# achacond/k-step_FM-index

Hardware: AMD Instinct MI355X
Metric: Mqueries/s (100 bp reads, 3 Gbase index) (higher is better)
Workload: dtype u32; 1 GPU; Task-2Step backward search, 3 Gbase index, 10M x 100 bp reads per GPU; backend=task-mid, k=2, d=64, ref_size=3000000000, queries_per_gpu=10000000, qlen=100, query_upload=ascii, parallelism=query-sharded dp1, index replicated per GPU, no collective

## Files before the change

### include/kstep_fmi.h

```cpp
#ifndef KSTEP_FMI_H_
#define KSTEP_FMI_H_

#include <stdint.h>

#ifdef __cplusplus
extern "C" {
#endif

enum {
  KFMI_SUCCESS                = 0,
  KFMI_E_OPENING_INDEX_FILE   = 1,
  KFMI_E_ALLOCATING_BWT       = 2,
  KFMI_E_ALLOCATING_FMI       = 3,
  KFMI_E_READING_BWT          = 4,
  KFMI_E_READING_FMI          = 5,
  KFMI_E_SAVING_INDEX_FILE    = 6,
  KFMI_E_SAVING_BWT_FILE      = 7,
  KFMI_E_BUILDING_BWT         = 8,
  KFMI_E_BUILDING_FMI         = 9,
  KFMI_E_OPENING_REFERENCE_FILE = 10,
  KFMI_E_ALLOCATING_REFERENCE = 11,
  KFMI_E_READING_MFASTA_FILE  = 12,
  KFMI_E_READING_REFERENCE_FILE = 13,
  KFMI_E_OPENING_MFASTA_FILE  = 14,
  KFMI_E_ALLOCATING_MFASTA    = 15,
  KFMI_E_ALLOCATING_RESULTS   = 16,
  KFMI_E_OPENING_RESULTS_FILE = 17,
  KFMI_E_READING_RESULTS_FILE = 18,
  KFMI_E_NOT_IMPLEMENTED      = 19,
  KFMI_E_NO_DEVICE            = 30,
  KFMI_E_DEVICE_ALLOC         = 31,
  KFMI_E_KERNEL               = 32,
  KFMI_E_BAD_ARGUMENT         = 33,
  KFMI_E_NOT_ON_DEVICE        = 34,
  KFMI_INDEX_VER_BASELINE      = 100,
  KFMI_INDEX_VER_INTERLEAVE    = 101,
  KFMI_INDEX_VER_BASELINE_AC   = 200,
  KFMI_INDEX_VER_INTERLEAVE_AC = 201
};


int32_t loadIndex(const char *fn, void **index);
int32_t saveIndex(const char *fn, void *index);
int32_t initResults(uint32_t numresults, void **results);
void    searchIndexGPU(void *index, void *queries, void *resIntervals);
void    searchIndexCPU(void *index, void *queries, void *resIntervals);
int32_t freeIndex(void **index);
int32_t freeReference(void **reference, void **index);
int32_t buildIndex(void *reference, void **index);
int32_t freeQueriesGPU(void **queries);
int32_t freeResultsGPU(void **results);
int32_t freeIndexGPU(void **index);
int32_t transferGPUtoCPU(void *results);
int32_t transferCPUtoGPU(void *index, void *queries, void *results);
int32_t kfmi_queries_upload_form(void *queries);

double   sampleTime(void);
uint32_t base2index(uint32_t base);
int32_t  loadRef(const char *fn, uint32_t refsize, void **reference);
int32_t  saveRef(const char *fn, void *reference);
int32_t  loadQueries(const char *fn, uint32_t sizequery, uint32_t numqueries, void **queries);
int32_t  writeResults(const char *fn, uint32_t *results, uint32_t numqueries);
int32_t  loadResults(const char *fn, void **results);
int32_t  freeQueries(void **queries);
int32_t  freeResults(void **results);
int32_t  saveResults(const char *fn, void *results, void *index);
char    *errorCommon(int32_t e);


int32_t     kfmi_set_backend(const char *name);
const char *kfmi_get_backend(void);
int32_t     kfmi_set_device(int32_t device);
int32_t     kfmi_device_count(void);
int32_t     kfmi_device_pci_bus_id(int32_t device, char *buf, int32_t len);
int32_t     kfmi_last_error(void);
int32_t     kfmi_search(void *index, void *queries, void *results);
int32_t     kfmi_search_cpu(void *index, void *queries, void *results, int32_t nthreads);
#define KFMI_FTAB_AUTO 0xFFFFFFFFu
int32_t     kfmi_set_ftab(uint32_t bases);
uint32_t    kfmi_ftab_auto_bases(uint64_t rows, uint32_t K, uint64_t budget_bytes);
#define KFMI_FTAB_BUDGET_FREE 0xFFFFFFFFFFFFFFFFull
int32_t     kfmi_set_ftab_budget(uint64_t bytes);
uint64_t    kfmi_device_ftab_bytes(void *index);
#define KFMI_SKIP_AUTO 0xFFFFFFFFu
int32_t     kfmi_set_skip(uint32_t mode);
uint32_t    kfmi_skip_in_effect(void);
uint32_t    kfmi_skip_auto(uint64_t rows, uint32_t K, uint64_t budget_bytes);
uint64_t    kfmi_device_skip_bytes(void *index);
int32_t     kfmi_device_skip_table(void *index, void *out, uint64_t entries, uint32_t *steps);
#define KFMI_JUMP_AUTO 0xFFFFFFFFu
#define KFMI_JUMP_MIN_DEFAULT 8u
int32_t     kfmi_set_jump(uint32_t mode);
uint32_t    kfmi_jump_in_effect(void);
int32_t     kfmi_set_jump_min(uint32_t bases);
uint32_t    kfmi_jump_min(void);
uint32_t    kfmi_jump_auto(uint64_t rows, uint32_t K, uint64_t budget_bytes);
uint64_t    kfmi_device_jump_bytes(void *index);
int32_t     kfmi_device_jump_tables(void *index, uint32_t member, uint32_t *sa, uint32_t *isa, uint64_t rows,
                                    uint32_t *text, uint64_t words);
int32_t     kfmi_set_jump_lines(uint32_t mode);
uint32_t    kfmi_jump_lines(void);
uint64_t    kfmi_device_jump_line_bytes(void *index);
int32_t     kfmi_device_jump_lines(void *index, uint32_t member, uint32_t *out, uint64_t lines);
int32_t     kfmi_jump_line_geometry(uint64_t n, uint64_t p, uint32_t nb, uint64_t *out);
int32_t     kfmi_set_split_class(uint32_t cls);
int32_t     kfmi_set_fused(int32_t on);
int32_t     kfmi_set_walk_check(uint32_t mode);
int32_t     kfmi_fail_index_uploads(uint32_t n);
int32_t     kfmi_walk_check_last(void);
int32_t     kfmi_set_devices(const int32_t *devices, int32_t n);
int32_t     kfmi_get_devices(int32_t *devices, int32_t cap);
int32_t     kfmi_last_timing(double *ms_total, double *ms_pack, double *ms_lf);

int32_t kfmi_load_index_tag(const char *fn, uint32_t required_tag, void **index);
int32_t kfmi_index_from_image(const void *image, uint64_t bytes, void **index);
int32_t kfmi_index_image(void *index, const void **image, uint64_t *bytes);
int32_t kfmi_index_header(void *index, uint32_t *out14);

int32_t kfmi_transform_interleave(void *index100, void **index101);
int32_t kfmi_transform_ac(void *index100, void **index200, void **index201);
int32_t kfmi_transform_plain(void *index_ac, void **index100);

int32_t   kfmi_queries_from_buffer(const char *ascii, uint64_t num, uint32_t size, void **queries);
int32_t   kfmi_results_alloc(uint64_t num, void **results);
uint32_t *kfmi_results_host(void *results);
uint64_t  kfmi_results_num(void *results);

int32_t kfmi_build_index_cpu(const char *text, uint64_t n, uint32_t k, uint32_t d, void **index);
int32_t kfmi_build_index_gpu(const char *text, uint64_t n, uint32_t k, uint32_t d,
                             int32_t want_host_image, void **index);
int32_t kfmi_derive_index_gpu(void *index, uint32_t k_out, int32_t want_host_image, void **out);
int32_t kfmi_set_alphabet(const char *mode);
int32_t kfmi_build_stats(uint64_t *ties, uint32_t *rounds);

int32_t kfmi_count_blocks(void *index, void *queries, uint64_t *blocks);
int32_t kfmi_count_lines(void *index, void *queries, uint64_t out[4]);

int32_t kfmi_search_stream(void *index, const char *ascii, uint64_t num, uint32_t size,
                           uint32_t *results, uint64_t chunk);
int32_t kfmi_load_queries_gpu(const char *fn, uint32_t sizequery, uint64_t numqueries, void **queries);
int32_t kfmi_pack_queries(const char *ascii, uint64_t num, uint32_t size, uint32_t *words);
int32_t kfmi_pack_queries_k(const char *ascii, uint64_t num, uint32_t size, uint32_t k, uint32_t *words);
int32_t kfmi_host_threads(void);
int32_t kfmi_host_alloc(uint64_t bytes, void **p);
int32_t kfmi_host_free(void *p);
int32_t kfmi_stream_release(void);
double  kfmi_stream_hostpacked_fraction(void);

enum { KFMI_STRAND_FWD = 1, KFMI_STRAND_REV = 2, KFMI_STRAND_BOTH = 3 };
int32_t kfmi_search_strands(void *index, void *queries, void *results, uint32_t strands);
int32_t kfmi_search_stream_strands(void *index, const char *ascii, uint64_t num, uint32_t size,
                                   uint32_t *results, uint64_t chunk, uint32_t strands);
int32_t kfmi_search_cpu_strands(void *index, void *queries, void *results, uint32_t strands, int32_t nthreads);
int32_t kfmi_revcomp_queries(const char *ascii, uint64_t num, uint32_t size, char *out);
int32_t kfmi_strand_words_host(const uint32_t *words, uint64_t num, uint32_t size, uint32_t k,
                               uint32_t strands, uint32_t *out);
int32_t kfmi_reverse_stream_host(const uint32_t *words, uint64_t num, uint32_t size, uint32_t maxw,
                                 uint32_t *out);

int32_t kfmi_search_seeds(void *index, void *queries, void *intervals, void *spans,
                          uint32_t max_seeds, uint32_t strands);
int32_t kfmi_search_seeds_cpu(void *index, void *queries, void *intervals, void *spans,
                              uint32_t max_seeds, uint32_t strands, int32_t nthreads);

#define KFMI_HIT_NONE         0xFFFFFFFFu
#define KFMI_HIT_MISM_MASK    0x0000FFFFu
#define KFMI_HIT_MULTI        0x00010000u
#define KFMI_HIT_SCORED_SHIFT 20
#define KFMI_VERIFY_MAX_OCC   256u
int32_t kfmi_verify_seeds(void *index, void *queries, void *intervals, void *spans, void *hits,
                          uint32_t max_seeds, uint32_t strands, uint32_t max_occ, uint32_t max_mism);
int32_t kfmi_verify_seeds_cpu(const char *text, uint64_t n, const uint32_t *sa, uint64_t rows,
                              void *queries, void *intervals, void *spans, void *hits,
                              uint32_t max_seeds, uint32_t strands, uint32_t max_occ, uint32_t max_mism,
                              int32_t nthreads);
int32_t kfmi_results_to_device(void *results);

enum {
  KFMI_TRACE_STEP = 1u, KFMI_TRACE_SKIP_HIT = 1u << 16, KFMI_TRACE_SKIP_MISS = 1u << 24,
  KFMI_TRACE_JUMP_TRIED = 1u, KFMI_TRACE_JUMP_LINE = 2u,
  KFMI_TRACE_JUMP_OUT_SHIFT = 2, KFMI_TRACE_JUMP_POS_SHIFT = 4, KFMI_TRACE_JUMP_NB_SHIFT = 16,
  KFMI_TRACE_JUMP_TAKEN = 0, KFMI_TRACE_JUMP_REFUSED = 1, KFMI_TRACE_JUMP_DIFFERED = 2, KFMI_TRACE_JUMP_BAD_ISA = 3
};
int32_t kfmi_search_trace(void *index, void *queries, void *results, uint32_t *trace);

int32_t kfmi_probe_replay(void *index, void *queries, int32_t unroll, int32_t groups, int32_t reps, double *ms,
                          uint64_t *lines, uint64_t *trace_bytes);

uint64_t kfmi_device_index_bytes(void *index);


int32_t kfmi_build_index_ex(const char *text, uint64_t n, uint32_t k, uint32_t d, uint32_t sa_rate,
                            int32_t on_device, void **index);
int32_t kfmi_index_sa(void *index, const uint32_t **sa, uint64_t *count, uint32_t *rate);
int32_t kfmi_save_sa(const char *fn, void *index);
int32_t kfmi_load_sa(const char *fn, void *index);
int32_t         kfmi_locate(void *index, void *results, uint32_t max_occ, void **locations);
uint64_t        kfmi_locations_total(void *locations);
const uint64_t *kfmi_locations_offsets(void *locations);
const uint32_t *kfmi_locations_positions(void *locations);
int32_t         kfmi_locations_free(void **locations);

#ifdef __cplusplus
}
#endif

#endif
```

### k-step_fm-index_amd/csrc/hip/kfmi_coop.h

```cpp
#ifndef KFMI_COOP_H_
#define KFMI_COOP_H_

#include <type_traits>

#include "kfmi_device.h"

namespace kfmi {


template <class G>
struct CoopCfg {
  static constexpr int BC = G::BMW / 4;
  static constexpr bool NBR = G::NEIGHBOR;
  static constexpr int TPR = NBR ? pow2ceil(2 * BC) : pow2ceil(BC + 1);
  static constexpr int RPR = 64 / TPR;
  static constexpr int SLOT = TPR * 16;
  static constexpr int MAXREQ = 128;
  static constexpr int MAXR = MAXREQ / RPR;
  using Desc = typename std::conditional<(G::NC > 16), uint64_t, uint32_t>::type;
  static constexpr int WAVE_LDS = MAXREQ * SLOT + MAXREQ * (int) sizeof(Desc);
  static constexpr int WPB0 = 65536 / WAVE_LDS;
  static constexpr int WPB = WPB0 < 1 ? 1 : (WPB0 > 4 ? 4 : WPB0);
  static constexpr bool OK = (G::BMW % 4 == 0) && (G::EW % 4 == 0) && (G::BOFF % 4 == 0) &&
                             (!G::ACRULE || G::HALF >= 4) && (!G::MIDLINES || G::NC >= 4) &&
                             TPR <= 64;
};

template <class G>
__device__ __forceinline__ const uint8_t* coop_chunk_addr(const IdxArgs& ix, uint32_t b, uint32_t c, int k)
{
  using C = CoopCfg<G>;
  const uint8_t* base = reinterpret_cast<const uint8_t*>(ix.ent);
  const uint64_t eb = (uint64_t) b * (G::EW * 4);
  if constexpr (G::MIDLINES) {
    const uint64_t lb = (uint64_t) (b >> 1) * (G::EW * 4);
    if (k < C::BC) return base + lb + ((b & 1u) * G::BMW + 4 * k) * 4;
    return base + lb + (G::MIDCNT + (c & ~3u)) * 4;
  }
  if constexpr (G::LAY == LAY_GRP) {
    const uint64_t lb = ((uint64_t) b * G::NGRP + c / G::NCG) * (G::EW * 4);
    if (k < C::BC) return base + lb + 16 * k;
    return base + lb + (G::BMW + ((c % G::NCG) & ~3u)) * 4;
  }
  if (k < C::BC) return base + eb + (G::BOFF + 4 * k) * 4;
  if constexpr (G::LAY == LAY_INTER) {
    return base + eb + (G::BMW + (c & ~3u)) * 4;
  } else {
    const bool e = ((b & 1u) != 0) == (c < (uint32_t) G::HALF);
    return base + (uint64_t) (b + (e ? 1u : 0u)) * (G::EW * 4) + ((c & (G::HALF - 1)) & ~3u) * 4;
  }
}

template <class G>
__device__ __forceinline__ uint32_t coop_lf(const IdxArgs& ix, const uint8_t* slot, uint32_t b, uint32_t X,
                                            uint32_t c, const uint32_t (&sx)[2 * G::K])
{
  using C = CoopCfg<G>;
  const int o = (int) (X - b * (uint32_t) G::D);
  bool e = false;
  if constexpr (G::ACRULE) e = ((b & 1u) != 0) == (c < (uint32_t) G::HALF);
  if constexpr (G::MIDLINES) e = (b & 1u) == 0;
  uint32_t pop = 0, all = 0;
  if constexpr (G::PW <= 4) {
#pragma unroll
    for (int k = 0; k < C::BC; ++k) {
      const uint4 v = *reinterpret_cast<const uint4*>(slot + 16 * k);
      const uint32_t pl[4] = {v.x, v.y, v.z, v.w};
#pragma unroll
      for (int h = 0; h < 4 / G::PW; ++h) {
        const int w = k * (4 / G::PW) + h;
        uint32_t m = row_mask(o - 32 * w);
        if constexpr (G::TWO_SIDED) m = e ? ~m : m;
        const uint32_t sel = select_rows<G::K>(&pl[h * G::PW], sx);
        pop += __popc(m & sel);
        if constexpr (G::LAY == LAY_MIDAC) all += __popc(sel);
      }
    }
  } else {
    uint32_t pl[G::BMW];
#pragma unroll
    for (int k = 0; k < C::BC; ++k) {
      const uint4 v = *reinterpret_cast<const uint4*>(slot + 16 * k);
      pl[4 * k] = v.x; pl[4 * k + 1] = v.y; pl[4 * k + 2] = v.z; pl[4 * k + 3] = v.w;
    }
#pragma unroll
    for (int w = 0; w < G::NB; ++w) {
      uint32_t m = row_mask(o - 32 * w);
      if constexpr (G::TWO_SIDED) m = e ? ~m : m;
      pop += __popc(m & select_rows<G::K>(&pl[w * G::PW], sx));
    }
  }
  const uint32_t cnt = reinterpret_cast<const uint32_t*>(slot + 16 * C::BC)[c & 3u];
  if constexpr (G::LAY == LAY_MIDAC)
    if (b >= ix.ac_tail_b0) return ac_tail_step<G>(ix, b, c, X, pop, all);
  return finish<G>(ix, cnt, pop, b, c, X, e);
}

template <class G>
__device__ __forceinline__ uint32_t coop_lf_nbr(const IdxArgs& ix, const uint8_t* slot, uint32_t b, uint32_t X,
                                                uint32_t c, const uint32_t (&sx)[2 * G::K], uint32_t cnt, bool e,
                                                bool prev)
{
  using C = CoopCfg<G>;
  const int o = (int) (X - b * (uint32_t) G::D);
  uint32_t pl[G::BMW];
#pragma unroll
  for (int k = 0; k < C::BC; ++k) {
    const uint4 v = *reinterpret_cast<const uint4*>(slot + 16 * k);
    pl[4 * k] = v.x; pl[4 * k + 1] = v.y; pl[4 * k + 2] = v.z; pl[4 * k + 3] = v.w;
  }
  uint32_t pop = 0;
#pragma unroll
  for (int w = 0; w < G::NB; ++w) {
    uint32_t m = row_mask(o - 32 * w);
    if constexpr (G::TWO_SIDED) m = e ? ~m : m;
    pop += __popc(m & select_rows<G::K>(&pl[w * G::PW], sx));
  }
  if (prev) {
#pragma unroll
    for (int k = 0; k < C::BC; ++k) {
      const uint4 v = *reinterpret_cast<const uint4*>(slot + 16 * (C::BC + k));
      pl[4 * k] = v.x; pl[4 * k + 1] = v.y; pl[4 * k + 2] = v.z; pl[4 * k + 3] = v.w;
    }
#pragma unroll
    for (int w = 0; w < G::NB; ++w) pop += __popc(select_rows<G::K>(&pl[w * G::PW], sx));
    return finish_prev<G>(ix, cnt, pop, b, c, X);
  }
  return finish<G>(ix, cnt, pop, b, c, X, e);
}

template <class G>
__host__ __device__ constexpr uint32_t coop_stage_rows(uint32_t m)
{
  uint32_t r = 64;
  while (r >= 16 && r * m + 16 > (uint32_t) CoopCfg<G>::WAVE_LDS) r >>= 1;
  return r >= 16 ? r : 0u;
}

template <class G, int MAXW>
__global__ __launch_bounds__(64 * CoopCfg<G>::WPB) void coop_kernel(IdxArgs ix, const uint32_t* __restrict__ qp,
                                                                    const uint8_t* __restrict__ ascii, uint32_t m,
                                                                    uint64_t num, uint32_t steps, uint32_t nwords,
                                                                    uint32_t* __restrict__ res)
{
  using C = CoopCfg<G>;
  constexpr int RW = MAXW > 0 ? MAXW : 1;
  constexpr int CW = MAXW > 0 && G::K == 3 ? k3_words<RW>() : RW;
  extern __shared__ __attribute__((aligned(16))) uint8_t lds[];
  const int wave = threadIdx.x >> 6;
  const int lane = threadIdx.x & 63;
  uint8_t* wl = lds + wave * C::WAVE_LDS;
  using Desc = typename C::Desc;
  Desc* tab = reinterpret_cast<Desc*>(wl + C::MAXREQ * C::SLOT);
  const uint64_t q0 = ((uint64_t) blockIdx.x * C::WPB + wave) * 64;
  if (q0 >= num) return;
  const uint64_t q = q0 + lane;
  const uint64_t qs = q < num ? q : num - 1;
  const int k = lane % C::TPR;
  const int g = lane / C::TPR;
  uint32_t cw[CW];
  uint32_t rc = 0;
  if constexpr (MAXW > 0) {
    uint32_t raw[RW];
    const uint32_t rpr = coop_stage_rows<G>(m);
#pragma unroll 1
    for (uint32_t h = 0; h < 64u / rpr; ++h) {
      const uint64_t r0 = q0 + h * rpr;
      const uint64_t nr = r0 < num ? (num - r0 < rpr ? num - r0 : rpr) : 0;
      const uint32_t n16 = (uint32_t) ((nr * m + 15) / 16);
      const uint4* src = reinterpret_cast<const uint4*>(ascii + r0 * m);
      for (uint32_t i = lane; i < n16; i += 64) reinterpret_cast<uint4*>(wl)[i] = src[i];
      asm volatile("s_waitcnt vmcnt(0) lgkmcnt(0)" ::: "memory");
      if ((uint32_t) lane / rpr == h) {
        row_codes<MAXW>(wl, (uint64_t) (lane % rpr) * m, m - ix.rem, raw);
        rc = rem_code(wl + (uint64_t) (lane % rpr) * m + m - ix.rem, ix.rem);
      }
      asm volatile("s_waitcnt lgkmcnt(0)" ::: "memory");
    }
    if (q >= num) {
#pragma unroll
      for (int i = 0; i < RW; ++i) raw[i] = 0;
      rc = 0;
    }
    if constexpr (G::K == 3) recut30<RW>(raw, cw);
    else {
#pragma unroll
      for (int i = 0; i < CW; ++i) cw[i] = raw[i];
    }
  }
  uint32_t L = 0, R = ix.bwtsize;
  uint32_t skip = 0;
  if (ix.ftab && steps >= ix.ftab_steps) {
    skip = ix.ftab_steps;
    uint32_t w0;
    if constexpr (MAXW > 0) w0 = cw[0];
    else w0 = qp[qs];
    const uint2 lr = ix.ftab[w0 & ix.ftab_mask];
    L = lr.x;
    R = lr.y;
  }
  if (ix.rem) {
    if constexpr (MAXW == 0) rc = qp[(uint64_t) nwords * num + qs];
    const uint2 lr = ix.rtab[rc];
    L = lr.x;
    R = lr.y;
  }

  for (uint32_t w = 0; w < nwords; ++w) {
    uint32_t word;
    if constexpr (MAXW > 0) {
      word = cw[0];
#pragma unroll
      for (int i = 0; i + 1 < CW; ++i) cw[i] = cw[i + 1];
    } else {
      word = qp[(uint64_t) w * num + qs];
    }
    const uint32_t left = steps - w * G::SPW;
#pragma unroll 1
    for (int j = 0; j < G::SPW; ++j) {
      if ((uint32_t) j >= left) break;
      if (w * G::SPW + j < skip) continue;
      const uint32_t c = (word >> (2 * G::K * j)) & (uint32_t) (G::NC - 1);
      const uint32_t bl = L / (uint32_t) G::D, br = R / (uint32_t) G::D;
      const bool needR = br != bl;
      const uint64_t mask = __ballot(needR);
      const uint32_t nreq = 64u + (uint32_t) __popcll(mask);
      const uint32_t slotR = 64u + __builtin_amdgcn_mbcnt_hi((uint32_t) (mask >> 32),
                                                             __builtin_amdgcn_mbcnt_lo((uint32_t) mask, 0u));
      bool eL = false, eR = false, pL = false, pR = false;
      const uint32_t* acL = nullptr;
      const uint32_t* acR = nullptr;
      if constexpr (C::NBR) {
        Where<G> wL = locate<G>(ix, bl, c);
        Where<G> wR = locate<G>(ix, br, c);
        line_local_prev<G>(ix, bl, c, wL);
        line_local_prev<G>(ix, br, c, wR);
        eL = wL.e;
        pL = wL.prev;
        acL = wL.cnt;
        eR = wR.e;
        pR = wR.prev;
        acR = wR.cnt;
      }
      tab[lane] = (Desc) bl * (Desc) G::NC + c;
      if (needR) tab[slotR] = (Desc) br * (Desc) G::NC + c;
      asm volatile("s_waitcnt lgkmcnt(0)" ::: "memory");
      uint32_t cwL = 0, cwR = 0;
      const uint32_t rounds = (nreq + C::RPR - 1) / C::RPR;
      for (uint32_t r = 0; r < rounds; ++r) {
        const uint32_t s = r * C::RPR + g;
        if constexpr (C::NBR) {
          if (s < nreq && k < 2 * C::BC) {
            const Desc desc = tab[s];
            const uint32_t b = (uint32_t) (desc / (Desc) G::NC), cc = (uint32_t) (desc % (Desc) G::NC);
            Where<G> w = locate<G>(ix, b, cc);
            line_local_prev<G>(ix, b, cc, w);
            const uint32_t* p = k < C::BC ? w.planes + 4 * k
                                : w.prev ? w.pplanes + 4 * (k - C::BC)
                                : k == C::BC ? reinterpret_cast<const uint32_t*>(reinterpret_cast<uintptr_t>(w.cnt) & ~(uintptr_t) 15)
                                : nullptr;
            if (p)
              __builtin_amdgcn_global_load_lds((const void*) p,
                                               (__attribute__((address_space(3))) void*) (wl + r * 1024), 16, 0, 0);
          }
        } else if (s < nreq && k <= C::BC) {
          const Desc desc = tab[s];
          const uint32_t b = (uint32_t) (desc / (Desc) G::NC), cc = (uint32_t) (desc % (Desc) G::NC);
          const uint8_t* src = coop_chunk_addr<G>(ix, b, cc, k);
          __builtin_amdgcn_global_load_lds((const void*) src,
                                           (__attribute__((address_space(3))) void*) (wl + r * 1024), 16, 0, 0);
        }
      }
      if constexpr (C::NBR) {
        const uint64_t mpl = __ballot(pL), mpr = __ballot(needR && pR);
        uint64_t sv, gm;
        asm volatile("s_mov_b64 %[sv], exec\n"
                     "s_bfm_b64 %[gm], 32, 0\n"
                     "s_and_b64 exec, %[sv], %[gm]\n"
                     "s_and_b64 exec, exec, %[ml]\n"
                     "s_cbranch_execz .Lcl0_%=\n"
                     "global_load_dword %[cl], %[al], off\n"
                     ".Lcl0_%=:\n"
                     "s_and_b64 exec, %[sv], %[gm]\n"
                     "s_and_b64 exec, exec, %[mr]\n"
                     "s_cbranch_execz .Lcc0_%=\n"
                     "global_load_dword %[cr], %[ar], off\n"
                     ".Lcc0_%=:\n"
                     "s_bfm_b64 %[gm], 32, 32\n"
                     "s_and_b64 exec, %[sv], %[gm]\n"
                     "s_and_b64 exec, exec, %[ml]\n"
                     "s_cbranch_execz .Lcl1_%=\n"
                     "global_load_dword %[cl], %[al], off\n"
                     ".Lcl1_%=:\n"
                     "s_and_b64 exec, %[sv], %[gm]\n"
                     "s_and_b64 exec, exec, %[mr]\n"
                     "s_cbranch_execz .Lcc1_%=\n"
                     "global_load_dword %[cr], %[ar], off\n"
                     ".Lcc1_%=:\n"
                     "s_mov_b64 exec, %[sv]\n"
                     "s_waitcnt vmcnt(0)\n"
                     : [cl] "=&v"(cwL), [cr] "=&v"(cwR), [sv] "=&s"(sv), [gm] "=&s"(gm)
                     : [al] "v"(acL), [ar] "v"(acR), [ml] "s"(mpl), [mr] "s"(mpr)
                     : "memory", "scc");
      } else {
        asm volatile("s_waitcnt vmcnt(0)" ::: "memory");
      }
      uint32_t sx[2 * G::K];
      plane_xor<G::K>(c, sx);
      uint32_t nL, nR;
      if constexpr (C::NBR) {
        const uint8_t* sL = wl + lane * C::SLOT;
        const uint8_t* sR = wl + (needR ? slotR : (uint32_t) lane) * C::SLOT;
        const uint32_t cL = pL ? cwL : reinterpret_cast<const uint32_t*>(sL + 16 * C::BC)[c & 3u];
        const uint32_t cR = needR ? (pR ? cwR : reinterpret_cast<const uint32_t*>(sR + 16 * C::BC)[c & 3u]) : cL;
        nL = coop_lf_nbr<G>(ix, sL, bl, L, c, sx, cL, eL, pL);
        nR = coop_lf_nbr<G>(ix, sR, br, R, c, sx, cR, needR ? eR : eL, needR ? pR : pL);
      } else {
        nL = coop_lf<G>(ix, wl + lane * C::SLOT, bl, L, c, sx);
        nR = coop_lf<G>(ix, wl + (needR ? slotR : (uint32_t) lane) * C::SLOT, br, R, c, sx);
      }
      L = nL;
      R = nR;
      asm volatile("s_waitcnt lgkmcnt(0)" ::: "memory");
    }
  }
  if (q < num) *reinterpret_cast<uint2*>(res + 2 * q) = make_uint2(L, R);
}

template <class G>
hipError_t coop_launch(hipStream_t st, IdxArgs ix, const uint32_t* qp, const uint8_t* ascii, uint32_t m, int maxw,
                       uint64_t num, uint32_t steps, uint32_t nwords, uint32_t* res)
{
  using C = CoopCfg<G>;
  if constexpr (!C::OK) {
    return hipErrorInvalidValue;
  } else {
    const uint64_t waves = (num + 63) / 64;
    const uint64_t blocks = (waves + C::WPB - 1) / C::WPB;
    const size_t lds = (size_t) C::WPB * C::WAVE_LDS;
    if (maxw == 8)
      hipLaunchKernelGGL((coop_kernel<G, 8>), dim3((uint32_t) blocks), dim3(64 * C::WPB), lds, st, ix, qp, ascii, m,
                         num, steps, nwords, res);
    else if (maxw == 16)
      hipLaunchKernelGGL((coop_kernel<G, 16>), dim3((uint32_t) blocks), dim3(64 * C::WPB), lds, st, ix, qp, ascii, m,
                         num, steps, nwords, res);
    else
      hipLaunchKernelGGL((coop_kernel<G, 0>), dim3((uint32_t) blocks), dim3(64 * C::WPB), lds, st, ix, qp, ascii, m,
                         num, steps, nwords, res);
    return hipGetLastError();
  }
}

}

#endif
```

### k-step_fm-index_amd/csrc/hip/kfmi_device.h

```cpp
#ifndef KFMI_DEVICE_H_
#define KFMI_DEVICE_H_

#include <hip/hip_runtime.h>
#include <stdint.h>

namespace kfmi {

enum Layout : int { LAY_INTER = 0, LAY_AC = 1, LAY_MID = 3, LAY_MIDAC = 5, LAY_GRP = 6 };

__host__ __device__ constexpr int pow2ceil(int x) { int p = 1; while (p < x) p <<= 1; return p; }

template <int K_, int NB_, int LAY_>
struct Geo {
  static constexpr int K = K_;
  static constexpr int NB = NB_;
  static constexpr int LAY = LAY_;
  static constexpr int D = 32 * NB;
  static constexpr int NC = 1 << (2 * K);
  static constexpr int HALF = NC / 2;
  static constexpr int PW = 2 * K;
  static constexpr int BMW = PW * NB;
  static constexpr int NCG = NC < 16 ? NC : 16;
  static constexpr int NGRP = NC / NCG;
  static constexpr int EW = LAY == LAY_INTER ? BMW + NC
                          : LAY == LAY_AC    ? HALF + BMW
                          : LAY == LAY_GRP    ? pow2ceil(BMW + NCG)
                          : pow2ceil(2 * BMW + NC);
  static constexpr int BOFF = LAY == LAY_AC ? HALF : 0;
  static constexpr int MIDCNT = 2 * BMW;
  static constexpr bool ACRULE = LAY == LAY_AC;
  static constexpr int SPW = 32 / (2 * K);
  static constexpr bool SMALL = BMW <= 16;
  static constexpr bool TWO_SIDED = LAY == LAY_AC || LAY == LAY_MID || LAY == LAY_MIDAC;
  static constexpr bool MIDLINES = LAY == LAY_MID || LAY == LAY_MIDAC;
  static constexpr bool NEIGHBOR = (LAY == LAY_INTER || LAY == LAY_AC) && SMALL && BOFF + EW + BMW <= 32;
};

struct DollarArgs {
  uint32_t dpos[4];
  uint32_t dbase[4];
  uint32_t dblk[4];
  uint32_t duniq;
};

struct IdxArgs {
  const uint32_t* __restrict__ ent;
  uint32_t bwtsize;
  DollarArgs dl;
  const uint2* __restrict__ ftab;
  uint32_t ftab_steps, ftab_mask;
  const uint32_t* __restrict__ ac_tail;
  uint32_t ac_tail_b0;
  const uint2* __restrict__ rtab;
  uint32_t rem;
  uint32_t split;
  uint32_t lf_cap;
  const uint2* __restrict__ skip;
  uint32_t skip_rows, skip_steps, skip_split;
  const uint32_t* __restrict__ jsa;
  uint32_t jump_min, jump_split;
};

constexpr uint32_t SKIP_NONE = 0xFFFFFFFFu;

constexpr uint32_t JUMP_LINE_S = 16, JUMP_LINE_W = 256 - JUMP_LINE_S, JUMP_LINE_DW = 32, JUMP_LINE_TEXT = JUMP_LINE_S;
static_assert(JUMP_LINE_S == 16 && JUMP_LINE_S + 256 / 16 == JUMP_LINE_DW, "a line: S entries, then 256 bases in 16 dwords");
constexpr uint32_t JUMP_SPLIT4 = 4u, JUMP_LINES = 0x100u, JUMP_LINES_GROUPED = 0x200u;
constexpr uint32_t JUMP_LINES_GROUPED_MAX_M = 192;

__host__ __device__ constexpr uint64_t jump_text_words(uint64_t n) { return n / 16 + 2; }
__host__ __device__ constexpr uint64_t jump_line_count(uint64_t n) { return n / JUMP_LINE_S + 2; }
__host__ __device__ constexpr uint64_t jump_lines_off(uint64_t rows)
{
  return (2 * rows + jump_text_words(rows - 1) + (JUMP_LINE_DW - 1)) & ~(uint64_t) (JUMP_LINE_DW - 1);
}

struct JumpLineAt {
  uint64_t isa_dw, text_dw;
  uint32_t shift, ndw;
};
__host__ __device__ constexpr JumpLineAt jump_line_at(uint32_t n, uint32_t p, uint32_t nb)
{
  const uint32_t e = n - p + nb, j = e / JUMP_LINE_S;
  const uint32_t s = 256u - JUMP_LINE_S + e % JUMP_LINE_S - nb;
  const uint64_t line = (uint64_t) j * JUMP_LINE_DW;
  return JumpLineAt{line + e % JUMP_LINE_S, line + JUMP_LINE_TEXT + (s >> 4), (s & 15u) * 2u,
                    ((s + nb + 15u) >> 4) - (s >> 4)};
}

typedef unsigned int v4u __attribute__((ext_vector_type(4)));
typedef unsigned int v2u __attribute__((ext_vector_type(2)));

template <bool NT>
__device__ __forceinline__ v4u ld4(const uint32_t* p)
{
  if constexpr (NT) return __builtin_nontemporal_load(reinterpret_cast<const v4u*>(p));
  else return *reinterpret_cast<const v4u*>(p);
}
template <bool NT>
__device__ __forceinline__ v2u ld2(const uint32_t* p)
{
  if constexpr (NT) return __builtin_nontemporal_load(reinterpret_cast<const v2u*>(p));
  else return *reinterpret_cast<const v2u*>(p);
}
template <bool NT>
__device__ __forceinline__ uint32_t ld1(const uint32_t* p)
{
  if constexpr (NT) return __builtin_nontemporal_load(p);
  else return *p;
}

template <class G>
__host__ __device__ constexpr int plane_align()
{
  int a = 16;
  while (a > 4 && ((4 * G::EW) % a || (4 * G::BOFF) % a)) a >>= 1;
  return a;
}

template <int A, int N, bool NT = false>
__device__ __forceinline__ void load_words(const uint32_t* __restrict__ p, uint32_t* __restrict__ out)
{
  if constexpr (A >= 16 && N % 4 == 0) {
#pragma unroll
    for (int i = 0; i < N / 4; ++i) {
      const v4u v = ld4<NT>(p + 4 * i);
      out[4 * i + 0] = v.x; out[4 * i + 1] = v.y; out[4 * i + 2] = v.z; out[4 * i + 3] = v.w;
    }
  } else if constexpr (A >= 8 && N % 2 == 0) {
#pragma unroll
    for (int i = 0; i < N / 2; ++i) {
      asm volatile("" ::: "memory");
      const v2u v = ld2<NT>(p + 2 * i);
      out[2 * i + 0] = v.x; out[2 * i + 1] = v.y;
    }
  } else {
#pragma unroll
    for (int i = 0; i < N; ++i) {
      asm volatile("" ::: "memory");
      out[i] = ld1<NT>(p + i);
    }
  }
}

__device__ __forceinline__ uint32_t code_of(uint32_t x)
{
  uint32_t b1 = x & 4u, f2 = x & 2u;
  uint32_t b0 = b1 ? (f2 ^ 2u) : f2;
  return (b1 | b0) >> 1;
}

__device__ __forceinline__ uint32_t group_codes_rev(uint32_t x)
{
  const uint32_t b1 = (x >> 2) & 0x01010101u;
  const uint32_t y = (b1 << 1) | (((x >> 1) & 0x01010101u) ^ b1);
  return ((y >> 24) & 0x03u) | ((y >> 14) & 0x0Cu) | ((y >> 4) & 0x30u) | ((y << 6) & 0xC0u);
}

template <int MAXW>
__device__ __forceinline__ void push_codes(uint32_t (&cw)[MAXW], uint32_t v, uint32_t sh)
{
#pragma unroll
  for (int k = MAXW - 1; k > 0; --k) cw[k] = __builtin_amdgcn_alignbit(cw[k], cw[k - 1], 32u - sh);
  cw[0] = (cw[0] << sh) | v;
}

template <int MAXW>
__device__ __forceinline__ void row_codes(const uint8_t* __restrict__ base, uint64_t off, uint32_t m,
                                          uint32_t (&cw)[MAXW])
{
  const uint32_t* a = reinterpret_cast<const uint32_t*>(base + (off & ~3ull));
  const uint32_t sh = (uint32_t) (off & 3u);
#pragma unroll
  for (int k = 0; k < MAXW; ++k) asm volatile("v_mov_b32 %0, 0" : "=v"(cw[k]));
  const uint32_t ng = m >> 2, rem = m & 3u;
  uint32_t lo = a[0];
#pragma unroll 8
  for (uint32_t i = 0; i < ng; ++i) {
    const uint32_t hi = a[i + 1];
    push_codes<MAXW>(cw, group_codes_rev(__builtin_amdgcn_alignbyte(hi, lo, sh)), 8u);
    lo = hi;
  }
  if (rem) {
    const uint32_t x = __builtin_amdgcn_alignbyte(a[ng + 1], lo, sh);
    push_codes<MAXW>(cw, group_codes_rev(x) >> (2u * (4u - rem)), 2u * rem);
  }
}

__device__ __forceinline__ uint32_t rem_code(const uint8_t* __restrict__ p, uint32_t rem)
{
  uint32_t c = 0;
  for (uint32_t u = 0; u < rem; ++u) c |= code_of(p[rem - 1 - u]) << (2 * u);
  return c;
}

template <int MAXW>
__host__ __device__ constexpr int k3_words() { return (MAXW * 32 + 29) / 30; }

template <int MAXW>
__device__ __forceinline__ void recut30(const uint32_t (&in)[MAXW], uint32_t (&out)[k3_words<MAXW>()])
{
#pragma unroll
  for (int j = 0; j < k3_words<MAXW>(); ++j) {
    const int bit = 30 * j, w = bit >> 5, sh = bit & 31;
    const uint32_t lo = w < MAXW ? in[w] : 0u;
    const uint32_t hi = w + 1 < MAXW ? in[w + 1] : 0u;
    out[j] = (sh ? ((lo >> sh) | (hi << (32 - sh))) : lo) & 0x3FFFFFFFu;
  }
}

__host__ __device__ constexpr uint32_t stage_rows(uint32_t m) { return m <= 128 ? 32u : 16u; }
__host__ __device__ constexpr uint32_t stage_slot_bytes(uint32_t m) { return (stage_rows(m) * m + 31u) & ~15u; }

template <int MAXW>
__device__ __forceinline__ void stage_query_codes(const uint8_t* __restrict__ ascii, uint64_t num, uint32_t m,
                                                  uint8_t* __restrict__ lds, uint32_t (&cw)[MAXW], uint32_t rem,
                                                  uint32_t& rc)
{
  const uint32_t lane = threadIdx.x & 63u, wv = threadIdx.x >> 6;
  const uint32_t rpr = stage_rows(m);
  uint8_t* wl = lds + wv * stage_slot_bytes(m);
  const uint64_t q0 = (uint64_t) blockIdx.x * 256 + wv * 64;
#pragma unroll 1
  for (uint32_t h = 0; h < 64u / rpr; ++h) {
    const uint64_t r0 = q0 + h * rpr;
    const uint64_t nr = r0 < num ? (num - r0 < rpr ? num - r0 : rpr) : 0;
    const uint32_t n16 = (uint32_t) ((nr * m + 15) / 16);
    const uint4* src = reinterpret_cast<const uint4*>(ascii + r0 * m);
    for (uint32_t i = lane; i < n16; i += 64) reinterpret_cast<uint4*>(wl)[i] = src[i];
    __syncthreads();
    if (lane / rpr == h) {
      row_codes<MAXW>(wl, (uint64_t) (lane % rpr) * m, m - rem, cw);
      rc = rem_code(wl + (uint64_t) (lane % rpr) * m + m - rem, rem);
    }
    __syncthreads();
  }
}

__device__ __forceinline__ uint32_t row_mask(int sh)
{
  sh = sh < 0 ? 0 : (sh > 32 ? 32 : sh);
  return (uint32_t) ((0xFFFFFFFF00000000ull) >> sh);
}

template <int K>
__device__ __forceinline__ void plane_xor(uint32_t c, uint32_t (&sx)[2 * K])
{
#pragma unroll
  for (int p = 0; p < 2 * K; ++p) sx[p] = ((c >> p) & 1u) ? 0u : 0xFFFFFFFFu;
}

template <int K>
__device__ __forceinline__ uint32_t select_rows(const uint32_t* pl, const uint32_t (&sx)[2 * K])
{
  uint32_t v = ~0u;
#pragma unroll
  for (int p = 0; p < 2 * K; ++p) v &= pl[p] ^ sx[p];
  return v;
}

template <int K, bool TWO>
__device__ __forceinline__ int dollar_fix(const DollarArgs& dl, uint32_t b, uint32_t c, uint32_t X, bool e)
{
  int corr = 0;
#pragma unroll
  for (int s = 0; s < K; ++s) {
    bool hit = (dl.dblk[s] == b) && (dl.dbase[s] == c);
    bool cond = (TWO && e) ? (X <= dl.dpos[s]) : (X > dl.dpos[s]);
    corr += (hit && cond) ? 1 : 0;
  }
  return corr;
}

template <class G>
struct Where {
  const uint32_t* planes;
  const uint32_t* cnt;
  bool e;
  bool prev = false;
  const uint32_t* pplanes = nullptr;
};

template <class G>
__device__ __forceinline__ void line_local_prev(const IdxArgs& ix, uint32_t b, uint32_t c, Where<G>& w)
{
  if constexpr (G::NEIGHBOR) {
    if (b == 0) return;
    const uint64_t pb = 4ull * ((uint64_t) b * G::EW + G::BOFF);
    const uint64_t line = pb >> 7;
    if (((uint64_t) (w.cnt - ix.ent) * 4ull) >> 7 == line) return;
    if constexpr (G::LAY == LAY_AC) {
      if (!w.e || b >= ix.ac_tail_b0) return;
    }
    const uint32_t cw = G::LAY == LAY_AC ? (c & (G::HALF - 1)) : (uint32_t) G::BMW + c;
    const uint64_t e0 = (uint64_t) (b - 1) * G::EW;
    if ((4ull * (e0 + G::BOFF)) >> 7 != line || (4ull * (e0 + G::BOFF + G::BMW) - 1) >> 7 != line ||
        (4ull * (e0 + cw)) >> 7 != line)
      return;
    w.prev = true;
    w.e = false;
    w.pplanes = ix.ent + e0 + G::BOFF;
    w.cnt = ix.ent + e0 + cw;
  }
}

template <class G>
__device__ __forceinline__ Where<G> locate(const IdxArgs& ix, uint32_t b, uint32_t c)
{
  Where<G> w;
  if constexpr (G::LAY == LAY_INTER) {
    const uint32_t* ent = ix.ent + (uint64_t) b * G::EW;
    w.planes = ent;
    w.cnt = ent + G::BMW + c;
    w.e = false;
  } else if constexpr (G::LAY == LAY_AC) {
    const uint32_t* ent = ix.ent + (uint64_t) b * G::EW;
    w.e = ((b & 1u) != 0) == (c < (uint32_t) G::HALF);
    w.planes = ent + G::BOFF;
    w.cnt = ix.ent + (uint64_t) (b + (w.e ? 1u : 0u)) * G::EW + (c & (G::HALF - 1));
  } else if constexpr (G::LAY == LAY_GRP) {
    const uint32_t* line = ix.ent + ((uint64_t) b * G::NGRP + c / G::NCG) * G::EW;
    w.planes = line;
    w.cnt = line + G::BMW + c % G::NCG;
    w.e = false;
  } else {
    const uint32_t* line = ix.ent + (uint64_t) (b >> 1) * G::EW;
    w.e = (b & 1u) == 0;
    w.planes = line + (b & 1u) * G::BMW;
    w.cnt = line + G::MIDCNT + c;
  }
  return w;
}

template <class G, bool NT = false>
__device__ __forceinline__ uint32_t load_counter(const IdxArgs& ix, const Where<G>& w, uint32_t b, uint32_t c)
{
  (void) ix; (void) b; (void) c;
  return ld1<NT>(w.cnt);
}

template <class G>
__device__ __forceinline__ uint32_t ac_clamp(const IdxArgs& ix, uint32_t v)
{
  const uint32_t cap = ((ix.bwtsize + (uint32_t) G::D - 1u) / (uint32_t) G::D + 2u) * (uint32_t) G::D - 1u;
  return v > cap ? cap : v;
}

template <int K>
__device__ __forceinline__ uint32_t dollar_dup(const DollarArgs& dl, uint32_t b, uint32_t c)
{
  uint32_t n = 0;
#pragma unroll
  for (int s = 1; s < K; ++s) n += (dl.dblk[s] == b && dl.dbase[s] == c && !((dl.duniq >> s) & 1u)) ? 1u : 0u;
  return n;
}

template <class G>
__device__ __forceinline__ bool ac_rule_e(uint32_t b, uint32_t c)
{
  return ((b & 1u) != 0) == (c < (uint32_t) G::HALF);
}

template <class G>
__device__ __forceinline__ uint32_t finish(const IdxArgs& ix, uint32_t cnt, uint32_t pop, uint32_t b, uint32_t c,
                                          uint32_t X, bool e)
{
  const int corr = dollar_fix<G::K, G::TWO_SIDED>(ix.dl, b, c, X, e);
  const uint32_t bc = pop - (uint32_t) corr;
  if constexpr (G::ACRULE) return ac_clamp<G>(ix, e ? cnt - bc : cnt + bc);
  if constexpr (G::MIDLINES) {
    uint32_t v = e ? cnt - bc : cnt + bc;
    if (G::K > 1 && ix.dl.duniq != (1u << G::K) - 1u) {
      const uint32_t dup = dollar_dup<G::K>(ix.dl, b, c);
      const bool want = G::LAY == LAY_MIDAC && ac_rule_e<G>(b, c);
      v = v - (e ? dup : 0u) + (want ? dup : 0u);
    }
    return min(v, ix.lf_cap);
  }
  if constexpr (G::TWO_SIDED) return min(e ? cnt - bc : cnt + bc, ix.lf_cap);
  return min(cnt + bc, ix.lf_cap);
}

template <class G>
__device__ __forceinline__ uint32_t finish_prev(const IdxArgs& ix, uint32_t cnt, uint32_t pop, uint32_t b,
                                               uint32_t c, uint32_t X)
{
  int corr = 0;
#pragma unroll
  for (int s = 0; s < G::K; ++s) {
    if (ix.dl.dbase[s] != c) continue;
    if (ix.dl.dblk[s] == b) corr += X > ix.dl.dpos[s] ? 1 : 0;
    else if (ix.dl.dblk[s] + 1u == b) corr += (ix.dl.duniq >> s) & 1u;
  }
  uint32_t v = cnt + pop - (uint32_t) corr;
  if constexpr (G::ACRULE) {
    if (G::K > 1 && ac_rule_e<G>(b, c)) v += dollar_dup<G::K>(ix.dl, b, c);
    return ac_clamp<G>(ix, v);
  }
  return min(v, ix.lf_cap);
}

template <class G>
__device__ __forceinline__ uint32_t ac_tail_step(const IdxArgs& ix, uint32_t b, uint32_t c, uint32_t X,
                                                 uint32_t pop_mid, uint32_t pop_all)
{
  const bool e = ((b & 1u) != 0) == (c < (uint32_t) G::HALF);
  const bool e_mid = (b & 1u) == 0;
  const uint32_t pop = e == e_mid ? pop_mid : pop_all - pop_mid;
  uint32_t row = b + (e ? 1u : 0u) - ix.ac_tail_b0;
  row = row > 2u ? 2u : row;
  const uint32_t cnt = ix.ac_tail[row * (uint32_t) G::NC + c];
  const int corr = dollar_fix<G::K, true>(ix.dl, b, c, X, e);
  const uint32_t bc = pop - (uint32_t) corr;
  return ac_clamp<G>(ix, e ? cnt - bc : cnt + bc);
}

template <class G>
struct Blk {
  uint32_t bm[G::BMW];
  uint32_t bp[G::NEIGHBOR ? G::BMW : 1];
  uint32_t cnt;
  uint32_t b;
  bool e;
  bool prev;
};

template <class G, bool NT = false>
__device__ __forceinline__ void load_planes(const uint32_t* __restrict__ p, uint32_t (&bm)[G::BMW])
{
  load_words<plane_align<G>(), G::BMW, NT>(p, bm);
}

template <class G, bool NT = false>
__device__ __forceinline__ void fetch_block(const IdxArgs& ix, uint32_t b, uint32_t c, Blk<G>& k)
{
  Where<G> w = locate<G>(ix, b, c);
  line_local_prev<G>(ix, b, c, w);
  k.b = b;
  k.e = w.e;
  k.prev = w.prev;
  load_planes<G, NT>(w.planes, k.bm);
  if constexpr (G::NEIGHBOR) {
    if (w.prev) load_planes<G, NT>(w.pplanes, k.bp);
  }
  k.cnt = load_counter<G, NT>(ix, w, b, c);
}

template <class G>
__device__ __forceinline__ uint32_t lf_from_block(const IdxArgs& ix, const Blk<G>& k, uint32_t X, uint32_t c,
                                                  const uint32_t (&sx)[2 * G::K])
{
  const int o = (int) (X - k.b * (uint32_t) G::D);
  uint32_t pop = 0;
#pragma unroll
  for (int w = 0; w < G::NB; ++w) {
    uint32_t m = row_mask(o - 32 * w);
    if constexpr (G::TWO_SIDED) m = k.e ? ~m : m;
    pop += __popc(m & select_rows<G::K>(&k.bm[w * G::PW], sx));
  }
  if constexpr (G::LAY == LAY_MIDAC) {
    if (k.b >= ix.ac_tail_b0) {
      uint32_t all = 0;
#pragma unroll
      for (int w = 0; w < G::NB; ++w) all += __popc(select_rows<G::K>(&k.bm[w * G::PW], sx));
      return ac_tail_step<G>(ix, k.b, c, X, pop, all);
    }
  }
  if constexpr (G::NEIGHBOR) {
    if (k.prev) {
#pragma unroll
      for (int w = 0; w < G::NB; ++w) pop += __popc(select_rows<G::K>(&k.bp[w * G::PW], sx));
      return finish_prev<G>(ix, k.cnt, pop, k.b, c, X);
    }
  }
  return finish<G>(ix, k.cnt, pop, k.b, c, X, k.e);
}

template <class G>
__device__ __forceinline__ uint32_t lf_stream(const IdxArgs& ix, uint32_t X, uint32_t c,
                                              const uint32_t (&sx)[2 * G::K])
{
  const uint32_t b = X / (uint32_t) G::D;
  const int o = (int) (X - b * (uint32_t) G::D);
  const Where<G> wh = locate<G>(ix, b, c);
  const uint32_t cnt = load_counter<G>(ix, wh, b, c);
  const uint32_t* pl = wh.planes;
  constexpr int CH = G::NB < 8 ? G::NB : 8;
  uint32_t pop = 0, all = 0;
#pragma unroll
  for (int w0 = 0; w0 < G::NB; w0 += CH) {
    uint32_t v[CH][G::PW];
#pragma unroll
    for (int j = 0; j < CH; ++j) {
      const int w = w0 + j;
      if (w >= G::NB) break;
      load_words<plane_align<G>(), G::PW>(pl + G::PW * w, v[j]);
    }
#pragma unroll
    for (int j = 0; j < CH; ++j) {
      const int w = w0 + j;
      if (w >= G::NB) break;
      uint32_t m = row_mask(o - 32 * w);
      if constexpr (G::TWO_SIDED) m = wh.e ? ~m : m;
      const uint32_t sel = select_rows<G::K>(v[j], sx);
      pop += __popc(m & sel);
      if constexpr (G::LAY == LAY_MIDAC) all += __popc(sel);
    }
  }
  if constexpr (G::LAY == LAY_MIDAC)
    if (b >= ix.ac_tail_b0) return ac_tail_step<G>(ix, b, c, X, pop, all);
  return finish<G>(ix, cnt, pop, b, c, X, wh.e);
}

}

#endif
```

### k-step_fm-index_amd/csrc/hip/kfmi_jump.hip

```cpp
#include <hip/hip_runtime.h>
#include <stdint.h>
#include <stdlib.h>
#include <atomic>
#include <mutex>
#include <shared_mutex>

#include "../kfmi_internal.h"
#include "kfmi_device.h"
#include "kfmi_runtime.h"

namespace kfmi {

static std::atomic<uint32_t> g_jump_min{KFMI_JUMP_MIN_DEFAULT};
static std::atomic<int> g_jump_lines{-1};

extern "C" int32_t kfmi_set_jump_min(uint32_t bases)
{
  if (bases < 1) return KFMI_E_BAD_ARGUMENT;
  g_jump_min.store(bases, std::memory_order_relaxed);
  return KFMI_SUCCESS;
}

extern "C" uint32_t kfmi_jump_min(void) { return g_jump_min.load(std::memory_order_relaxed); }

extern "C" int32_t kfmi_set_jump_lines(uint32_t mode)
{
  if (mode > 2) return KFMI_E_BAD_ARGUMENT;
  g_jump_lines.store((int) mode, std::memory_order_relaxed);
  return KFMI_SUCCESS;
}

extern "C" uint32_t kfmi_jump_lines(void)
{
  const int v = g_jump_lines.load(std::memory_order_relaxed);
  if (v >= 0) return (uint32_t) v;
  static const uint32_t env = [] {
    const char* e = getenv("KFMI_JUMP_LINES");
    if (!e || !*e) return 1u;
    const int x = atoi(e);
    return x < 0 || x > 2 ? 1u : (uint32_t) x;
  }();
  return env;
}

static uint64_t text_words(uint64_t n) { return jump_text_words(n); }

extern "C" int32_t kfmi_jump_line_geometry(uint64_t n, uint64_t p, uint32_t nb, uint64_t* out)
{
  if (!out || n < 1 || n >= 0xFFFFFFFFull || p > n || nb < 1 || nb > JUMP_LINE_W || nb > p) return KFMI_E_BAD_ARGUMENT;
  const JumpLineAt at = jump_line_at((uint32_t) n, (uint32_t) p, nb);
  out[0] = jump_lines_off(n + 1);
  out[1] = jump_line_count(n);
  out[2] = at.isa_dw;
  out[3] = at.text_dw;
  out[4] = at.shift;
  out[5] = at.ndw;
  return KFMI_SUCCESS;
}

extern "C" uint32_t kfmi_jump_auto(uint64_t rows, uint32_t K, uint64_t budget_bytes)
{
  if (K < 1 || K > 2 || rows < 2 || rows > 0xFFFFFFFFull) return 0;
  return 16 * rows + 4 * text_words(rows - 1) <= budget_bytes ? 1u : 0u;
}

static bool jump_applies(const kfmi_dev_index* di)
{
  return di->K >= 1 && di->K <= 2 && !is_coop(di->backend) && (di->layout == LAY_INTER || di->layout == LAY_MID) &&
         di->bwtsize >= 2;
}

constexpr uint32_t JUMP_BAD_CHAIN = 1u, JUMP_BAD_POS = 2u, JUMP_BAD_ISA = 4u;

__device__ __forceinline__ int dollar_of(uint32_t row, const DollarArgs& dl, uint32_t K)
{
  int s = -1;
  for (int t = (int) K - 1; t >= 0; --t)
    if (dl.dpos[t] == row) s = t;
  return s;
}

__global__ __launch_bounds__(256) void jump_dist0_kernel(const uint32_t* __restrict__ next, uint64_t rows,
                                                         uint32_t* __restrict__ dist)
{
  for (uint64_t i = (uint64_t) blockIdx.x * 256 + threadIdx.x; i < rows; i += (uint64_t) gridDim.x * 256)
    dist[i] = next[i] == (uint32_t) i ? 0u : 1u;
}

__global__ __launch_bounds__(256) void jump_round_kernel(const uint32_t* __restrict__ next, const uint32_t* __restrict__ dist,
                                                         uint64_t rows, uint32_t split, uint32_t* __restrict__ next2,
                                                         uint32_t* __restrict__ dist2)
{
  const int grp = (int) (threadIdx.x & 63) / 16;
  for (uint64_t i0 = (uint64_t) blockIdx.x * 256 + (threadIdx.x & ~63u); i0 < rows; i0 += (uint64_t) gridDim.x * 256) {
    const uint64_t i = i0 + (threadIdx.x & 63u);
    const bool on = i < rows;
    const uint32_t j = on ? next[i] : 0u;
    const uint32_t d = on ? dist[i] : 0u;
    const bool ok = on && (uint64_t) j < rows;
    uint32_t nj = j, dj = 0u;
    if (split) {
#pragma unroll
      for (int g = 0; g < 4; ++g)
        if (ok && grp == g) {
          nj = next[j];
          dj = dist[j];
        }
    } else if (ok) {
      nj = next[j];
      dj = dist[j];
    }
    if (on) {
      next2[i] = nj;
      dist2[i] = d + dj;
    }
  }
}

__global__ __launch_bounds__(256) void jump_sa_kernel(uint32_t* __restrict__ next_sa, const uint32_t* __restrict__ dist,
                                                      uint64_t rows, DollarArgs dl, uint32_t K, uint32_t* __restrict__ bad)
{
  for (uint64_t i = (uint64_t) blockIdx.x * 256 + threadIdx.x; i < rows; i += (uint64_t) gridDim.x * 256) {
    const int s = dollar_of(next_sa[i], dl, K);
    const uint64_t p = (uint64_t) (s < 0 ? 0 : s) + (uint64_t) K * dist[i];
    uint32_t v = (uint32_t) p;
    if (s < 0) {
      atomicOr(bad, JUMP_BAD_CHAIN);
      v = SKIP_NONE;
    } else if (p >= rows) {
      atomicOr(bad, JUMP_BAD_POS);
      v = SKIP_NONE;
    }
    next_sa[i] = v;
  }
}

__global__ __launch_bounds__(256) void jump_isa_kernel(const uint32_t* __restrict__ sa, uint64_t rows, uint32_t split,
                                                       uint32_t* __restrict__ isa)
{
  const int grp = (int) (threadIdx.x & 63) / 16;
  for (uint64_t i0 = (uint64_t) blockIdx.x * 256 + (threadIdx.x & ~63u); i0 < rows; i0 += (uint64_t) gridDim.x * 256) {
    const uint64_t i = i0 + (threadIdx.x & 63u);
    const uint32_t p = i < rows ? sa[i] : SKIP_NONE;
    const bool ok = (uint64_t) p < rows;
    if (split) {
#pragma unroll
      for (int g = 0; g < 4; ++g)
        if (ok && grp == g) isa[p] = (uint32_t) i;
    } else if (ok) {
      isa[p] = (uint32_t) i;
    }
  }
}

__global__ __launch_bounds__(256) void jump_isa_check_kernel(const uint32_t* __restrict__ isa, uint64_t rows,
                                                             uint32_t* __restrict__ bad)
{
  for (uint64_t i = (uint64_t) blockIdx.x * 256 + threadIdx.x; i < rows; i += (uint64_t) gridDim.x * 256)
    if ((uint64_t) isa[i] >= rows) atomicOr(bad, JUMP_BAD_ISA);
}

void free_jump(kfmi_dev_index* di)
{
  if (di->jump_sa) (void) hipFree(di->jump_sa);
  di->jump_sa = nullptr;
  di->jump_auto = -1;
}

static int32_t build_jump(kfmi_dev_index* di, hipStream_t st)
{
  const uint64_t rows = di->bwtsize, n = rows - 1, words = text_words(n);
  const uint64_t loff = jump_lines_off(rows), lines = jump_line_count(n);
  uint32_t *keep = nullptr, *bad = nullptr;
  auto done = [&](int32_t code) {
    if (keep) (void) hipFree(keep);
    if (bad) (void) hipFree(bad);
    (void) hipGetLastError();
    return code;
  };
  static_assert(JUMP_LINE_DW >= 2 * JUMP_LINE_S, "two distance dwords per row fit the lines' part");
  if (hipMalloc((void**) &keep, 4 * (loff + lines * JUMP_LINE_DW)) != hipSuccess || hipMalloc((void**) &bad, 8) != hipSuccess)
    return done(KFMI_E_DEVICE_ALLOC);
  uint32_t* tmp = keep + loff;
  uint32_t* a[4] = {keep, tmp, keep + rows, tmp + rows};
  const uint32_t split = split_for(8 * rows, LAY_INTER) == 4u ? 1u : 0u;
  const dim3 grid(grid_blocks((rows + 255) / 256, 1u << 20));
  uint32_t rounds = 0;
  for (uint64_t span = 1; span < rows; span <<= 1) ++rounds;
  int cur = (rounds & 1u) ? 2 : 0;
  SearchLaunch l{};
  l.st = st;
  l.ix = idx_args(di);
  l.num = rows;
  l.perm_next = a[cur];
  l.perm_bad = bad;
  uint32_t h_bad[2] = {0, 0};
  auto flags = [&] {
    return hipGetLastError() == hipSuccess && hipMemcpyAsync(h_bad, bad, 8, hipMemcpyDeviceToHost, st) == hipSuccess &&
           hipStreamSynchronize(st) == hipSuccess;
  };
  if (hipMemsetAsync(bad, 0, 8, st) != hipSuccess || dispatch(Op::PermCheck, di->K, di->nb, di->layout, l) != hipSuccess)
    return done(KFMI_E_KERNEL);
  hipLaunchKernelGGL(jump_dist0_kernel, grid, dim3(256), 0, st, a[cur], rows, a[cur + 1]);
  for (uint32_t r = 0; r < rounds; ++r, cur ^= 2)
    hipLaunchKernelGGL(jump_round_kernel, grid, dim3(256), 0, st, a[cur], a[cur + 1], rows, split, a[cur ^ 2],
                       a[(cur ^ 2) + 1]);
  uint32_t *sa = a[0], *dist = a[1], *isa = a[2], *text = keep + 2 * rows;
  hipLaunchKernelGGL(jump_sa_kernel, grid, dim3(256), 0, st, sa, dist, rows, di->dl, di->K, bad + 1);
  if (hipMemsetAsync(isa, 0xFF, 4 * rows, st) != hipSuccess) return done(KFMI_E_KERNEL);
  hipLaunchKernelGGL(jump_isa_kernel, grid, dim3(256), 0, st, sa, rows, split, isa);
  hipLaunchKernelGGL(jump_isa_check_kernel, grid, dim3(256), 0, st, isa, rows, bad + 1);
  if (!flags()) return done(KFMI_E_KERNEL);
  if (h_bad[0] | h_bad[1]) {
    di->jump_none = 1;
    return done(KFMI_SUCCESS);
  }
  l.jump_isa = isa;
  l.jump_text = text;
  l.jump_words = words;
  l.jump_split = l.ix.split == 1u ? 0u : 1u;
  l.num = n;
  l.jump_lines = tmp;
  if (dispatch(Op::JumpText, di->K, di->nb, di->layout, l) != hipSuccess ||
      dispatch(Op::JumpLines, di->K, di->nb, di->layout, l) != hipSuccess || hipStreamSynchronize(st) != hipSuccess)
    return done(KFMI_E_KERNEL);
  di->jump_sa = keep;
  keep = nullptr;
  return done(KFMI_SUCCESS);
}

int32_t auto_jump(kfmi_dev_index* di, hipStream_t st)
{
  std::lock_guard<std::mutex> lk(di->ftab_mu);
  if (di->jump_auto >= 0 || di->jump_sa) return KFMI_SUCCESS;
  di->jump_auto = 0;
  if (!jump_applies(di) || di->jump_none) return KFMI_SUCCESS;
  if (!kfmi_jump_auto(di->bwtsize, di->K, table_budget_now())) return KFMI_SUCCESS;
  const int32_t e = build_jump(di, st);
  if (e && e != KFMI_E_DEVICE_ALLOC) return e;
  di->jump_auto = (!e && di->jump_sa) ? 1 : 0;
  return KFMI_SUCCESS;
}

int32_t use_jump(kfmi_dev_index* di, hipStream_t st, IdxArgs& ix, uint32_t want)
{
  ix.jsa = nullptr;
  ix.jump_min = 0xFFFFFFFFu;
  ix.jump_split = 1;
  if (!want || !jump_applies(di)) return KFMI_SUCCESS;
  if (want == 2) {
    const int32_t e = auto_jump(di, st);
    if (e) return e;
  }
  {
    std::lock_guard<std::mutex> lk(di->ftab_mu);
    if (!di->jump_sa) {
      if (want == 2 || di->jump_none) return KFMI_SUCCESS;
      const int32_t e = build_jump(di, st);
      if (e) return e;
      if (!di->jump_sa) return KFMI_SUCCESS;
    }
  }
  ix.jsa = di->jump_sa;
  ix.jump_min = g_jump_min.load(std::memory_order_relaxed);
  const uint32_t lines = kfmi_jump_lines();
  const bool split4 = split_for(8ull * di->bwtsize, LAY_INTER) == 4u;
  ix.jump_split = (split4 ? JUMP_SPLIT4 : 0u) | (lines ? JUMP_LINES : 0u) | (lines == 1u && split4 ? JUMP_LINES_GROUPED : 0u);
  return KFMI_SUCCESS;
}

static uint64_t jump_bytes_of(kfmi_dev_index* di)
{
  std::lock_guard<std::mutex> lk(di->ftab_mu);
  return di->jump_sa ? 8ull * di->bwtsize + 4 * text_words(di->bwtsize - 1) : 0ull;
}

static uint64_t jump_line_bytes_of(kfmi_dev_index* di)
{
  std::lock_guard<std::mutex> lk(di->ftab_mu);
  return di->jump_sa ? 4ull * JUMP_LINE_DW * jump_line_count(di->bwtsize - 1) : 0ull;
}

extern "C" uint64_t kfmi_device_jump_bytes(void* index) { return sum_members(index, jump_bytes_of); }

extern "C" uint64_t kfmi_device_jump_line_bytes(void* index) { return sum_members(index, jump_line_bytes_of); }

extern "C" int32_t kfmi_device_jump_tables(void* index, uint32_t member, uint32_t* sa, uint32_t* isa, uint64_t rows,
                                           uint32_t* text, uint64_t words)
{
  kfmi_fmi_t* f = (kfmi_fmi_t*) index;
  if (!f || !sa || !isa || !text) return KFMI_E_BAD_ARGUMENT;
  DeviceGuard dg;
  std::shared_lock<RwLock> lk(index_lock(f));
  kfmi_dev_index* di = nullptr;
  const int32_t e = member_index(f, member, &di);
  if (e) return e;
  std::lock_guard<std::mutex> tl(di->ftab_mu);
  if (!di->jump_sa) return KFMI_E_NOT_ON_DEVICE;
  if (rows != di->bwtsize || words != text_words(di->bwtsize - 1)) return KFMI_E_BAD_ARGUMENT;
  if (hipSetDevice(di->device) != hipSuccess) return KFMI_E_NO_DEVICE;
  HIP_OK(hipMemcpy(sa, di->jump_sa, 4ull * rows, hipMemcpyDeviceToHost));
  HIP_OK(hipMemcpy(isa, di->jump_sa + rows, 4ull * rows, hipMemcpyDeviceToHost));
  HIP_OK(hipMemcpy(text, di->jump_sa + 2 * rows, 4ull * words, hipMemcpyDeviceToHost));
  return KFMI_SUCCESS;
}

extern "C" int32_t kfmi_device_jump_lines(void* index, uint32_t member, uint32_t* out, uint64_t lines)
{
  kfmi_fmi_t* f = (kfmi_fmi_t*) index;
  if (!f || !out) return KFMI_E_BAD_ARGUMENT;
  DeviceGuard dg;
  std::shared_lock<RwLock> lk(index_lock(f));
  kfmi_dev_index* di = nullptr;
  const int32_t e = member_index(f, member, &di);
  if (e) return e;
  std::lock_guard<std::mutex> tl(di->ftab_mu);
  if (!di->jump_sa) return KFMI_E_NOT_ON_DEVICE;
  if (lines != jump_line_count(di->bwtsize - 1)) return KFMI_E_BAD_ARGUMENT;
  if (hipSetDevice(di->device) != hipSuccess) return KFMI_E_NO_DEVICE;
  HIP_OK(hipMemcpy(out, di->jump_sa + jump_lines_off(di->bwtsize), 4ull * JUMP_LINE_DW * lines, hipMemcpyDeviceToHost));
  return KFMI_SUCCESS;
}

}
```

### k-step_fm-index_amd/csrc/hip/kfmi_kernels.h

```cpp
#ifndef KFMI_KERNELS_H_
#define KFMI_KERNELS_H_

#include <hip/hip_runtime.h>
#include <stdint.h>
#include <stdlib.h>
#include <algorithm>

#include "../../../include/kstep_fmi.h"
#include "kfmi_device.h"
#include "kfmi_grid.h"
#include "kfmi_strands.h"
#include "kfmi_coop.h"
#include "kfmi_locate.h"

namespace kfmi {



template <class G, int QPT>
__device__ __forceinline__ void fetch_ends(const IdxArgs& ix, const uint32_t (&L)[QPT], const uint32_t (&R)[QPT],
                                           const uint32_t (&c)[QPT], Blk<G> (&kl)[QPT], Blk<G> (&kr)[QPT])
{
#pragma unroll
  for (int i = 0; i < QPT; ++i) fetch_block<G>(ix, L[i] / (uint32_t) G::D, c[i], kl[i]);
#pragma unroll
  for (int i = 0; i < QPT; ++i) {
    const uint32_t br = R[i] / (uint32_t) G::D;
    if (br != kl[i].b) fetch_block<G>(ix, br, c[i], kr[i]);
    else kr[i] = kl[i];
  }
}

template <class G>
struct X4 {
  static constexpr bool OK = G::SMALL && G::BMW == 8 && G::BOFF % 4 == 0 && G::EW % 4 == 0;
};

#define KFMI_X4_BODY(T)                                      \
  "s_and_b64 exec, %[sv], %[gm]\n"                           \
  "global_load_dwordx4 %[l0], %[al], off\n"                  \
  "global_load_dwordx4 %[l1], %[al], off offset:16\n"        \
  "global_load_dword %[cl], %[acl], off\n"                   \
  KFMI_X4_PREV_L(T)                                          \
  "s_and_b64 exec, %[sv], %[gm]\n"                           \
  "s_and_b64 exec, exec, %[nr]\n"                            \
  KFMI_X4_SJ("r" T)                                          \
  "global_load_dwordx4 %[r0], %[ar], off\n"                  \
  "global_load_dwordx4 %[r1], %[ar], off offset:16\n"        \
  "global_load_dword %[cr], %[acr], off\n"                   \
  KFMI_X4_PREV_R(T)                                          \
  KFMI_X4_SL("r" T)
#define KFMI_X4_G1 "s_mov_b64 %[gm], -1\n" KFMI_X4_BODY("a")
#define KFMI_X4_G2 "s_bfm_b64 %[gm], 32, 0\n" KFMI_X4_BODY("a") "s_bfm_b64 %[gm], 32, 32\n" KFMI_X4_BODY("b")
#define KFMI_X4_ASM(GROUPS) "s_mov_b64 %[sv], exec\n" GROUPS "s_mov_b64 exec, %[sv]\ns_waitcnt vmcnt(0)\n"
#define KFMI_X4_OUT                                                                                          \
  [l0] "=&v"(l0), [l1] "=&v"(l1), [r0] "=&v"(r0), [r1] "=&v"(r1), [cl] "=&v"(cl), [cr] "=&v"(cr), [sv] "=&s"(sv), \
      [gm] "=&s"(gm)
#define KFMI_X4_IN [al] "v"(wl.planes), [acl] "v"(wl.cnt), [ar] "v"(wr.planes), [acr] "v"(wr.cnt), [nr] "s"(nr)
#define KFMI_X4_OUTP KFMI_X4_OUT, [p0] "=&v"(p0), [p1] "=&v"(p1), [q0] "=&v"(q0), [q1] "=&v"(q1)
#define KFMI_X4_INP KFMI_X4_IN, [pl] "s"(pl), [pr] "s"(pr), [po0] "i"(PO), [po1] "i"(PO + 16)
#define KFMI_X4_SJ(L) "s_cbranch_execz .Lx4" L "_%=\n"
#define KFMI_X4_SL(L) ".Lx4" L "_%=:\n"
#define KFMI_X4_PREV_L_ON(T)                                 \
  "s_and_b64 exec, exec, %[pl]\n"                            \
  KFMI_X4_SJ("p" T)                                          \
  "global_load_dwordx4 %[p0], %[al], off offset:%[po0]\n"    \
  "global_load_dwordx4 %[p1], %[al], off offset:%[po1]\n"    \
  KFMI_X4_SL("p" T)
#define KFMI_X4_PREV_R_ON(T)                                 \
  "s_and_b64 exec, exec, %[pr]\n"                            \
  KFMI_X4_SJ("r" T)                                          \
  "global_load_dwordx4 %[q0], %[ar], off offset:%[po0]\n"    \
  "global_load_dwordx4 %[q1], %[ar], off offset:%[po1]\n"

template <class G, int SPLIT>
__device__ __forceinline__ void fetch_ends_x4(const IdxArgs& ix, uint32_t L, uint32_t R, uint32_t c, Blk<G>& kl,
                                              Blk<G>& kr)
{
  static_assert(SPLIT == 7 || SPLIT == 8, "fetch form: 7, 8 = two, one lane group(s)");
  const uint32_t bl = L / (uint32_t) G::D, br = R / (uint32_t) G::D;
  Where<G> wl = locate<G>(ix, bl, c);
  Where<G> wr = locate<G>(ix, br, c);
  line_local_prev<G>(ix, bl, c, wl);
  line_local_prev<G>(ix, br, c, wr);
  const bool needR = br != bl;
  const uint64_t nr = __ballot(needR);
  v4u l0, l1, r0, r1;
  uint32_t cl, cr;
  uint64_t sv, gm;
  if constexpr (G::NEIGHBOR) {
    const uint64_t pl = __ballot(wl.prev), pr = __ballot(wr.prev);
    constexpr int PO = -4 * G::EW;
    v4u p0, p1, q0, q1;
#define KFMI_X4_PREV_L(T) KFMI_X4_PREV_L_ON(T)
#define KFMI_X4_PREV_R(T) KFMI_X4_PREV_R_ON(T)
    if constexpr (SPLIT == 8)
      asm volatile(KFMI_X4_ASM(KFMI_X4_G1) : KFMI_X4_OUTP : KFMI_X4_INP : "memory", "scc");
    else
      asm volatile(KFMI_X4_ASM(KFMI_X4_G2) : KFMI_X4_OUTP : KFMI_X4_INP : "memory", "scc");
#undef KFMI_X4_PREV_L
#undef KFMI_X4_PREV_R
    const v4u pa = needR ? q0 : p0, pb = needR ? q1 : p1;
    kl.bp[0] = p0.x; kl.bp[1] = p0.y; kl.bp[2] = p0.z; kl.bp[3] = p0.w;
    kl.bp[4] = p1.x; kl.bp[5] = p1.y; kl.bp[6] = p1.z; kl.bp[7] = p1.w;
    kr.bp[0] = pa.x; kr.bp[1] = pa.y; kr.bp[2] = pa.z; kr.bp[3] = pa.w;
    kr.bp[4] = pb.x; kr.bp[5] = pb.y; kr.bp[6] = pb.z; kr.bp[7] = pb.w;
  } else {
#define KFMI_X4_PREV_L(T)
#define KFMI_X4_PREV_R(T)
    if constexpr (SPLIT == 8)
      asm volatile(KFMI_X4_ASM(KFMI_X4_G1) : KFMI_X4_OUT : KFMI_X4_IN : "memory", "scc");
    else
      asm volatile(KFMI_X4_ASM(KFMI_X4_G2) : KFMI_X4_OUT : KFMI_X4_IN : "memory", "scc");
#undef KFMI_X4_PREV_L
#undef KFMI_X4_PREV_R
  }
  const v4u ra = needR ? r0 : l0, rb = needR ? r1 : l1;
  kl.bm[0] = l0.x; kl.bm[1] = l0.y; kl.bm[2] = l0.z; kl.bm[3] = l0.w;
  kl.bm[4] = l1.x; kl.bm[5] = l1.y; kl.bm[6] = l1.z; kl.bm[7] = l1.w;
  kr.bm[0] = ra.x; kr.bm[1] = ra.y; kr.bm[2] = ra.z; kr.bm[3] = ra.w;
  kr.bm[4] = rb.x; kr.bm[5] = rb.y; kr.bm[6] = rb.z; kr.bm[7] = rb.w;
  kl.cnt = cl;
  kr.cnt = needR ? cr : cl;
  kl.b = bl;
  kr.b = br;
  kl.e = wl.e;
  kr.e = wr.e;
  kl.prev = wl.prev;
  kr.prev = wr.prev;
}
#undef KFMI_X4_BODY
#undef KFMI_X4_G1
#undef KFMI_X4_G2
#undef KFMI_X4_ASM
#undef KFMI_X4_OUT
#undef KFMI_X4_IN
#undef KFMI_X4_OUTP
#undef KFMI_X4_INP
#undef KFMI_X4_SJ
#undef KFMI_X4_SL
#undef KFMI_X4_PREV_L_ON
#undef KFMI_X4_PREV_R_ON

template <class G, int QPT, int SPLIT>
__device__ __forceinline__ void fetch_ends_split(const IdxArgs& ix, const uint32_t (&L)[QPT],
                                                 const uint32_t (&R)[QPT], const uint32_t (&c)[QPT],
                                                 Blk<G> (&kl)[QPT], Blk<G> (&kr)[QPT])
{
  static_assert(SPLIT == 1 || SPLIT == 4 || ((SPLIT == 7 || SPLIT == 8) && QPT == 1 && X4<G>::OK),
                "fetch form: 1 / 4 (C++ fetch), 7 / 8 (asm fetch, X4 geometries)");
  if constexpr (SPLIT >= 7) {
    fetch_ends_x4<G, SPLIT>(ix, L[0], R[0], c[0], kl[0], kr[0]);
  } else if constexpr (SPLIT == 1) {
    fetch_ends<G, QPT>(ix, L, R, c, kl, kr);
  } else {
    const int grp = (int) (threadIdx.x & 63) / 16;
#pragma unroll
    for (int g = 0; g < 4; ++g)
      if (grp == g) fetch_ends<G, QPT>(ix, L, R, c, kl, kr);
  }
}

struct NoTrace {
  static constexpr bool ON = false;
  struct Out {};
  static Out from(uint4*) { return Out{}; }
  __device__ static Out at(Out, uint64_t) { return Out{}; }
};
struct Trace {
  static constexpr bool ON = true;
  typedef uint4* Out;
  static Out from(uint4* t) { return t; }
  __device__ static Out at(Out t, uint64_t q) { return t + q; }
};

template <class G, int MAXW, int SPLIT, bool JUMP = false, class TR = NoTrace>
__device__ __forceinline__ void skip_walk(const IdxArgs& ix, const uint32_t (&cw)[MAXW], uint32_t steps, uint32_t pos,
                                          uint32_t& Lq, uint32_t& Rq, typename TR::Out tr = typename TR::Out{})
{
  static_assert(G::K <= 2 && MAXW > 0, "skip table: fused task kernels at K <= 2");
  [[maybe_unused]] uint32_t tr_walk = 0, tr_jump = 0, tr_line = 0;
  [[maybe_unused]] const uint32_t tr_start = pos;
  extern __shared__ __attribute__((aligned(16))) uint8_t stage[];
  const uint32_t lane = threadIdx.x & 63u, wv = threadIdx.x >> 6;
  uint32_t* cl = reinterpret_cast<uint32_t*>(stage) + wv * (64u * MAXW) + lane;
#pragma unroll
  for (int k = 0; k < MAXW; ++k) cl[64 * k] = cw[k];
  const uint32_t J = ix.skip_steps;
  const int grp = (int) lane / 16;
  uint32_t L[1] = {Lq}, R[1] = {Rq};
  bool dead = false;
  uint32_t fl = 0;
  auto is_dead = [&]() -> bool {
    if constexpr (JUMP) return (fl & 1u) != 0u;
    else return dead;
  };
  while (__ballot(pos < steps)) {
    const bool act = pos < steps;
    const uint32_t bit = pos * (2u * G::K), k = bit >> 5;
    const uint32_t lo = k < (uint32_t) MAXW ? cl[64u * k] : 0u;
    const uint32_t hi = k + 1u < (uint32_t) MAXW ? cl[64u * (k + 1u)] : 0u;
    const uint32_t code = __builtin_amdgcn_alignbit(hi, lo, bit & 31u);
    const bool row1 = act && R[0] == L[0] + 1u;
    bool jmp = false;
    uint32_t p = SKIP_NONE;
    if constexpr (JUMP) {
      jmp = row1 && !(fl & 2u) && L[0] < ix.bwtsize && (steps - pos) * (uint32_t) G::K >= ix.jump_min;
      if (ix.jump_split & JUMP_SPLIT4) {
#pragma unroll
        for (int g = 0; g < 4; ++g)
          if (jmp && grp == g) p = ix.jsa[L[0]];
      } else if (jmp) {
        p = ix.jsa[L[0]];
      }
    }
    const bool one = row1 && !jmp && !is_dead() && L[0] < ix.skip_rows && pos + J <= steps;
    uint2 e = make_uint2(SKIP_NONE, 0u);
    if (ix.skip_split == 4u) {
#pragma unroll
      for (int g = 0; g < 4; ++g)
        if (one && grp == g) e = ix.skip[L[0]];
    } else if (one) {
      e = ix.skip[L[0]];
    }
    if (act && !one && !jmp) {
      uint32_t c[1] = {code & (uint32_t) (G::NC - 1)};
      uint32_t sx[2 * G::K];
      plane_xor<G::K>(c[0], sx);
      if constexpr (G::SMALL) {
        Blk<G> kl[1], kr[1];
        fetch_ends_split<G, 1, SPLIT>(ix, L, R, c, kl, kr);
        L[0] = lf_from_block<G>(ix, kl[0], L[0], c[0], sx);
        R[0] = lf_from_block<G>(ix, kr[0], R[0], c[0], sx);
      } else {
        L[0] = lf_stream<G>(ix, L[0], c[0], sx);
        R[0] = lf_stream<G>(ix, R[0], c[0], sx);
      }
      ++pos;
      if constexpr (TR::ON) tr_walk += KFMI_TRACE_STEP;
    }
    if (one) {
      if (e.x != SKIP_NONE && e.y == code) {
        L[0] = e.x;
        R[0] = e.x + 1u;
        pos += J;
        if constexpr (TR::ON) tr_walk += KFMI_TRACE_SKIP_HIT;
      } else {
        if constexpr (JUMP) fl |= 1u;
        else dead = true;
        if constexpr (TR::ON) tr_walk += KFMI_TRACE_SKIP_MISS;
      }
    }
    if constexpr (JUMP) {
      if (__ballot(jmp)) {
        const uint32_t nb = (steps - pos) * (uint32_t) G::K;
        const bool ok = jmp && p < ix.bwtsize && p >= nb;
        const uint32_t q = ok ? p - nb : 0u;
        const uint32_t off = ok ? ix.bwtsize - 1u - p : 0u;
        uint32_t tsh = (off & 15u) * 2u;
        const uint32_t nw = ok ? (nb + 15u) >> 4 : 0u;
        const uint32_t* tp = ix.jsa + (2ull * ix.bwtsize + (off >> 4));
        const uint32_t* ip = ix.jsa + ((uint64_t) ix.bwtsize + q);
        uint32_t lim = ok ? nw + 1u : 0u;
        if (ok && (ix.jump_split & JUMP_LINES) && nb <= JUMP_LINE_W) {
          const JumpLineAt at = jump_line_at(ix.bwtsize - 1u, p, nb);
          const uint32_t* lb = ix.jsa + jump_lines_off(ix.bwtsize);
          tp = lb + at.text_dw;
          ip = lb + at.isa_dw;
          tsh = at.shift;
          lim = at.ndw;
          if constexpr (TR::ON) tr_line = KFMI_TRACE_JUMP_LINE;
        }
        uint32_t tx[MAXW + 1];
#pragma unroll
        for (int j = 0; j <= MAXW; ++j) tx[j] = 0u;
        uint32_t r = SKIP_NONE;
        if (ix.jump_split & JUMP_LINES_GROUPED) {
#pragma unroll
          for (int g = 0; g < 4; ++g)
            if (ok && grp == g) {
#pragma unroll
              for (int j = 0; j <= MAXW; ++j)
                if ((uint32_t) j < lim) tx[j] = tp[j];
              r = *ip;
            }
        } else {
#pragma unroll
          for (int j = 0; j <= MAXW; ++j)
            if ((uint32_t) j < lim) tx[j] = tp[j];
          if (ix.jump_split & JUMP_SPLIT4) {
#pragma unroll
            for (int g = 0; g < 4; ++g)
              if (ok && grp == g) r = *ip;
          } else if (ok) {
            r = *ip;
          }
        }
        uint32_t diff = 0u;
#pragma unroll
        for (int j = 0; j < MAXW; ++j) {
          if ((uint32_t) j < nw) {
            const uint32_t kj = k + (uint32_t) j;
            const uint32_t rl = kj < (uint32_t) MAXW ? cl[64u * kj] : 0u;
            const uint32_t rh = kj + 1u < (uint32_t) MAXW ? cl[64u * (kj + 1u)] : 0u;
            const uint32_t rw = __builtin_amdgcn_alignbit(rh, rl, bit & 31u);
            const uint32_t tv = __builtin_amdgcn_alignbit(tx[j + 1], tx[j], tsh);
            const uint32_t left = 2u * nb - 32u * (uint32_t) j;
            diff |= (rw ^ tv) & (left >= 32u ? 0xFFFFFFFFu : (1u << left) - 1u);
          }
        }
        if constexpr (TR::ON) {
          if (jmp) {
            const uint32_t out = !ok ? KFMI_TRACE_JUMP_REFUSED
                                     : (diff != 0u ? KFMI_TRACE_JUMP_DIFFERED
                                                   : (r < ix.bwtsize ? KFMI_TRACE_JUMP_TAKEN : KFMI_TRACE_JUMP_BAD_ISA));
            tr_jump = KFMI_TRACE_JUMP_TRIED | tr_line | (out << KFMI_TRACE_JUMP_OUT_SHIFT) |
                      (pos << KFMI_TRACE_JUMP_POS_SHIFT) | (nb << KFMI_TRACE_JUMP_NB_SHIFT);
          }
        }
        if (ok && diff == 0u && r < ix.bwtsize) {
          L[0] = r;
          R[0] = r + 1u;
          pos = steps;
        } else if (jmp) {
          fl |= 2u;
        }
      }
    }
  }
  Lq = L[0];
  Rq = R[0];
  if constexpr (TR::ON) *tr = make_uint4(tr_walk, tr_jump, tr_start, ix.jump_split);
}

template <class G, int MAXW, int SPLIT>
__device__ __forceinline__ void seed_walk(const IdxArgs& ix, const uint32_t (&cw)[MAXW], uint32_t steps, uint32_t mk,
                                          uint32_t Lq, uint32_t Rq, uint32_t e, uint32_t S, uint2* __restrict__ iv,
                                          uint2* __restrict__ sp)
{
  static_assert(G::K <= 2 && MAXW > 0, "seed search: task kernels at K <= 2");
  extern __shared__ __attribute__((aligned(16))) uint8_t stage[];
  const uint32_t lane = threadIdx.x & 63u, wv = threadIdx.x >> 6;
  uint32_t* cl = reinterpret_cast<uint32_t*>(stage) + wv * (64u * MAXW) + lane;
#pragma unroll
  for (int k = 0; k < MAXW; ++k) cl[64 * k] = cw[k];
  const uint32_t J = ix.skip_steps, F = ix.ftab ? ix.ftab_steps : 0u;
  const int grp = (int) lane / 16;
  uint32_t L[1] = {Lq}, R[1] = {Rq};
  uint32_t pos = 0, cnt = 0;
  bool dead = false;
  while (__ballot(pos < steps && cnt < S)) {
    const bool act = pos < steps && cnt < S;
    const uint32_t bit = pos * (2u * G::K), k = bit >> 5;
    const uint32_t lo = k < (uint32_t) MAXW ? cl[64u * k] : 0u;
    const uint32_t hi = k + 1u < (uint32_t) MAXW ? cl[64u * (k + 1u)] : 0u;
    const uint32_t code = __builtin_amdgcn_alignbit(hi, lo, bit & 31u);
    const uint32_t b = mk - (uint32_t) G::K * pos;
    const bool fresh = e == b;
    const bool jump = act && !dead && fresh && F != 0u && pos + F <= steps;
    const bool one = act && !dead && !fresh && R[0] == L[0] + 1u && L[0] < ix.skip_rows && pos + J <= steps;
    const bool look = one || jump;
    const uint2* tp = one ? ix.skip + L[0] : ix.ftab + (jump ? code & ix.ftab_mask : 0u);
    uint2 te = make_uint2(SKIP_NONE, 0u);
    if (ix.skip_split == 4u) {
#pragma unroll
      for (int g = 0; g < 4; ++g)
        if (look && grp == g) te = *tp;
    } else if (look) {
      te = *tp;
    }
    if (act && !look) {
      const uint32_t pL = L[0], pR = R[0];
      uint32_t c[1] = {code & (uint32_t) (G::NC - 1)};
      uint32_t sx[2 * G::K];
      plane_xor<G::K>(c[0], sx);
      if constexpr (G::SMALL) {
        Blk<G> kl[1], kr[1];
        fetch_ends_split<G, 1, SPLIT>(ix, L, R, c, kl, kr);
        L[0] = lf_from_block<G>(ix, kl[0], L[0], c[0], sx);
        R[0] = lf_from_block<G>(ix, kr[0], R[0], c[0], sx);
      } else {
        L[0] = lf_stream<G>(ix, L[0], c[0], sx);
        R[0] = lf_stream<G>(ix, R[0], c[0], sx);
      }
      if (R[0] <= L[0]) {
        if (fresh) {
          ++pos;
          e = b - (uint32_t) G::K;
        } else {
          iv[cnt] = make_uint2(pL, pR);
          sp[cnt] = make_uint2(b, e - b);
          ++cnt;
          e = b;
        }
        L[0] = 0u;
        R[0] = ix.bwtsize;
        dead = false;
      } else {
        ++pos;
      }
    }
    if (one) {
      if (te.x != SKIP_NONE && te.y == code) {
        L[0] = te.x;
        R[0] = te.x + 1u;
        pos += J;
      } else {
        dead = true;
      }
    } else if (jump) {
      if (te.y > te.x) {
        L[0] = te.x;
        R[0] = te.y;
        pos += F;
      } else {
        dead = true;
      }
    }
  }
  const uint32_t b = mk - (uint32_t) G::K * pos;
  if (cnt < S && e != b) {
    iv[cnt] = make_uint2(L[0], R[0]);
    sp[cnt] = make_uint2(b, e - b);
    ++cnt;
  }
  for (; cnt < S; ++cnt) {
    iv[cnt] = make_uint2(0u, 0u);
    sp[cnt] = make_uint2(0u, 0u);
  }
}

template <class G, int QPT, int MAXW, int SPLIT = 1, bool SKIP = false, bool JUMP = false, class TR = NoTrace>
__global__ __launch_bounds__(256) void task_kernel(IdxArgs ix, const uint32_t* __restrict__ qp,
                                                   const uint8_t* __restrict__ ascii, uint32_t m, uint64_t num,
                                                   uint32_t steps, uint32_t nwords, uint32_t* __restrict__ res,
                                                   typename TR::Out trace)
{
  static_assert(!TR::ON || SKIP, "walk trace: skip_walk's hooks");
  constexpr int SPW = G::SPW;
  constexpr int CW = MAXW > 0 ? (G::K == 3 ? k3_words<(MAXW > 0 ? MAXW : 1)>() : MAXW) : 1;
  static_assert(MAXW == 0 || QPT == 1, "fused packing: one query per thread");
  static_assert(!SKIP || (MAXW > 0 && G::K <= 2), "skip table: fused task kernels at K <= 2");
  static_assert(!JUMP || (SKIP && (G::LAY == LAY_INTER || G::LAY == LAY_MID)), "text jump: skip_walk, plain layouts");
  const uint64_t base = (uint64_t) blockIdx.x * (256 * QPT) + threadIdx.x;
  uint32_t cw[QPT][CW];
  uint32_t rc = 0;
  if constexpr (MAXW > 0) {
    extern __shared__ __attribute__((aligned(16))) uint8_t stage[];
    if constexpr (G::K == 3) {
      uint32_t raw[MAXW];
      stage_query_codes<MAXW>(ascii, num, m, stage, raw, ix.rem, rc);
      recut30<MAXW>(raw, cw[0]);
    } else {
      stage_query_codes<MAXW>(ascii, num, m, stage, cw[0], ix.rem, rc);
    }
  }
  if (base >= num) return;
  uint64_t q[QPT];
  uint32_t L[QPT], R[QPT];
#pragma unroll
  for (int i = 0; i < QPT; ++i) {
    q[i] = base + (uint64_t) i * 256;
    if (q[i] >= num) q[i] = base;
    L[i] = 0;
    R[i] = ix.bwtsize;
  }
  uint32_t skip = 0;
  if (ix.ftab && steps >= ix.ftab_steps) {
    skip = ix.ftab_steps;
#pragma unroll
    for (int i = 0; i < QPT; ++i) {
      uint32_t w0;
      if constexpr (MAXW > 0) w0 = cw[i][0];
      else w0 = qp[q[i]];
      const uint2 lr = ix.ftab[w0 & ix.ftab_mask];
      L[i] = lr.x;
      R[i] = lr.y;
    }
  }
  if (ix.rem) {
#pragma unroll
    for (int i = 0; i < QPT; ++i) {
      const uint2 lr = ix.rtab[MAXW > 0 ? rc : qp[(uint64_t) nwords * num + q[i]]];
      L[i] = lr.x;
      R[i] = lr.y;
    }
  }
  if constexpr (SKIP) {
    skip_walk<G, MAXW, SPLIT, JUMP, TR>(ix, cw[0], steps, skip, L[0], R[0], TR::at(trace, base));
    *reinterpret_cast<uint2*>(res + 2 * base) = make_uint2(L[0], R[0]);
    return;
  }
  for (uint32_t w = 0; w < nwords; ++w) {
    uint32_t word[QPT];
#pragma unroll
    for (int i = 0; i < QPT; ++i) {
      if constexpr (MAXW > 0) {
        word[i] = cw[i][0];
#pragma unroll
        for (int k = 0; k + 1 < CW; ++k) cw[i][k] = cw[i][k + 1];
      } else {
        word[i] = qp[(uint64_t) w * num + q[i]];
      }
    }
    const uint32_t left = steps - w * SPW;
#pragma unroll
    for (int j = 0; j < SPW; ++j) {
      if ((uint32_t) j >= left) continue;
      if (w * SPW + j < skip) continue;
      uint32_t c[QPT];
#pragma unroll
      for (int i = 0; i < QPT; ++i) c[i] = (word[i] >> (2 * G::K * j)) & (uint32_t) (G::NC - 1);
      if constexpr (G::SMALL) {
        Blk<G> kl[QPT], kr[QPT];
        fetch_ends_split<G, QPT, SPLIT>(ix, L, R, c, kl, kr);
#pragma unroll
        for (int i = 0; i < QPT; ++i) {
          uint32_t sx[2 * G::K];
          plane_xor<G::K>(c[i], sx);
          L[i] = lf_from_block<G>(ix, kl[i], L[i], c[i], sx);
          R[i] = lf_from_block<G>(ix, kr[i], R[i], c[i], sx);
        }
      } else {
#pragma unroll
        for (int i = 0; i < QPT; ++i) {
          uint32_t sx[2 * G::K];
          plane_xor<G::K>(c[i], sx);
          L[i] = lf_stream<G>(ix, L[i], c[i], sx);
          R[i] = lf_stream<G>(ix, R[i], c[i], sx);
        }
      }
    }
  }
#pragma unroll
  for (int i = 0; i < QPT; ++i) {
    const uint64_t qi = base + (uint64_t) i * 256;
    if (qi < num) *reinterpret_cast<uint2*>(res + 2 * qi) = make_uint2(L[i], R[i]);
  }
}

template <class G, int MAXW, int SPLIT>
__global__ __launch_bounds__(256) void task_words_skip_kernel(IdxArgs ix, const uint32_t* __restrict__ qp, uint64_t num,
                                                              uint32_t steps, uint32_t nwords,
                                                              uint32_t* __restrict__ res)
{
  static_assert(G::K <= 2 && MAXW > 0, "skip table: task kernels at K <= 2");
  const uint64_t q = (uint64_t) blockIdx.x * 256 + threadIdx.x;
  if (q >= num) return;
  uint32_t cw[MAXW];
#pragma unroll
  for (int k = 0; k < MAXW; ++k) cw[k] = (uint32_t) k < nwords ? qp[(uint64_t) k * num + q] : 0u;
  uint32_t L = 0, R = ix.bwtsize, skip = 0;
  if (ix.ftab && steps >= ix.ftab_steps) {
    skip = ix.ftab_steps;
    const uint2 lr = ix.ftab[cw[0] & ix.ftab_mask];
    L = lr.x;
    R = lr.y;
  }
  if (ix.rem) {
    const uint2 lr = ix.rtab[qp[(uint64_t) nwords * num + q]];
    L = lr.x;
    R = lr.y;
  }
  skip_walk<G, MAXW, SPLIT>(ix, cw, steps, skip, L, R);
  *reinterpret_cast<uint2*>(res + 2 * q) = make_uint2(L, R);
}

template <int MAXW>
__device__ __forceinline__ void stage_strand_codes(const uint8_t* __restrict__ ascii, uint64_t num, uint32_t m,
                                                   uint8_t* __restrict__ lds, uint32_t (&cw)[MAXW], uint32_t strands)
{
  const uint32_t lane = threadIdx.x & 63u, wv = threadIdx.x >> 6;
  const uint32_t both = strands == 3u ? 1u : 0u;
  const uint32_t rpr = stage_rows(m);
  const uint32_t lr = lane >> both;
  const bool rev = both ? (lane & 1u) != 0u : true;
  uint8_t* wl = lds + wv * stage_slot_bytes(m);
  const uint64_t q0 = ((uint64_t) blockIdx.x * 256 + wv * 64) >> both;
#pragma unroll 1
  for (uint32_t h = 0; h < (64u >> both) / rpr; ++h) {
    const uint64_t r0 = q0 + h * rpr;
    const uint64_t nr = r0 < num ? (num - r0 < rpr ? num - r0 : rpr) : 0;
    const uint32_t n16 = (uint32_t) ((nr * m + 15) / 16);
    const uint4* src = reinterpret_cast<const uint4*>(ascii + r0 * m);
    for (uint32_t i = lane; i < n16; i += 64) reinterpret_cast<uint4*>(wl)[i] = src[i];
    __syncthreads();
    if (lr / rpr == h) {
      uint32_t fw[MAXW], rv[MAXW];
      row_codes<MAXW>(wl, (uint64_t) (lr % rpr) * m, m, fw);
      reverse_stream<MAXW>(fw, m, rv);
#pragma unroll
      for (int k = 0; k < MAXW; ++k) cw[k] = rev ? rv[k] : fw[k];
    }
    __syncthreads();
  }
}

template <class G, int MAXW, int SPLIT>
__global__ __launch_bounds__(256) void task_strands_kernel(IdxArgs ix, const uint8_t* __restrict__ ascii, uint32_t m,
                                                           uint64_t num, uint32_t steps, uint32_t strands,
                                                           uint32_t* __restrict__ res)
{
  static_assert(G::K <= 2 && MAXW > 0, "strand staging: task kernels at K <= 2");
  extern __shared__ __attribute__((aligned(16))) uint8_t stage[];
  uint32_t cw[MAXW];
  stage_strand_codes<MAXW>(ascii, num, m, stage, cw, strands);
  const uint64_t t = (uint64_t) blockIdx.x * 256 + threadIdx.x;
  if (t >= (strands == 3u ? 2u : 1u) * num) return;
  uint32_t L = 0, R = ix.bwtsize, skip = 0;
  if (ix.ftab && steps >= ix.ftab_steps) {
    skip = ix.ftab_steps;
    const uint2 lr = ix.ftab[cw[0] & ix.ftab_mask];
    L = lr.x;
    R = lr.y;
  }
  skip_walk<G, MAXW, SPLIT>(ix, cw, steps, skip, L, R);
  *reinterpret_cast<uint2*>(res + 2 * t) = make_uint2(L, R);
}

template <class G, int MAXW, int SPLIT>
__device__ __forceinline__ void seed_task(const IdxArgs& ix, const uint32_t (&cw)[MAXW], uint32_t rc, uint32_t m,
                                          uint32_t steps, uint64_t t, uint32_t S, uint32_t* __restrict__ res,
                                          uint32_t* __restrict__ spans)
{
  const uint32_t mk = m - ix.rem;
  uint32_t L = 0, R = ix.bwtsize, e = mk;
  if (ix.rem) {
    const uint2 lr = ix.rtab[rc];
    if (lr.y > lr.x) {
      L = lr.x;
      R = lr.y;
      e = m;
    }
  }
  seed_walk<G, MAXW, SPLIT>(ix, cw, steps, mk, L, R, e, S, reinterpret_cast<uint2*>(res) + t * S,
                            reinterpret_cast<uint2*>(spans) + t * S);
}

template <class G, int MAXW, int SPLIT>
__global__ __launch_bounds__(256) void seed_kernel(IdxArgs ix, const uint8_t* __restrict__ ascii, uint32_t m,
                                                   uint64_t num, uint32_t steps, uint32_t S,
                                                   uint32_t* __restrict__ res, uint32_t* __restrict__ spans)
{
  extern __shared__ __attribute__((aligned(16))) uint8_t stage[];
  uint32_t cw[MAXW];
  uint32_t rc = 0;
  stage_query_codes<MAXW>(ascii, num, m, stage, cw, ix.rem, rc);
  const uint64_t t = (uint64_t) blockIdx.x * 256 + threadIdx.x;
  if (t >= num) return;
  seed_task<G, MAXW, SPLIT>(ix, cw, rc, m, steps, t, S, res, spans);
}

template <class G, int MAXW, int SPLIT>
__global__ __launch_bounds__(256) void seed_strands_kernel(IdxArgs ix, const uint8_t* __restrict__ ascii, uint32_t m,
                                                           uint64_t num, uint32_t steps, uint32_t strands, uint32_t S,
                                                           uint32_t* __restrict__ res, uint32_t* __restrict__ spans)
{
  extern __shared__ __attribute__((aligned(16))) uint8_t stage[];
  uint32_t cw[MAXW];
  stage_strand_codes<MAXW>(ascii, num, m, stage, cw, strands);
  const uint64_t t = (uint64_t) blockIdx.x * 256 + threadIdx.x;
  if (t >= (strands == 3u ? 2u : 1u) * num) return;
  seed_task<G, MAXW, SPLIT>(ix, cw, 0u, m, steps, t, S, res, spans);
}

template <class G, int MAXW, int SPLIT>
__global__ __launch_bounds__(256) void seed_words_kernel(IdxArgs ix, const uint32_t* __restrict__ qp, uint32_t m,
                                                         uint64_t num, uint32_t steps, uint32_t nwords, uint32_t S,
                                                         uint32_t* __restrict__ res, uint32_t* __restrict__ spans)
{
  const uint64_t t = (uint64_t) blockIdx.x * 256 + threadIdx.x;
  if (t >= num) return;
  uint32_t cw[MAXW];
#pragma unroll
  for (int k = 0; k < MAXW; ++k) cw[k] = (uint32_t) k < nwords ? qp[(uint64_t) k * num + t] : 0u;
  const uint32_t rc = ix.rem ? qp[(uint64_t) nwords * num + t] & ((1u << (2u * ix.rem)) - 1u) : 0u;
  seed_task<G, MAXW, SPLIT>(ix, cw, rc, m, steps, t, S, res, spans);
}

template <class G>
__global__ __launch_bounds__(256) void ftab_level_kernel(IdxArgs ix, uint32_t t, uint64_t parents, uint2* out)
{
  for (uint64_t v = (uint64_t) blockIdx.x * 256 + threadIdx.x; v < parents; v += (uint64_t) gridDim.x * 256) {
    uint2 lr = make_uint2(0u, ix.bwtsize);
    if (t) lr = out[v];
#pragma unroll 1
    for (uint32_t c = 0; c < (uint32_t) G::NC; ++c) {
      uint32_t sx[2 * G::K];
      plane_xor<G::K>(c, sx);
      const uint32_t L = lf_stream<G>(ix, lr.x, c, sx);
      const uint32_t R = lf_stream<G>(ix, lr.y, c, sx);
      out[v | ((uint64_t) c << (2 * G::K * t))] = make_uint2(L, R);
    }
  }
}

template <class G>
__global__ __launch_bounds__(256) void skip_level0_kernel(IdxArgs ix, uint64_t rows, uint2* __restrict__ out)
{
  for (uint64_t i = (uint64_t) blockIdx.x * 256 + threadIdx.x; i < rows; i += (uint64_t) gridDim.x * 256) {
    const uint32_t X = (uint32_t) i;
    const uint32_t c = row_code<G>(ix, X);
    uint32_t sx[2 * G::K];
    plane_xor<G::K>(c, sx);
    const uint32_t L = lf_stream<G>(ix, X, c, sx);
    const uint32_t R = lf_stream<G>(ix, X + 1u, c, sx);
    bool ok = R == L + 1u && (uint64_t) L < rows;
#pragma unroll
    for (int s = 0; s < G::K; ++s) ok = ok && ix.dl.dpos[s] != X;
    out[i] = ok ? make_uint2(L, c) : make_uint2(SKIP_NONE, 0u);
  }
}

template <class G>
__global__ __launch_bounds__(256) void jump_text_kernel(IdxArgs ix, const uint32_t* __restrict__ isa, uint64_t n,
                                                        uint64_t words, uint32_t split, uint32_t* __restrict__ out)
{
  const int grp = (int) (threadIdx.x & 63) / 16;
  for (uint64_t w0 = (uint64_t) blockIdx.x * 256 + (threadIdx.x & ~63u); w0 < words; w0 += (uint64_t) gridDim.x * 256) {
    const uint64_t w = w0 + (threadIdx.x & 63u);
    uint32_t v = 0;
#pragma unroll 1
    for (uint32_t u = 0; u < 16u / (uint32_t) G::K; ++u) {
      const uint64_t back = 16ull * w + (uint64_t) u * G::K;
      const bool on = w < words && back < n;
      const uint64_t p = on ? n - back : 0;
      const uint32_t row = on ? isa[p] : 0u;
      const bool ok = on && row < ix.bwtsize;
      uint32_t c = 0;
      if (split) {
#pragma unroll
        for (int g = 0; g < 4; ++g)
          if (ok && grp == g) c = row_code<G>(ix, row);
      } else if (ok) {
        c = row_code<G>(ix, row);
      }
      if (p < (uint64_t) G::K) c &= (1u << (2u * (uint32_t) p)) - 1u;
      v |= c << (2u * (uint32_t) G::K * u);
    }
    if (w < words) out[w] = v;
  }
}

template <class G>
__global__ __launch_bounds__(256) void jump_lines_kernel(const uint32_t* __restrict__ isa, const uint32_t* __restrict__ text,
                                                         uint64_t n, uint64_t words, uint64_t lines,
                                                         uint32_t* __restrict__ out)
{
  const uint64_t total = lines * JUMP_LINE_DW;
  for (uint64_t i = (uint64_t) blockIdx.x * 256 + threadIdx.x; i < total; i += (uint64_t) gridDim.x * 256) {
    const uint64_t j = i / JUMP_LINE_DW;
    const uint32_t t = (uint32_t) (i % JUMP_LINE_DW);
    uint32_t v;
    if (t < JUMP_LINE_TEXT) {
      const uint64_t e = j * JUMP_LINE_S + t;
      v = e <= n ? isa[n - e] : SKIP_NONE;
    } else {
      const uint64_t w = j + t;
      v = w >= JUMP_LINE_DW - 1 && w - (JUMP_LINE_DW - 1) < words ? text[w - (JUMP_LINE_DW - 1)] : 0u;
    }
    out[i] = v;
  }
}

template <class G>
__global__ __launch_bounds__(64) void rem_tab_kernel(IdxArgs ix, uint32_t rem, uint2* __restrict__ out)
{
  const uint32_t x = threadIdx.x;
  if (rem == 0 || rem >= (uint32_t) G::K || x >= (1u << (2 * rem))) return;
  const uint32_t pad = 2 * ((uint32_t) G::K - rem);
  const uint32_t cA = x << pad, cT = cA | ((1u << pad) - 1u);
  uint32_t sx[2 * G::K];
  plane_xor<G::K>(cA, sx);
  uint32_t L = lf_stream<G>(ix, 0u, cA, sx);
  plane_xor<G::K>(cT, sx);
  const uint32_t R = lf_stream<G>(ix, ix.bwtsize, cT, sx);
  const uint32_t n = ix.bwtsize - 1u;
  const uint32_t tail = row_code<G>(ix, 0u);
  for (uint32_t j = 0; j + rem < (uint32_t) G::K; ++j)
    if (j + rem <= n && (tail & ((1u << (2 * j)) - 1u)) == 0u && ((tail >> (2 * j)) & ((1u << (2 * rem)) - 1u)) == x)
      --L;
  out[x] = make_uint2(L, R);
}

template <class G>
__global__ __launch_bounds__(256) void count_blocks_kernel(IdxArgs ix, const uint32_t* __restrict__ qp, uint64_t num,
                                                           uint32_t steps, uint32_t nwords,
                                                           unsigned long long* __restrict__ total)
{
  const uint64_t q = (uint64_t) blockIdx.x * 256 + threadIdx.x;
  uint32_t cnt = 0;
  if (q < num) {
    uint32_t L = 0, R = ix.bwtsize;
    if (ix.rem) {
      const uint2 lr = ix.rtab[qp[(uint64_t) nwords * num + q]];
      L = lr.x;
      R = lr.y;
    }
    for (uint32_t t = 0; t < steps; ++t) {
      const uint32_t word = qp[(uint64_t) (t / G::SPW) * num + q];
      const uint32_t c = (word >> (2 * G::K * (t % G::SPW))) & (uint32_t) (G::NC - 1);
      uint32_t sx[2 * G::K];
      plane_xor<G::K>(c, sx);
      cnt += (L / (uint32_t) G::D == R / (uint32_t) G::D) ? 1u : 2u;
      L = lf_stream<G>(ix, L, c, sx);
      R = lf_stream<G>(ix, R, c, sx);
    }
  }
  for (int off = 32; off > 0; off >>= 1) cnt += __shfl_xor(cnt, off);
  if ((threadIdx.x & 63) == 0) atomicAdd(total, (unsigned long long) cnt);
}

template <class G>
__global__ __launch_bounds__(256) void lf_next_kernel(IdxArgs ix, uint64_t rows, uint32_t* __restrict__ next,
                                                      uint32_t* __restrict__ bad)
{
  for (uint64_t i = (uint64_t) blockIdx.x * 256 + threadIdx.x; i < rows; i += (uint64_t) gridDim.x * 256) {
    const uint32_t X = (uint32_t) i;
    bool dollar = false;
#pragma unroll
    for (int s = 0; s < G::K; ++s) dollar = dollar || ix.dl.dpos[s] == X;
    uint32_t j = X;
    if (!dollar) {
      j = lf_row<G>(ix, X);
      if ((uint64_t) j >= rows) {
        atomicOr(bad, 1u);
        j = X;
      }
    }
    next[i] = j;
  }
}

template <class G>
__global__ __launch_bounds__(256) void derive_codes_kernel(IdxArgs ix, uint64_t rows, uint8_t* __restrict__ codes,
                                                           uint32_t* __restrict__ isa)
{
  for (uint64_t i = (uint64_t) blockIdx.x * 256 + threadIdx.x; i < rows; i += (uint64_t) gridDim.x * 256) {
    const uint32_t X = (uint32_t) i;
    const uint32_t c = row_code<G>(ix, X);
    bool dollar = false;
#pragma unroll
    for (int s = 0; s < G::K; ++s) dollar = dollar || ix.dl.dpos[s] == X;
    uint32_t up = 0;
    if (!dollar) {
      uint32_t sx[2 * G::K];
      plane_xor<G::K>(c, sx);
      const uint32_t j = lf_stream<G>(ix, X, c, sx);
      up = row_code<G>(ix, j);
#pragma unroll
      for (int s = 0; s < G::K; ++s)
        if (ix.dl.dpos[s] == j) isa[s] = X;
    }
    codes[i] = (uint8_t) (c | (up << (2 * G::K)));
  }
}

template <class G>
__device__ __forceinline__ int lf_lines(const IdxArgs& ix, uint32_t X, uint32_t c, uint64_t* ln, uint32_t* extra,
                                        uint32_t* prev)
{
  const uint32_t b = X / (uint32_t) G::D;
  Where<G> w = locate<G>(ix, b, c);
  line_local_prev<G>(ix, b, c, w);
  int n = 0;
  const uint64_t p0 = (uint64_t) (uintptr_t) w.planes >> 7, p1 = (uint64_t) (uintptr_t) (w.planes + G::BMW - 1) >> 7;
  ln[n++] = p0;
  if (p1 != p0) ln[n++] = p1;
  const uint64_t cl = (uint64_t) (uintptr_t) w.cnt >> 7;
  *extra = (cl != p0 && cl != p1) ? 1u : 0u;
  if (*extra) ln[n++] = cl;
  *prev = w.prev ? 1u : 0u;
  if (w.prev) {
    const uint64_t q0 = (uint64_t) (uintptr_t) w.pplanes >> 7, q1 = (uint64_t) (uintptr_t) (w.pplanes + G::BMW - 1) >> 7;
    if (q0 != p0 && q0 != p1) ln[n++] = q0;
    if (q1 != q0 && q1 != p0 && q1 != p1) ln[n++] = q1;
  }
  return n;
}

template <class G>
__global__ __launch_bounds__(256) void count_lines_kernel(IdxArgs ix, const uint32_t* __restrict__ qp, uint64_t num,
                                                          uint32_t steps, uint32_t nwords,
                                                          unsigned long long* __restrict__ out)
{
  const uint64_t q = (uint64_t) blockIdx.x * 256 + threadIdx.x;
  uint32_t lines = 0, extra = 0, ends = 0, prevs = 0;
  if (q < num) {
    uint32_t L = 0, R = ix.bwtsize;
    if (ix.rem) {
      const uint2 lr = ix.rtab[qp[(uint64_t) nwords * num + q]];
      L = lr.x;
      R = lr.y;
    }
    for (uint32_t t = 0; t < steps; ++t) {
      const uint32_t word = qp[(uint64_t) (t / G::SPW) * num + q];
      const uint32_t c = (word >> (2 * G::K * (t % G::SPW))) & (uint32_t) (G::NC - 1);
      uint64_t ln[10];
      uint32_t ex, pv;
      int n = lf_lines<G>(ix, L, c, ln, &ex, &pv);
      extra += ex;
      prevs += pv;
      ++ends;
      if (R / (uint32_t) G::D != L / (uint32_t) G::D) {
        n += lf_lines<G>(ix, R, c, ln + n, &ex, &pv);
        extra += ex;
        prevs += pv;
        ++ends;
      }
      for (int i = 0; i < n; ++i) {
        bool dup = false;
        for (int j = 0; j < i; ++j) dup = dup || ln[j] == ln[i];
        lines += dup ? 0u : 1u;
      }
      uint32_t sx[2 * G::K];
      plane_xor<G::K>(c, sx);
      L = lf_stream<G>(ix, L, c, sx);
      R = lf_stream<G>(ix, R, c, sx);
    }
  }
  for (int off = 32; off > 0; off >>= 1) {
    lines += __shfl_xor(lines, off);
    extra += __shfl_xor(extra, off);
    ends += __shfl_xor(ends, off);
    prevs += __shfl_xor(prevs, off);
  }
  if ((threadIdx.x & 63) == 0) {
    atomicAdd(out + 0, (unsigned long long) lines);
    atomicAdd(out + 1, (unsigned long long) extra);
    atomicAdd(out + 2, (unsigned long long) ends);
    atomicAdd(out + 3, (unsigned long long) prevs);
  }
}


struct SearchLaunch {
  hipStream_t st;
  IdxArgs ix;
  const uint32_t* qp;
  const uint8_t* ascii;
  uint32_t m;
  int maxw;
  int words_maxw;
  uint32_t strands;
  uint64_t num;
  uint32_t steps, nwords;
  uint32_t* res;
  uint32_t* spans;
  uint32_t max_seeds;
  const uint32_t* sa;
  uint32_t sa_log2;
  const uint64_t* off;
  const uint32_t* owner;
  uint64_t total;
  uint32_t* pos;
  unsigned long long* slot_ctr;
  uint32_t slot_chunk;
  uint2* ftab_out;
  uint32_t ftab_steps;
  uint64_t ftab_n;
  uint32_t rem;
  uint2* skip_out;
  uint8_t* derive_codes;
  uint32_t* derive_isa;
  uint32_t* perm_next;
  uint32_t* perm_bad;
  const uint32_t* jump_isa;
  uint32_t* jump_text;
  uint64_t jump_words;
  uint32_t jump_split;
  uint32_t* jump_lines;
  uint4* trace;
};

template <class G, int SPLIT, class TR = NoTrace>
static void launch_task_split(const SearchLaunch& a)
{
  constexpr bool TRACED = G::K <= 2 && (G::LAY == LAY_INTER || G::LAY == LAY_MID);
  static_assert(!TR::ON || TRACED, "walk trace: fused forward task kernels, plain layouts, K <= 2");
  const typename TR::Out tr = TR::from(a.trace);
  if (a.maxw) {
    const size_t lds = 4 * (size_t) stage_slot_bytes(a.m);
    if constexpr (G::K <= 2 && !TR::ON) {
      if (a.strands) {
        const uint64_t tblocks = ((a.strands == 3u ? 2u : 1u) * a.num + 255) / 256;
        const size_t lds_str = std::max(lds, (size_t) 4 * 64 * 4 * (size_t) a.maxw);
        if (a.maxw == 8)
          hipLaunchKernelGGL((task_strands_kernel<G, 8, SPLIT>), dim3((uint32_t) tblocks), dim3(256), lds_str, a.st,
                             a.ix, a.ascii, a.m, a.num, a.steps, a.strands, a.res);
        else
          hipLaunchKernelGGL((task_strands_kernel<G, 16, SPLIT>), dim3((uint32_t) tblocks), dim3(256), lds_str, a.st,
                             a.ix, a.ascii, a.m, a.num, a.steps, a.strands, a.res);
        return;
      }
    }
    const uint64_t blocks = (a.num + 255) / 256;
    if constexpr (G::K <= 2) {
      if (TR::ON || a.ix.skip || a.ix.jsa) {
        const size_t lds_skip = std::max(lds, (size_t) 4 * 64 * 4 * (size_t) a.maxw);
        if constexpr (G::LAY == LAY_INTER || G::LAY == LAY_MID) {
          if (a.ix.jsa) {
            IdxArgs ix = a.ix;
            if ((ix.jump_split & JUMP_LINES_GROUPED) && a.m > JUMP_LINES_GROUPED_MAX_M)
              ix.jump_split &= ~(JUMP_LINES | JUMP_LINES_GROUPED);
            if (a.maxw == 8)
              hipLaunchKernelGGL((task_kernel<G, 1, 8, SPLIT, true, true, TR>), dim3((uint32_t) blocks), dim3(256),
                                 lds_skip, a.st, ix, a.qp, a.ascii, a.m, a.num, a.steps, a.nwords, a.res, tr);
            else
              hipLaunchKernelGGL((task_kernel<G, 1, 16, SPLIT, true, true, TR>), dim3((uint32_t) blocks), dim3(256),
                                 lds_skip, a.st, ix, a.qp, a.ascii, a.m, a.num, a.steps, a.nwords, a.res, tr);
            return;
          }
        }
        if (a.maxw == 8)
          hipLaunchKernelGGL((task_kernel<G, 1, 8, SPLIT, true, false, TR>), dim3((uint32_t) blocks), dim3(256), lds_skip,
                             a.st, a.ix, a.qp, a.ascii, a.m, a.num, a.steps, a.nwords, a.res, tr);
        else
          hipLaunchKernelGGL((task_kernel<G, 1, 16, SPLIT, true, false, TR>), dim3((uint32_t) blocks), dim3(256), lds_skip,
                             a.st, a.ix, a.qp, a.ascii, a.m, a.num, a.steps, a.nwords, a.res, tr);
        return;
      }
    }
    if constexpr (!TR::ON) {
      if (a.maxw == 8)
        hipLaunchKernelGGL((task_kernel<G, 1, 8, SPLIT>), dim3((uint32_t) blocks), dim3(256), lds, a.st, a.ix, a.qp,
                           a.ascii, a.m, a.num, a.steps, a.nwords, a.res, tr);
      else
        hipLaunchKernelGGL((task_kernel<G, 1, 16, SPLIT>), dim3((uint32_t) blocks), dim3(256), lds, a.st, a.ix, a.qp,
                           a.ascii, a.m, a.num, a.steps, a.nwords, a.res, tr);
    }
  } else if constexpr (!TR::ON) {
    const uint64_t blocks = (a.num + 255) / 256;
    if constexpr (G::K <= 2) {
      if (a.ix.skip && a.words_maxw) {
        const size_t lds_skip = (size_t) 4 * 64 * 4 * (size_t) a.words_maxw;
        if (a.words_maxw == 8)
          hipLaunchKernelGGL((task_words_skip_kernel<G, 8, SPLIT>), dim3((uint32_t) blocks), dim3(256), lds_skip, a.st,
                             a.ix, a.qp, a.num, a.steps, a.nwords, a.res);
        else
          hipLaunchKernelGGL((task_words_skip_kernel<G, 16, SPLIT>), dim3((uint32_t) blocks), dim3(256), lds_skip,
                             a.st, a.ix, a.qp, a.num, a.steps, a.nwords, a.res);
        return;
      }
    }
    hipLaunchKernelGGL((task_kernel<G, 1, 0, SPLIT>), dim3((uint32_t) blocks), dim3(256), 0, a.st, a.ix, a.qp,
                       a.ascii, a.m, a.num, a.steps, a.nwords, a.res, tr);
  }
}

template <class G, class TR = NoTrace>
static hipError_t launch_task(const SearchLaunch& a)
{
  if constexpr (G::SMALL) {
    const uint32_t want = a.ix.split;
    if constexpr (X4<G>::OK) {
      if (want == 1) launch_task_split<G, 8, TR>(a);
      else launch_task_split<G, 7, TR>(a);
      return hipGetLastError();
    }
    const int mw = a.maxw ? a.maxw : (a.ix.skip ? a.words_maxw : 0);
    if (want == 4 || (want == 2 && mw == 8)) {
      launch_task_split<G, 4, TR>(a);
      return hipGetLastError();
    }
  }
  launch_task_split<G, 1, TR>(a);
  return hipGetLastError();
}

template <class G, int SPLIT>
static void launch_seeds_split(const SearchLaunch& a)
{
#define KFMI_SEED_MAXW(MW, KERNEL, GRID, LDS, ...)                                                           \
  do {                                                                                                       \
    if ((MW) == 8)                                                                                           \
      hipLaunchKernelGGL((KERNEL<G, 8, SPLIT>), dim3((uint32_t) (GRID)), dim3(256), LDS, a.st, __VA_ARGS__); \
    else                                                                                                     \
      hipLaunchKernelGGL((KERNEL<G, 16, SPLIT>), dim3((uint32_t) (GRID)), dim3(256), LDS, a.st, __VA_ARGS__); \
  } while (0)
  if (a.maxw) {
    const size_t lds = std::max((size_t) 4 * stage_slot_bytes(a.m), (size_t) 4 * 64 * 4 * (size_t) a.maxw);
    if (a.strands) {
      const uint64_t tblocks = ((a.strands == 3u ? 2u : 1u) * a.num + 255) / 256;
      KFMI_SEED_MAXW(a.maxw, seed_strands_kernel, tblocks, lds, a.ix, a.ascii, a.m, a.num, a.steps, a.strands,
                     a.max_seeds, a.res, a.spans);
    } else {
      KFMI_SEED_MAXW(a.maxw, seed_kernel, (a.num + 255) / 256, lds, a.ix, a.ascii, a.m, a.num, a.steps, a.max_seeds,
                     a.res, a.spans);
    }
  } else {
    const size_t lds = (size_t) 4 * 64 * 4 * (size_t) a.words_maxw;
    KFMI_SEED_MAXW(a.words_maxw, seed_words_kernel, (a.num + 255) / 256, lds, a.ix, a.qp, a.m, a.num, a.steps,
                   a.nwords, a.max_seeds, a.res, a.spans);
  }
#undef KFMI_SEED_MAXW
}

template <class G>
static hipError_t launch_seeds(const SearchLaunch& a)
{
  if constexpr (G::K <= 2 && (G::LAY == LAY_INTER || G::LAY == LAY_MID)) {
    const int mw = a.maxw ? a.maxw : a.words_maxw;
    if (mw != 8 && mw != 16) return hipErrorInvalidValue;
    const uint32_t want = a.ix.split;
    if constexpr (G::SMALL && X4<G>::OK) {
      if (want == 1) launch_seeds_split<G, 8>(a);
      else launch_seeds_split<G, 7>(a);
    } else if constexpr (G::SMALL) {
      if (want == 4 || (want == 2 && mw == 8)) launch_seeds_split<G, 4>(a);
      else launch_seeds_split<G, 1>(a);
    } else {
      launch_seeds_split<G, 1>(a);
    }
    return hipGetLastError();
  } else {
    return hipErrorInvalidValue;
  }
}

template <class G>
static hipError_t launch_coop(const SearchLaunch& a)
{
  return coop_launch<G>(a.st, a.ix, a.qp, a.ascii, a.m, a.maxw, a.num, a.steps, a.nwords, a.res);
}

template <class G>
static hipError_t launch_count(const SearchLaunch& a, unsigned long long* d_total)
{
  const uint64_t blocks = (a.num + 255) / 256;
  hipLaunchKernelGGL((count_blocks_kernel<G>), dim3((uint32_t) blocks), dim3(256), 0, a.st, a.ix, a.qp, a.num,
                     a.steps, a.nwords, d_total);
  return hipGetLastError();
}


#define KFMI_FOR_NB(X, K, LAY) \
  X(K, 1, LAY) X(K, 2, LAY) X(K, 4, LAY) X(K, 6, LAY) X(K, 8, LAY) X(K, 14, LAY) X(K, 30, LAY)


template <class G>
static hipError_t launch_locate(const SearchLaunch& a)
{
  int dev = 0, cus = 256;
  if (hipGetDevice(&dev) != hipSuccess ||
      hipDeviceGetAttribute(&cus, hipDeviceAttributeMultiprocessorCount, dev) != hipSuccess || cus < 1)
    cus = 256;
  uint64_t blocks = (a.total + 255) / 256;
  if constexpr (locate_coop_ok<G>()) {
    static const bool coop = [] {
      const char* e = getenv("KFMI_LOCATE_COOP");
      return !e || atoi(e) != 0;
    }();
    if (coop) {
      hipLaunchKernelGGL((locate_coop_kernel<G>), dim3(grid_blocks(blocks, (uint64_t) cus * 5)), dim3(256), 0, a.st, a.ix,
                         a.sa, a.sa_log2,
                         a.owner, a.total, a.pos, a.slot_ctr, a.slot_chunk);
      return hipGetLastError();
    }
  }
  hipLaunchKernelGGL((locate_kernel<G>), dim3(grid_blocks(blocks, (uint64_t) cus * 8)), dim3(256), 0, a.st, a.ix, a.sa,
                     a.sa_log2, a.owner, a.total, a.pos);
  return hipGetLastError();
}

template <class G>
static hipError_t launch_ftab(const SearchLaunch& a)
{
  uint64_t parents = 1;
  for (uint32_t t = 0; t < a.ftab_steps; ++t, parents <<= 2 * G::K) {
    if ((parents << (2 * G::K)) > a.ftab_n) return hipErrorInvalidValue;
    const uint64_t blocks = (parents + 255) / 256;
    hipLaunchKernelGGL((ftab_level_kernel<G>), dim3(grid_blocks(blocks, 1u << 20)), dim3(256), 0, a.st, a.ix, t,
                       parents, a.ftab_out);
    const hipError_t e = hipGetLastError();
    if (e != hipSuccess) return e;
  }
  return hipSuccess;
}

template <class G>
static hipError_t launch_rem_tab(const SearchLaunch& a)
{
  hipLaunchKernelGGL((rem_tab_kernel<G>), dim3(1), dim3(64), 0, a.st, a.ix, a.rem, a.ftab_out);
  return hipGetLastError();
}

template <class G>
static hipError_t launch_skip0(const SearchLaunch& a)
{
  if constexpr (G::K <= 2 && G::LAY != LAY_GRP) {
    hipLaunchKernelGGL((skip_level0_kernel<G>), dim3(grid_blocks((a.num + 255) / 256, 1u << 20)), dim3(256), 0, a.st,
                       a.ix, a.num, a.skip_out);
    return hipGetLastError();
  }
  return hipErrorInvalidValue;
}

template <class G>
static hipError_t launch_count_lines(const SearchLaunch& a, unsigned long long* d_out)
{
  const uint64_t blocks = (a.num + 255) / 256;
  hipLaunchKernelGGL((count_lines_kernel<G>), dim3((uint32_t) blocks), dim3(256), 0, a.st, a.ix, a.qp, a.num,
                     a.steps, a.nwords, d_out);
  return hipGetLastError();
}

template <class G>
static hipError_t launch_derive(const SearchLaunch& a)
{
  if constexpr (G::LAY == LAY_INTER && G::K <= 2) {
    hipLaunchKernelGGL((derive_codes_kernel<G>), dim3(grid_blocks((a.num + 255) / 256, 65536)), dim3(256), 0, a.st,
                       a.ix, a.num, a.derive_codes, a.derive_isa);
    return hipGetLastError();
  }
  return hipErrorInvalidValue;
}

template <class G>
static hipError_t launch_perm(const SearchLaunch& a)
{
  hipLaunchKernelGGL((lf_next_kernel<G>), dim3(grid_blocks((a.num + 255) / 256, 65536)), dim3(256), 0, a.st, a.ix,
                     a.num, a.perm_next, a.perm_bad);
  return hipGetLastError();
}

template <class G>
static hipError_t launch_jump_text(const SearchLaunch& a)
{
  if constexpr (G::K <= 2 && (G::LAY == LAY_INTER || G::LAY == LAY_MID)) {
    hipLaunchKernelGGL((jump_text_kernel<G>), dim3(grid_blocks((a.jump_words + 255) / 256, 1u << 20)), dim3(256), 0, a.st,
                       a.ix, a.jump_isa, a.num, a.jump_words, a.jump_split, a.jump_text);
    return hipGetLastError();
  }
  return hipErrorInvalidValue;
}

template <class G>
static hipError_t launch_jump_lines(const SearchLaunch& a)
{
  if constexpr (G::K <= 2 && (G::LAY == LAY_INTER || G::LAY == LAY_MID)) {
    const uint64_t lines = jump_line_count(a.num);
    hipLaunchKernelGGL((jump_lines_kernel<G>), dim3(grid_blocks((lines * JUMP_LINE_DW + 255) / 256, 1u << 20)), dim3(256), 0,
                       a.st, a.jump_isa, a.jump_text, a.num, a.jump_words, lines, a.jump_lines);
    return hipGetLastError();
  }
  return hipErrorInvalidValue;
}

enum class Op { Task, Coop, Count, Locate, Ftab, RemTab, CountLines, Derive, PermCheck, Skip0, JumpText, JumpLines, Trace };

template <int K, int NB, int LAY>
hipError_t dispatch_one(Op op, const SearchLaunch& a, unsigned long long* d_total)
{
  using G = Geo<K, NB, LAY>;
  switch (op) {
    case Op::Task: return launch_task<G>(a);
    case Op::Coop: return launch_coop<G>(a);
    case Op::Locate: return launch_locate<G>(a);
    case Op::Ftab: return launch_ftab<G>(a);
    case Op::RemTab: return launch_rem_tab<G>(a);
    case Op::CountLines: return launch_count_lines<G>(a, d_total);
    case Op::Derive: return launch_derive<G>(a);
    case Op::PermCheck: return launch_perm<G>(a);
    case Op::Skip0: return launch_skip0<G>(a);
    case Op::JumpText: return launch_jump_text<G>(a);
    case Op::JumpLines: return launch_jump_lines<G>(a);
    case Op::Trace: return hipErrorInvalidValue;
    default: return launch_count<G>(a, d_total);
  }
}

#define KFMI_INSTANTIATE(KK, NBV, LAYV) \
  template hipError_t dispatch_one<KK, NBV, LAYV>(Op, const SearchLaunch&, unsigned long long*);
#define KFMI_EXTERN(KK, NBV, LAYV) \
  extern template hipError_t dispatch_one<KK, NBV, LAYV>(Op, const SearchLaunch&, unsigned long long*);

template <int K, int NB, int LAY>
hipError_t seeds_one(const SearchLaunch& a)
{
  return launch_seeds<Geo<K, NB, LAY>>(a);
}

#define KFMI_SEEDS_INSTANTIATE(KK, NBV, LAYV) template hipError_t seeds_one<KK, NBV, LAYV>(const SearchLaunch&);
#define KFMI_SEEDS_EXTERN(KK, NBV, LAYV) extern template hipError_t seeds_one<KK, NBV, LAYV>(const SearchLaunch&);

template <int K, int NB, int LAY>
hipError_t trace_one(const SearchLaunch& a)
{
  if (!a.trace || !a.maxw || a.strands) return hipErrorInvalidValue;
  return launch_task<Geo<K, NB, LAY>, Trace>(a);
}

#define KFMI_TRACE_INSTANTIATE(KK, NBV, LAYV) template hipError_t trace_one<KK, NBV, LAYV>(const SearchLaunch&);
#define KFMI_TRACE_EXTERN(KK, NBV, LAYV) extern template hipError_t trace_one<KK, NBV, LAYV>(const SearchLaunch&);

}

#endif
```

### k-step_fm-index_amd/csrc/hip/kfmi_runtime.h

```cpp
#ifndef KFMI_RUNTIME_H_
#define KFMI_RUNTIME_H_

#include <hip/hip_runtime.h>
#include <atomic>
#include <stdint.h>
#include <stdio.h>
#include <mutex>
#include <shared_mutex>
#include <pthread.h>

#include "../kfmi_internal.h"
#include "kfmi_devguard.h"
#include "kfmi_kernels.h"

#define HIP_OK(x)                                                                   \
  do {                                                                              \
    hipError_t _e = (x);                                                            \
    if (_e != hipSuccess) {                                                         \
      fprintf(stderr, "kstepfmi: %s failed: %s (%s:%d)\n", #x, hipGetErrorString(_e), \
              __FILE__, __LINE__);                                                  \
      return KFMI_E_KERNEL;                                                         \
    }                                                                               \
  } while (0)


struct kfmi_dev_index {
  int device = -1;
  int backend = -1;
  int layout = -1;
  uint32_t K = 0, d = 0, nb = 0, bwtsize = 0, nentries = 0;
  kfmi::DollarArgs dl{};
  uint32_t* ent = nullptr;
  uint64_t ent_bytes = 0;
  uint32_t* sa = nullptr;
  std::atomic<int> lf_perm{-1};
  uint64_t sa_bytes = 0;
  uint32_t sa_log2 = 0, sa_gen = 0;
  uint2* ftab[17] = {};
  std::mutex ftab_mu;
  int ftab_auto = -1;
  uint2* skip = nullptr;
  int skip_auto = -1;
  uint32_t* jump_sa = nullptr;
  int jump_auto = -1;
  int jump_none = 0;
  uint2* rtab[4] = {};
  uint32_t* ac_tail = nullptr;
  uint32_t ac_tail_b0 = 0xFFFFFFFFu;
};

struct kfmi_dev_queries {
  int device = -1;
  uint8_t* ascii = nullptr;
  uint32_t* packed = nullptr;
  uint64_t num = 0;
  uint32_t size = 0, K = 0, steps = 0, nwords = 0, rem = 0;
  uint32_t packed_rows = 0;
  uint32_t* strand_words = nullptr;
  uint64_t strand_cap = 0;
};

namespace kfmi {

struct RwLock {
  pthread_rwlock_t rw;
  void lock() { pthread_rwlock_wrlock(&rw); }
  void unlock() { pthread_rwlock_unlock(&rw); }
  bool try_lock() { return pthread_rwlock_trywrlock(&rw) == 0; }
  void lock_shared() { pthread_rwlock_rdlock(&rw); }
  void unlock_shared() { pthread_rwlock_unlock(&rw); }
  bool try_lock_shared() { return pthread_rwlock_tryrdlock(&rw) == 0; }
};
RwLock& index_lock(const void* f);

struct DevCtx {
  bool init = false;
  hipStream_t st = nullptr;
  std::mutex up_mu;
  void* up_buf[2] = {nullptr, nullptr};
  hipEvent_t up_ev[2] = {nullptr, nullptr};
  uint64_t up_cap = 0;
};
void release_upload_staging();
hipError_t upload_staging(DevCtx* ctx, uint64_t need);
int32_t ctx_for(int dev, DevCtx** out);
hipEvent_t* thread_events(int dev);
struct SearchLane {
  DevCtx* ctx = nullptr;
  hipStream_t st = nullptr;
  hipEvent_t* ev = nullptr;
};
int32_t search_lane(int dev, SearchLane* lane);

extern thread_local int t_device;
extern thread_local int32_t t_last_error;
extern thread_local double t_ms[3];

bool is_coop(int backend);
int backend_for(uint32_t K);
int fused_maxw(int backend, uint32_t bases);
int32_t check_lf_walks(kfmi_dev_index* di, hipStream_t st);
hipError_t dispatch(Op op, uint32_t K, uint32_t nb, int lay, const SearchLaunch& a,
                    unsigned long long* d_total = nullptr);
IdxArgs idx_args(const kfmi_dev_index* di);
uint32_t split_for(uint64_t table_bytes, int layout);
hipError_t launch_pack(const kfmi_dev_queries* dq, hipStream_t st);

struct TableWants {
  uint32_t ftab = 0, skip = 0, jump = 0;
  TableWants no_jump() const { return TableWants{ftab, skip, 0u}; }
};
TableWants tables_wanted(void);
int32_t use_tables(kfmi_dev_index* di, hipStream_t st, IdxArgs& ix, const TableWants& w, uint32_t rem);
int32_t auto_tables(kfmi_dev_index* di, hipStream_t st, const TableWants& w);
void drop_ftabs(kfmi_dev_index* di);
uint64_t table_budget_now(void);
bool rem_supported(int layout);
uint64_t sum_members(void* index, uint64_t (*of)(kfmi_dev_index*));
int32_t member_index(const kfmi_fmi_t* f, uint32_t member, kfmi_dev_index** di);
int32_t auto_jump(kfmi_dev_index* di, hipStream_t st);
int32_t use_jump(kfmi_dev_index* di, hipStream_t st, IdxArgs& ix, uint32_t want);
void free_jump(kfmi_dev_index* di);

int32_t upload_index(kfmi_fmi_t* f, int backend, int dev, DevCtx* ctx, kfmi_dev_index** out = nullptr);
int32_t derive_index(kfmi_fmi_t* f, uint32_t k_out, int dev, bool host_image, kfmi_fmi_t** out);
uint32_t device_steps(const kfmi_fmi_t* f);
int32_t upload_sa(const kfmi_fmi_t* f, kfmi_dev_index* di, DevCtx* ctx);
int32_t upload_queries(kfmi_qrys_t* q, uint32_t K, int dev, DevCtx* ctx);
void query_geometry(kfmi_dev_queries* dq, uint32_t K);
void free_dev_index(kfmi_dev_index* di);
void free_dev_queries(kfmi_dev_queries* dq);
hipError_t h2d(void* dst, const void* src, uint64_t bytes, hipStream_t st);

int32_t search_enqueue(kfmi_dev_index* di, kfmi_dev_queries* dq, uint32_t* d_res, hipStream_t st, hipEvent_t* ev,
                       const TableWants& want, uint4* trace = nullptr);
int32_t search_finish(hipStream_t st, hipEvent_t* ev, double* ms);

int32_t strand_reserve(kfmi_dev_queries* dq, uint64_t cq, DevCtx* ctx);
int strand_words_maxw(uint32_t nwords);
int strand_fused_maxw(const kfmi_dev_index* di, bool ascii, uint32_t K, uint32_t steps, uint32_t rem);
hipError_t launch_strand_pack(const kfmi_dev_queries* dq, uint32_t* out, uint32_t strands, bool from_words,
                              hipStream_t st);

bool host_pinned(const void* p);
void par_copy(void* dst, const void* src, uint64_t bytes);
void par_pack(const char* src, uint64_t n, uint32_t size, uint32_t rem, uint32_t* out);
bool par_pread(int fd, void* dst, uint64_t off, uint64_t bytes);

constexpr int KFMI_MAX_GROUP = 16;
struct GroupIndex {
  int n = 0, backend = -1;
  int dev[KFMI_MAX_GROUP] = {};
  kfmi_dev_index* di[KFMI_MAX_GROUP] = {};
  hipStream_t st[KFMI_MAX_GROUP] = {};
  hipEvent_t ev[KFMI_MAX_GROUP][3] = {};
};

struct GroupSlices {
  int n = 0;
  int dev[KFMI_MAX_GROUP] = {};
  uint64_t q0[KFMI_MAX_GROUP] = {}, num[KFMI_MAX_GROUP] = {};
  kfmi_dev_queries* dq[KFMI_MAX_GROUP] = {};
  uint32_t* d_res[KFMI_MAX_GROUP] = {};
};
int group_devices(int* devs);
int32_t group_transfer(kfmi_fmi_t* f, kfmi_qrys_t* q, kfmi_res_t* r, const int* devs, int n);
int32_t group_search(kfmi_fmi_t* f, kfmi_qrys_t* q, kfmi_res_t* r);
int32_t group_to_host(kfmi_res_t* r);
void group_free_index(kfmi_fmi_t* f);
void group_free_queries(kfmi_qrys_t* q);
void group_free_results(kfmi_res_t* r);

}

#endif
```

### k-step_fm-index_amd/csrc/hip/kfmi_tables.hip

```cpp
#include <hip/hip_runtime.h>
#include <stdint.h>
#include <stdlib.h>
#include <string.h>
#include <atomic>
#include <mutex>
#include <shared_mutex>

#include "../kfmi_internal.h"
#include "kfmi_device.h"
#include "kfmi_runtime.h"

namespace kfmi {

static thread_local int t_ftab = -1;
static thread_local int t_skip = -1;
static thread_local int t_jump = -1;

extern "C" int32_t kfmi_set_ftab(uint32_t bases)
{
  if (bases > 16 && bases != KFMI_FTAB_AUTO) return KFMI_E_BAD_ARGUMENT;
  t_ftab = bases == KFMI_FTAB_AUTO ? -2 : (int) bases;
  return KFMI_SUCCESS;
}

static uint32_t ftab_bases(void)
{
  if (t_ftab >= 0) return (uint32_t) t_ftab;
  if (t_ftab == -2) return KFMI_FTAB_AUTO;
  static const uint32_t env = [] {
    const char* e = getenv("KFMI_FTAB");
    if (!e || !*e || !strcmp(e, "auto")) return (uint32_t) KFMI_FTAB_AUTO;
    const int v = atoi(e);
    return v > 0 && v <= 16 ? (uint32_t) v : 0u;
  }();
  return env;
}

extern "C" uint32_t kfmi_ftab_auto_bases(uint64_t rows, uint32_t K, uint64_t budget_bytes)
{
  if (K < 1 || K > 4 || rows < 8) return 0;
  uint32_t n = 16 - 16 % K;
  while (n && (1ull << (2 * n)) > 2 * rows) n -= K;
  while (n && (8ull << (2 * n)) > budget_bytes) n -= K;
  return n;
}

static int mode_from_env(const char* name)
{
  const char* e = getenv(name);
  if (!e || !*e || !strcmp(e, "auto")) return 2;
  return atoi(e) ? 1 : 0;
}

extern "C" int32_t kfmi_set_skip(uint32_t mode)
{
  if (mode > 1 && mode != KFMI_SKIP_AUTO) return KFMI_E_BAD_ARGUMENT;
  t_skip = mode == KFMI_SKIP_AUTO ? 2 : (int) mode;
  return KFMI_SUCCESS;
}

static uint32_t skip_wanted(void)
{
  int v = t_skip;
  if (v < 0) {
    static const int env = mode_from_env("KFMI_SKIP");
    v = env;
  }
  if (v == 2) return ftab_bases() == KFMI_FTAB_AUTO ? 2u : 0u;
  return (uint32_t) v;
}

extern "C" uint32_t kfmi_skip_in_effect(void) { return skip_wanted(); }

extern "C" uint32_t kfmi_skip_auto(uint64_t rows, uint32_t K, uint64_t budget_bytes)
{
  if (K < 1 || K > 2 || rows < 8 || rows > 0xFFFFFFFFull) return 0;
  return 16 * rows <= budget_bytes ? 1u : 0u;
}

extern "C" int32_t kfmi_set_jump(uint32_t mode)
{
  if (mode > 1 && mode != KFMI_JUMP_AUTO) return KFMI_E_BAD_ARGUMENT;
  t_jump = mode == KFMI_JUMP_AUTO ? 2 : (int) mode;
  return KFMI_SUCCESS;
}

static uint32_t jump_wanted(void)
{
  int v = t_jump;
  if (v < 0) {
    static const int env = mode_from_env("KFMI_JUMP");
    v = env;
  }
  if (v == 2) return skip_wanted() == 2u ? 2u : 0u;
  return (uint32_t) v;
}

extern "C" uint32_t kfmi_jump_in_effect(void) { return jump_wanted(); }

TableWants tables_wanted(void) { return TableWants{ftab_bases(), skip_wanted(), jump_wanted()}; }

static std::atomic<uint64_t> g_ftab_budget{KFMI_FTAB_BUDGET_FREE};

extern "C" int32_t kfmi_set_ftab_budget(uint64_t bytes)
{
  g_ftab_budget.store(bytes, std::memory_order_relaxed);
  return KFMI_SUCCESS;
}

uint64_t table_budget_now(void)
{
  const uint64_t budget = g_ftab_budget.load(std::memory_order_relaxed);
  if (budget != KFMI_FTAB_BUDGET_FREE) return budget;
  size_t free_b = 0, total_b = 0;
  if (hipMemGetInfo(&free_b, &total_b) != hipSuccess) {
    (void) hipGetLastError();
    return 0;
  }
  return (uint64_t) free_b / 4;
}

bool rem_supported(int layout)
{
  return layout == LAY_INTER || layout == LAY_MID || layout == LAY_GRP;
}

static int32_t use_rtab(kfmi_dev_index* di, hipStream_t st, IdxArgs& ix, uint32_t rem)
{
  ix.rtab = nullptr;
  ix.rem = 0;
  if (!rem) return KFMI_SUCCESS;
  if (rem >= di->K || rem > 3 || !rem_supported(di->layout)) return KFMI_E_BAD_ARGUMENT;
  {
    std::lock_guard<std::mutex> lk(di->ftab_mu);
    if (!di->rtab[rem]) {
      uint2* t = nullptr;
      if (hipMalloc((void**) &t, 8ull << (2 * rem)) != hipSuccess) return KFMI_E_DEVICE_ALLOC;
      SearchLaunch a{};
      a.st = st;
      a.ix = idx_args(di);
      a.ftab_out = t;
      a.rem = rem;
      if (dispatch(Op::RemTab, di->K, di->nb, di->layout, a) != hipSuccess || hipStreamSynchronize(st) != hipSuccess) {
        (void) hipFree(t);
        return KFMI_E_KERNEL;
      }
      di->rtab[rem] = t;
    }
  }
  ix.rtab = di->rtab[rem];
  ix.rem = rem;
  ix.ftab = nullptr;
  ix.ftab_steps = 0;
  ix.ftab_mask = 0;
  return KFMI_SUCCESS;
}

static int32_t build_ftab(kfmi_dev_index* di, hipStream_t st, uint32_t bases)
{
  uint2* t = nullptr;
  if (hipMalloc((void**) &t, 8ull << (2 * bases)) != hipSuccess) {
    (void) hipGetLastError();
    return KFMI_E_DEVICE_ALLOC;
  }
  SearchLaunch a{};
  a.st = st;
  a.ix = idx_args(di);
  a.ftab_out = t;
  a.ftab_steps = bases / di->K;
  a.ftab_n = 1ull << (2 * bases);
  if (dispatch(Op::Ftab, di->K, di->nb, di->layout, a) != hipSuccess || hipStreamSynchronize(st) != hipSuccess) {
    (void) hipFree(t);
    return KFMI_E_KERNEL;
  }
  di->ftab[bases] = t;
  return KFMI_SUCCESS;
}

static int32_t auto_ftab(kfmi_dev_index* di, hipStream_t st, uint32_t* bases)
{
  std::lock_guard<std::mutex> lk(di->ftab_mu);
  if (di->ftab_auto < 0) {
    uint32_t n = kfmi_ftab_auto_bases(di->bwtsize, di->K, table_budget_now());
    for (; n; n -= di->K) {
      if (di->ftab[n]) break;
      const int32_t e = build_ftab(di, st, n);
      if (!e) break;
      if (e != KFMI_E_DEVICE_ALLOC) return e;
    }
    di->ftab_auto = (int) n;
  }
  if (bases) *bases = (uint32_t) di->ftab_auto;
  return KFMI_SUCCESS;
}

static int32_t use_ftab(kfmi_dev_index* di, hipStream_t st, IdxArgs& ix, uint32_t bases)
{
  ix.ftab = nullptr;
  ix.ftab_steps = 0;
  ix.ftab_mask = 0;
  if (bases == KFMI_FTAB_AUTO) {
    const int32_t e = auto_ftab(di, st, &bases);
    if (e) return e;
  }
  if (!bases || bases % di->K || bases > 16) return KFMI_SUCCESS;
  {
    std::lock_guard<std::mutex> lk(di->ftab_mu);
    if (!di->ftab[bases]) {
      const int32_t e = build_ftab(di, st, bases);
      if (e) return e;
    }
  }
  ix.ftab = di->ftab[bases];
  ix.ftab_steps = bases / di->K;
  ix.ftab_mask = bases >= 16 ? 0xFFFFFFFFu : (1u << (2 * bases)) - 1u;
  return KFMI_SUCCESS;
}

__global__ __launch_bounds__(256) void skip_double_kernel(const uint2* __restrict__ in, uint64_t rows, uint32_t shift,
                                                          uint32_t split, uint2* __restrict__ out)
{
  const int grp = (int) (threadIdx.x & 63) / 16;
  for (uint64_t i = (uint64_t) blockIdx.x * 256 + threadIdx.x; i < rows; i += (uint64_t) gridDim.x * 256) {
    const uint2 a = in[i];
    const bool ok = a.x != SKIP_NONE && (uint64_t) a.x < rows;
    uint2 b = make_uint2(SKIP_NONE, 0u);
    if (split) {
#pragma unroll
      for (int g = 0; g < 4; ++g)
        if (ok && grp == g) b = in[a.x];
    } else if (ok) {
      b = in[a.x];
    }
    out[i] = (ok && b.x != SKIP_NONE) ? make_uint2(b.x, a.y | (b.y << shift)) : make_uint2(SKIP_NONE, 0u);
  }
}

static int32_t build_skip(kfmi_dev_index* di, hipStream_t st)
{
  const uint64_t rows = di->bwtsize;
  uint2* buf[2] = {nullptr, nullptr};
  for (uint2*& b : buf)
    if (hipMalloc((void**) &b, 8ull * rows) != hipSuccess) {
      (void) hipGetLastError();
      if (buf[0]) (void) hipFree(buf[0]);
      return KFMI_E_DEVICE_ALLOC;
    }
  SearchLaunch a{};
  a.st = st;
  a.ix = idx_args(di);
  a.num = rows;
  a.skip_out = buf[0];
  bool ok = dispatch(Op::Skip0, di->K, di->nb, di->layout, a) == hipSuccess;
  const uint32_t J = 16u / di->K;
  const uint32_t split = split_for(8ull * rows, LAY_INTER) == 4u ? 1u : 0u;
  int cur = 0;
  for (uint32_t s = 1; ok && s < J; s *= 2, cur ^= 1) {
    hipLaunchKernelGGL(skip_double_kernel, dim3(grid_blocks((rows + 255) / 256, 1u << 20)), dim3(256), 0, st, buf[cur],
                       rows, 2u * di->K * s, split, buf[cur ^ 1]);
    ok = hipGetLastError() == hipSuccess;
  }
  ok = hipStreamSynchronize(st) == hipSuccess && ok;
  (void) hipFree(buf[cur ^ 1]);
  if (!ok) {
    (void) hipFree(buf[cur]);
    return KFMI_E_KERNEL;
  }
  di->skip = buf[cur];
  return KFMI_SUCCESS;
}

static bool skip_applies(const kfmi_dev_index* di)
{
  return di->K >= 1 && di->K <= 2 && !is_coop(di->backend) && di->layout != LAY_GRP;
}

static int32_t auto_skip(kfmi_dev_index* di, hipStream_t st)
{
  std::lock_guard<std::mutex> lk(di->ftab_mu);
  if (di->skip_auto >= 0 || di->skip) return KFMI_SUCCESS;
  di->skip_auto = 0;
  if (!skip_applies(di)) return KFMI_SUCCESS;
  if (!kfmi_skip_auto(di->bwtsize, di->K, table_budget_now())) return KFMI_SUCCESS;
  const int32_t e = build_skip(di, st);
  if (e && e != KFMI_E_DEVICE_ALLOC) return e;
  di->skip_auto = e ? 0 : 1;
  return KFMI_SUCCESS;
}

static int32_t use_skip(kfmi_dev_index* di, hipStream_t st, IdxArgs& ix, uint32_t want)
{
  ix.skip = nullptr;
  ix.skip_rows = 0;
  ix.skip_steps = 0;
  ix.skip_split = 1;
  if (!want || !skip_applies(di)) return KFMI_SUCCESS;
  if (want == 2) {
    const int32_t e = auto_skip(di, st);
    if (e) return e;
  }
  {
    std::lock_guard<std::mutex> lk(di->ftab_mu);
    if (!di->skip) {
      if (want == 2) return KFMI_SUCCESS;
      const int32_t e = build_skip(di, st);
      if (e) return e;
    }
  }
  ix.skip = di->skip;
  ix.skip_rows = di->bwtsize;
  ix.skip_steps = 16u / di->K;
  ix.skip_split = split_for(8ull * di->bwtsize, LAY_INTER);
  return KFMI_SUCCESS;
}

int32_t use_tables(kfmi_dev_index* di, hipStream_t st, IdxArgs& ix, const TableWants& w, uint32_t rem)
{
  int32_t err = use_ftab(di, st, ix, w.ftab);
  if (!err) err = use_rtab(di, st, ix, rem);
  if (!err) err = use_jump(di, st, ix, w.jump);
  if (!err) err = use_skip(di, st, ix, w.skip);
  return err;
}

int32_t auto_tables(kfmi_dev_index* di, hipStream_t st, const TableWants& w)
{
  int32_t err = KFMI_SUCCESS;
  if (w.ftab == KFMI_FTAB_AUTO) err = auto_ftab(di, st, nullptr);
  if (!err && w.skip == 2u) err = auto_skip(di, st);
  if (!err && w.jump == 2u) err = auto_jump(di, st);
  return err;
}

void drop_ftabs(kfmi_dev_index* di)
{
  if (!di) return;
  std::lock_guard<std::mutex> lk(di->ftab_mu);
  if (di->device >= 0) (void) hipSetDevice(di->device);
  for (uint2*& t : di->ftab)
    if (t) {
      (void) hipFree(t);
      t = nullptr;
    }
  di->ftab_auto = -1;
  if (di->skip) (void) hipFree(di->skip);
  di->skip = nullptr;
  di->skip_auto = -1;
  free_jump(di);
}

uint64_t sum_members(void* index, uint64_t (*of)(kfmi_dev_index*))
{
  kfmi_fmi_t* f = (kfmi_fmi_t*) index;
  if (!f) return 0;
  std::shared_lock<RwLock> lk(index_lock(f));
  uint64_t b = 0;
  if (f->grp) {
    const GroupIndex* g = (const GroupIndex*) f->grp;
    for (int i = 0; i < g->n; ++i) b += of(g->di[i]);
  } else if (f->dev) {
    b = of(f->dev);
  }
  return b;
}

int32_t member_index(const kfmi_fmi_t* f, uint32_t member, kfmi_dev_index** di)
{
  *di = f->dev;
  if (f->grp) {
    const GroupIndex* g = (const GroupIndex*) f->grp;
    if ((int) member >= g->n) return KFMI_E_BAD_ARGUMENT;
    *di = g->di[member];
  } else if (member) {
    return KFMI_E_BAD_ARGUMENT;
  }
  return *di ? KFMI_SUCCESS : KFMI_E_NOT_ON_DEVICE;
}

static uint64_t ftab_bytes_of(kfmi_dev_index* di)
{
  std::lock_guard<std::mutex> lk(di->ftab_mu);
  uint64_t b = 0;
  for (uint32_t n = 1; n <= 16; ++n)
    if (di->ftab[n]) b += 8ull << (2 * n);
  return b;
}

static uint64_t skip_bytes_of(kfmi_dev_index* di)
{
  std::lock_guard<std::mutex> lk(di->ftab_mu);
  return di->skip ? 8ull * di->bwtsize : 0ull;
}

extern "C" uint64_t kfmi_device_ftab_bytes(void* index) { return sum_members(index, ftab_bytes_of); }

extern "C" uint64_t kfmi_device_skip_bytes(void* index) { return sum_members(index, skip_bytes_of); }

extern "C" int32_t kfmi_device_skip_table(void* index, void* out, uint64_t entries, uint32_t* steps)
{
  kfmi_fmi_t* f = (kfmi_fmi_t*) index;
  if (!f || !out) return KFMI_E_BAD_ARGUMENT;
  DeviceGuard dg;
  std::shared_lock<RwLock> lk(index_lock(f));
  kfmi_dev_index* di = nullptr;
  const int32_t e = f->grp ? KFMI_E_NOT_ON_DEVICE : member_index(f, 0, &di);
  if (e) return e;
  std::lock_guard<std::mutex> tl(di->ftab_mu);
  if (!di->skip) return KFMI_E_NOT_ON_DEVICE;
  if (entries != di->bwtsize) return KFMI_E_BAD_ARGUMENT;
  if (hipSetDevice(di->device) != hipSuccess) return KFMI_E_NO_DEVICE;
  HIP_OK(hipMemcpy(out, di->skip, 8ull * entries, hipMemcpyDeviceToHost));
  if (steps) *steps = 16u / di->K;
  return KFMI_SUCCESS;
}

}
```

### k-step_fm-index_amd/kstep_fmi/__init__.py

```python
from __future__ import annotations

import ctypes
import os
import subprocess
from pathlib import Path

import numpy as np

PKG_DIR = Path(__file__).resolve().parent.parent
LIB_PATH = PKG_DIR / "lib" / "libkstepfmi.so"
BIN_DIR = PKG_DIR / "bin"

BACKENDS = ("task", "coop", "task-ac", "coop-ac", "task-mid", "coop-mid", "task-ac-mid", "coop-ac-mid",
            "task-grp", "coop-grp")
BACKEND_TAG = {"task": 101, "coop": 101, "task-ac": 201, "coop-ac": 201, "task-mid": 101, "coop-mid": 101,
               "task-ac-mid": 201, "coop-ac-mid": 201, "task-grp": 101, "coop-grp": 101}

_lib = None


class KfmiError(RuntimeError):
    def __init__(self, code: int, what: str = ""):
        self.code = code
        msg = _lib.errorCommon(code).decode() if _lib is not None else f"error {code}"
        super().__init__(f"{what}: {msg} (code {code})" if what else f"{msg} (code {code})")


def build(jobs: int = 8) -> None:
    subprocess.run(["make", "-C", str(PKG_DIR), f"-j{jobs}"], check=True)


def load() -> ctypes.CDLL:
    global _lib
    if _lib is not None:
        return _lib
    if not LIB_PATH.exists():
        raise FileNotFoundError(f"{LIB_PATH} not built -- run kstep_fmi.build() / make -C {PKG_DIR}")
    L = ctypes.CDLL(str(LIB_PATH), mode=ctypes.RTLD_GLOBAL)
    vp, u32, u64, i32 = ctypes.c_void_p, ctypes.c_uint32, ctypes.c_uint64, ctypes.c_int32
    pvp = ctypes.POINTER(ctypes.c_void_p)
    sig = {
        "loadIndex": (i32, [ctypes.c_char_p, pvp]),
        "saveIndex": (i32, [ctypes.c_char_p, vp]),
        "initResults": (i32, [u32, pvp]),
        "searchIndexGPU": (None, [vp, vp, vp]),
        "freeIndex": (i32, [pvp]),
        "freeReference": (i32, [pvp, pvp]),
        "buildIndex": (i32, [vp, pvp]),
        "freeQueriesGPU": (i32, [pvp]),
        "freeResultsGPU": (i32, [pvp]),
        "freeIndexGPU": (i32, [pvp]),
        "transferGPUtoCPU": (i32, [vp]),
        "transferCPUtoGPU": (i32, [vp, vp, vp]),
        "sampleTime": (ctypes.c_double, []),
        "base2index": (u32, [u32]),
        "loadRef": (i32, [ctypes.c_char_p, u32, pvp]),
        "saveRef": (i32, [ctypes.c_char_p, vp]),
        "loadQueries": (i32, [ctypes.c_char_p, u32, u32, pvp]),
        "writeResults": (i32, [ctypes.c_char_p, ctypes.POINTER(ctypes.c_uint32), u32]),
        "loadResults": (i32, [ctypes.c_char_p, pvp]),
        "freeQueries": (i32, [pvp]),
        "freeResults": (i32, [pvp]),
        "saveResults": (i32, [ctypes.c_char_p, vp, vp]),
        "errorCommon": (ctypes.c_char_p, [i32]),
        "kfmi_set_backend": (i32, [ctypes.c_char_p]),
        "kfmi_get_backend": (ctypes.c_char_p, []),
        "kfmi_set_device": (i32, [i32]),
        "kfmi_device_count": (i32, []),
        "kfmi_device_pci_bus_id": (i32, [i32, ctypes.c_char_p, i32]),
        "kfmi_last_error": (i32, []),
        "kfmi_search": (i32, [vp, vp, vp]),
        "searchIndexCPU": (None, [vp, vp, vp]),
        "kfmi_search_cpu": (i32, [vp, vp, vp, i32]),
        "kfmi_last_timing": (i32, [ctypes.POINTER(ctypes.c_double)] * 3),
        "kfmi_load_index_tag": (i32, [ctypes.c_char_p, u32, pvp]),
        "kfmi_index_from_image": (i32, [vp, u64, pvp]),
        "kfmi_index_image": (i32, [vp, pvp, ctypes.POINTER(ctypes.c_uint64)]),
        "kfmi_index_header": (i32, [vp, vp]),
        "kfmi_transform_interleave": (i32, [vp, pvp]),
        "kfmi_transform_ac": (i32, [vp, pvp, pvp]),
        "kfmi_transform_plain": (i32, [vp, pvp]),
        "kfmi_queries_from_buffer": (i32, [vp, u64, u32, pvp]),
        "kfmi_load_queries_gpu": (i32, [ctypes.c_char_p, u32, u64, pvp]),
        "kfmi_results_alloc": (i32, [u64, pvp]),
        "kfmi_results_host": (ctypes.POINTER(ctypes.c_uint32), [vp]),
        "kfmi_results_num": (u64, [vp]),
        "kfmi_build_index_cpu": (i32, [vp, u64, u32, u32, pvp]),
        "kfmi_build_index_gpu": (i32, [vp, u64, u32, u32, i32, pvp]),
        "kfmi_derive_index_gpu": (i32, [vp, u32, i32, pvp]),
        "kfmi_build_stats": (i32, [ctypes.POINTER(ctypes.c_uint64), ctypes.POINTER(ctypes.c_uint32)]),
        "kfmi_count_blocks": (i32, [vp, vp, ctypes.POINTER(ctypes.c_uint64)]),
        "kfmi_count_lines": (i32, [vp, vp, ctypes.POINTER(ctypes.c_uint64)]),
        "kfmi_probe_replay": (i32, [vp, vp, i32, i32, i32, ctypes.POINTER(ctypes.c_double),
                                    ctypes.POINTER(ctypes.c_uint64), ctypes.POINTER(ctypes.c_uint64)]),
        "kfmi_device_index_bytes": (u64, [vp]),
        "kfmi_search_stream": (i32, [vp, vp, u64, u32, vp, u64]),
        "kfmi_host_alloc": (i32, [u64, pvp]),
        "kfmi_host_threads": (i32, []),
        "kfmi_host_free": (i32, [vp]),
        "kfmi_stream_release": (i32, []),
        "kfmi_stream_hostpacked_fraction": (ctypes.c_double, []),
        "kfmi_pack_queries": (i32, [vp, u64, u32, vp]),
        "kfmi_pack_queries_k": (i32, [vp, u64, u32, u32, vp]),
        "kfmi_queries_upload_form": (i32, [vp]),
        "kfmi_set_devices": (i32, [ctypes.POINTER(ctypes.c_int32), i32]),
        "kfmi_get_devices": (i32, [ctypes.POINTER(ctypes.c_int32), i32]),
        "kfmi_build_index_ex": (i32, [vp, u64, u32, u32, u32, i32, pvp]),
        "kfmi_set_ftab": (i32, [u32]),
        "kfmi_ftab_auto_bases": (u32, [u64, u32, u64]),
        "kfmi_set_ftab_budget": (i32, [u64]),
        "kfmi_device_ftab_bytes": (u64, [vp]),        "kfmi_set_split_class": (i32, [u32]),
        "kfmi_set_skip": (i32, [u32]),
        "kfmi_skip_in_effect": (u32, []),
        "kfmi_skip_auto": (u32, [u64, u32, u64]),
        "kfmi_device_skip_bytes": (u64, [vp]),
        "kfmi_device_skip_table": (i32, [vp, vp, u64, ctypes.POINTER(u32)]),
        "kfmi_set_jump": (i32, [u32]),
        "kfmi_jump_in_effect": (u32, []),
        "kfmi_set_jump_min": (i32, [u32]),
        "kfmi_jump_min": (u32, []),
        "kfmi_jump_auto": (u32, [u64, u32, u64]),
        "kfmi_device_jump_bytes": (u64, [vp]),
        "kfmi_device_jump_tables": (i32, [vp, u32, vp, vp, u64, vp, u64]),
        "kfmi_set_jump_lines": (i32, [u32]),
        "kfmi_jump_lines": (u32, []),
        "kfmi_device_jump_line_bytes": (u64, [vp]),
        "kfmi_device_jump_lines": (i32, [vp, u32, vp, u64]),
        "kfmi_jump_line_geometry": (i32, [u64, u64, u32, ctypes.POINTER(ctypes.c_uint64)]),
        "kfmi_set_fused": (i32, [i32]),
        "kfmi_set_walk_check": (i32, [u32]),
        "kfmi_fail_index_uploads": (i32, [u32]),
        "kfmi_walk_check_last": (i32, []),
        "kfmi_set_alphabet": (i32, [ctypes.c_char_p]),
        "kfmi_index_sa": (i32, [vp, pvp, ctypes.POINTER(ctypes.c_uint64), ctypes.POINTER(ctypes.c_uint32)]),
        "kfmi_save_sa": (i32, [ctypes.c_char_p, vp]),
        "kfmi_load_sa": (i32, [ctypes.c_char_p, vp]),
        "kfmi_locate": (i32, [vp, vp, u32, pvp]),
        "kfmi_locations_total": (u64, [vp]),
        "kfmi_locations_offsets": (vp, [vp]),
        "kfmi_locations_positions": (vp, [vp]),
        "kfmi_locations_free": (i32, [pvp]),
        "kfmi_search_strands": (i32, [vp, vp, vp, u32]),
        "kfmi_search_stream_strands": (i32, [vp, vp, u64, u32, vp, u64, u32]),
        "kfmi_search_cpu_strands": (i32, [vp, vp, vp, u32, i32]),
        "kfmi_revcomp_queries": (i32, [vp, u64, u32, vp]),
        "kfmi_strand_words_host": (i32, [vp, u64, u32, u32, u32, vp]),
        "kfmi_reverse_stream_host": (i32, [vp, u64, u32, u32, vp]),
        "kfmi_search_seeds": (i32, [vp, vp, vp, vp, u32, u32]),
        "kfmi_search_seeds_cpu": (i32, [vp, vp, vp, vp, u32, u32, i32]),
        "kfmi_search_trace": (i32, [vp, vp, vp, vp]),
        "kfmi_results_to_device": (i32, [vp]),
        "kfmi_verify_seeds": (i32, [vp, vp, vp, vp, vp, u32, u32, u32, u32]),
        "kfmi_verify_seeds_cpu": (i32, [vp, u64, vp, u64, vp, vp, vp, vp, u32, u32, u32, u32, i32]),
    }
    for name, (res, args) in sig.items():
        f = getattr(L, name)
        f.restype = res
        f.argtypes = args
    _lib = L
    return L


def exported_symbols():
    load()
    return [n for n in _lib.__dict__ if not n.startswith("_")]


def _check(code: int, what: str) -> None:
    if code:
        raise KfmiError(code, what)


def set_backend(name: str) -> None:
    _check(load().kfmi_set_backend(name.encode()), f"set_backend({name})")


def get_backend() -> str:
    return load().kfmi_get_backend().decode()


FTAB_AUTO = 0xFFFFFFFF


def set_ftab(bases) -> None:
    n = FTAB_AUTO if bases == "auto" else int(bases)
    _check(load().kfmi_set_ftab(n), f"set_ftab({bases})")


def ftab_auto_bases(rows: int, k: int, budget_bytes: int) -> int:
    return int(load().kfmi_ftab_auto_bases(int(rows), int(k), int(budget_bytes)))


def set_ftab_budget(nbytes) -> None:
    _check(load().kfmi_set_ftab_budget(0xFFFFFFFFFFFFFFFF if nbytes is None else int(nbytes)), "set_ftab_budget")


SKIP_AUTO = 0xFFFFFFFF


def set_skip(mode) -> None:
    n = SKIP_AUTO if mode == "auto" else int(mode)
    _check(load().kfmi_set_skip(n), f"set_skip({mode})")


def skip_in_effect() -> int:
    return int(load().kfmi_skip_in_effect())


def skip_auto(rows: int, k: int, budget_bytes: int) -> bool:
    return bool(load().kfmi_skip_auto(int(rows), int(k), int(budget_bytes)))


JUMP_AUTO = 0xFFFFFFFF
JUMP_MIN_DEFAULT = 8


def set_jump(mode) -> None:
    n = JUMP_AUTO if mode == "auto" else int(mode)
    _check(load().kfmi_set_jump(n), f"set_jump({mode})")


def jump_in_effect() -> int:
    return int(load().kfmi_jump_in_effect())


def set_jump_min(bases: int) -> None:
    _check(load().kfmi_set_jump_min(int(bases)), f"set_jump_min({bases})")


def jump_min() -> int:
    return int(load().kfmi_jump_min())


def set_jump_lines(mode: int) -> None:
    _check(load().kfmi_set_jump_lines(int(mode)), f"set_jump_lines({mode})")


def jump_lines() -> int:
    return int(load().kfmi_jump_lines())


def jump_line_geometry(n: int, p: int, nb: int):
    out = (ctypes.c_uint64 * 6)()
    _check(load().kfmi_jump_line_geometry(int(n), int(p), int(nb), out), f"jump_line_geometry({n}, {p}, {nb})")
    return tuple(int(x) for x in out)


def jump_auto(rows: int, k: int, budget_bytes: int) -> bool:
    return bool(load().kfmi_jump_auto(int(rows), int(k), int(budget_bytes)))


def set_split_class(cls: int) -> None:
    _check(load().kfmi_set_split_class(int(cls)), f"set_split_class({cls})")


def set_fused(on: bool) -> None:
    _check(load().kfmi_set_fused(1 if on else 0), f"set_fused({on})")


def fail_index_uploads(n: int) -> None:
    _check(load().kfmi_fail_index_uploads(int(n)), f"fail_index_uploads({n})")


def set_walk_check(mode: int) -> None:
    _check(load().kfmi_set_walk_check(int(mode)), f"set_walk_check({mode})")


def walk_check_last() -> int:
    return int(load().kfmi_walk_check_last())


def set_alphabet(mode: str | None) -> None:
    _check(load().kfmi_set_alphabet(mode.encode() if mode else None), f"set_alphabet({mode})")


def set_device(dev: int) -> None:
    _check(load().kfmi_set_device(int(dev)), f"set_device({dev})")


def set_devices(devs) -> None:
    devs = [int(d) for d in devs]
    arr = (ctypes.c_int32 * max(len(devs), 1))(*devs)
    _check(load().kfmi_set_devices(arr, len(devs)), f"set_devices({devs})")


def get_devices() -> list:
    arr = (ctypes.c_int32 * 16)()
    n = load().kfmi_get_devices(arr, 16)
    return [arr[i] for i in range(n)]


def build_stats() -> dict:
    t, r = ctypes.c_uint64(), ctypes.c_uint32()
    _check(load().kfmi_build_stats(ctypes.byref(t), ctypes.byref(r)), "build_stats")
    return {"ties": int(t.value), "rounds": int(r.value)}


def device_count() -> int:
    return int(load().kfmi_device_count())


def host_threads() -> int:
    return int(load().kfmi_host_threads())


def device_pci_bus_id(dev: int) -> str:
    buf = ctypes.create_string_buffer(64)
    _check(load().kfmi_device_pci_bus_id(int(dev), buf, 64), f"device_pci_bus_id({dev})")
    return buf.value.decode()


def upload_form(queries) -> str:
    return ("none", "ascii", "packed")[load().kfmi_queries_upload_form(queries.ptr)]


def last_timing():
    t = [ctypes.c_double() for _ in range(3)]
    load().kfmi_last_timing(*[ctypes.byref(x) for x in t])
    return {"total_ms": t[0].value, "pack_ms": t[1].value, "lf_ms": t[2].value}


def _owned_view(addr: int, nbytes: int, dtype, owner) -> np.ndarray:
    buf = (ctypes.c_uint8 * nbytes).from_address(addr)
    buf._kfmi_owner = owner
    return np.frombuffer(buf, dtype=dtype)


class _Handle:
    _free = ""

    def __init__(self, ptr):
        self._p = ctypes.c_void_p(ptr)

    @property
    def ptr(self):
        return self._p

    def close(self):
        if self._p and self._p.value:
            getattr(load(), self._free)(ctypes.byref(self._p))
            self._p = ctypes.c_void_p(None)

    def __del__(self):
        try:
            self.close()
        except Exception:
            pass


class Index(_Handle):
    _free = "freeIndex"

    @classmethod
    def load(cls, path, required_tag: int = 0) -> "Index":
        L = load()
        p = ctypes.c_void_p()
        if required_tag:
            _check(L.kfmi_load_index_tag(str(path).encode(), required_tag, ctypes.byref(p)), f"load {path}")
        else:
            _check(L.loadIndex(str(path).encode(), ctypes.byref(p)), f"load {path}")
        return cls(p.value)

    @classmethod
    def from_image(cls, image) -> "Index":
        buf = np.ascontiguousarray(np.frombuffer(image, dtype=np.uint8) if isinstance(image, (bytes, bytearray))
                                   else image).view(np.uint8)
        p = ctypes.c_void_p()
        _check(load().kfmi_index_from_image(buf.ctypes.data, buf.nbytes, ctypes.byref(p)), "index_from_image")
        return cls(p.value)

    @classmethod
    def build(cls, text: bytes, k: int = 2, d: int = 64, gpu: bool = False, host_image: bool = True,
              sa_rate: int = 0) -> "Index":
        L = load()
        buf = np.frombuffer(text, dtype=np.uint8)
        p = ctypes.c_void_p()
        if sa_rate:
            err = L.kfmi_build_index_ex(buf.ctypes.data, buf.size, k, d, int(sa_rate), int(bool(gpu)),
                                        ctypes.byref(p))
        elif gpu:
            err = L.kfmi_build_index_gpu(buf.ctypes.data, buf.size, k, d, int(host_image), ctypes.byref(p))
        else:
            err = L.kfmi_build_index_cpu(buf.ctypes.data, buf.size, k, d, ctypes.byref(p))
        _check(err, "build_index")
        return cls(p.value)

    def header(self) -> dict:
        out = np.zeros(14, dtype=np.uint32)
        _check(load().kfmi_index_header(self._p, out.ctypes.data), "header")
        k = int(out[1])
        return dict(tag=int(out[0]), steps=k, bwtsize=int(out[2]), ncounters=int(out[3]),
                    nentries=int(out[4]), chunk=int(out[5]),
                    dollar_pos=[int(x) for x in out[6:6 + k]],
                    dollar_base=[int(x) for x in out[10:10 + k]])

    def image(self) -> np.ndarray:
        p = ctypes.c_void_p()
        n = ctypes.c_uint64()
        _check(load().kfmi_index_image(self._p, ctypes.byref(p), ctypes.byref(n)), "image")
        return _owned_view(p.value, n.value, np.uint8, self)

    def save(self, fn) -> None:
        _check(load().saveIndex(str(fn).encode(), self._p), f"saveIndex {fn}")

    def derive(self, k: int, host_image: bool = False) -> "Index":
        p = ctypes.c_void_p()
        _check(load().kfmi_derive_index_gpu(self._p, int(k), int(bool(host_image)), ctypes.byref(p)), "derive_index")
        return Index(p.value)

    def interleave(self) -> "Index":
        p = ctypes.c_void_p()
        _check(load().kfmi_transform_interleave(self._p, ctypes.byref(p)), "transform_interleave")
        return Index(p.value)

    def alt_counters(self):
        a, b = ctypes.c_void_p(), ctypes.c_void_p()
        _check(load().kfmi_transform_ac(self._p, ctypes.byref(a), ctypes.byref(b)), "transform_ac")
        return Index(a.value), Index(b.value)

    def plain(self) -> "Index":
        p = ctypes.c_void_p()
        _check(load().kfmi_transform_plain(self._p, ctypes.byref(p)), "transform_plain")
        return Index(p.value)

    def device_bytes(self) -> int:
        return int(load().kfmi_device_index_bytes(self._p))

    def ftab_bytes(self) -> int:
        return int(load().kfmi_device_ftab_bytes(self._p))

    def skip_bytes(self) -> int:
        return int(load().kfmi_device_skip_bytes(self._p))

    def jump_bytes(self) -> int:
        return int(load().kfmi_device_jump_bytes(self._p))

    def jump_tables(self, member: int = 0):
        rows = int(self.header()["bwtsize"])
        words = (rows - 1) // 16 + 2
        sa = np.empty(rows, dtype=np.uint32)
        isa = np.empty(rows, dtype=np.uint32)
        text = np.empty(words, dtype=np.uint32)
        as_p = lambda a: a.ctypes.data_as(ctypes.c_void_p)
        _check(load().kfmi_device_jump_tables(self._p, int(member), as_p(sa), as_p(isa), rows, as_p(text), words),
               "jump_tables")
        return sa, isa, text

    def jump_line_bytes(self) -> int:
        return int(load().kfmi_device_jump_line_bytes(self._p))

    def jump_lines(self, member: int = 0):
        lines = (int(self.header()["bwtsize"]) - 1) // 16 + 2
        out = np.empty((lines, 32), dtype=np.uint32)
        _check(load().kfmi_device_jump_lines(self._p, int(member), out.ctypes.data_as(ctypes.c_void_p), lines),
               "jump_lines")
        return out

    def skip_table(self):
        rows = int(self.header()["bwtsize"])
        out = np.empty((rows, 2), dtype=np.uint32)
        j = ctypes.c_uint32(0)
        _check(load().kfmi_device_skip_table(self._p, out.ctypes.data_as(ctypes.c_void_p), rows, ctypes.byref(j)),
               "skip_table")
        return int(j.value), out

    def sa(self):
        p = ctypes.c_void_p()
        n = ctypes.c_uint64()
        rate = ctypes.c_uint32()
        _check(load().kfmi_index_sa(self._p, ctypes.byref(p), ctypes.byref(n), ctypes.byref(rate)), "index_sa")
        if not n.value:
            return 0, np.zeros(0, dtype=np.uint32)
        return int(rate.value), _owned_view(p.value, 4 * n.value, np.uint32, self)

    def save_sa(self, fn) -> None:
        _check(load().kfmi_save_sa(str(fn).encode(), self._p), f"save_sa {fn}")

    def load_sa(self, fn) -> None:
        _check(load().kfmi_load_sa(str(fn).encode(), self._p), f"load_sa {fn}")

    def free_gpu(self) -> None:
        load().freeIndexGPU(ctypes.byref(self._p))


class Queries(_Handle):
    _free = "freeQueries"

    @classmethod
    def from_array(cls, q: np.ndarray) -> "Queries":
        q = np.ascontiguousarray(q, dtype=np.uint8)
        n, m = q.shape
        p = ctypes.c_void_p()
        _check(load().kfmi_queries_from_buffer(q.ctypes.data, n, m, ctypes.byref(p)), "queries_from_buffer")
        return cls(p.value)

    @classmethod
    def load(cls, path, size: int, num: int) -> "Queries":
        p = ctypes.c_void_p()
        _check(load().loadQueries(str(path).encode(), size, num, ctypes.byref(p)), f"loadQueries {path}")
        return cls(p.value)

    @classmethod
    def load_gpu(cls, path, size: int, num: int = 0) -> "Queries":
        p = ctypes.c_void_p()
        _check(load().kfmi_load_queries_gpu(str(path).encode(), size, num, ctypes.byref(p)),
               f"kfmi_load_queries_gpu {path}")
        return cls(p.value)

    def num(self) -> int:
        return int(ctypes.c_uint64.from_address(self._p.value).value)

    def free_gpu(self) -> None:
        load().freeQueriesGPU(ctypes.byref(self._p))


class Results(_Handle):
    _free = "freeResults"

    @classmethod
    def alloc(cls, num: int) -> "Results":
        p = ctypes.c_void_p()
        _check(load().kfmi_results_alloc(num, ctypes.byref(p)), "results_alloc")
        return cls(p.value)

    def array(self) -> np.ndarray:
        L = load()
        n = int(L.kfmi_results_num(self._p))
        ptr = L.kfmi_results_host(self._p)
        if not n:
            return np.zeros(0, dtype=np.uint32)
        return _owned_view(ctypes.cast(ptr, ctypes.c_void_p).value, 8 * n, np.uint32, self)

    def save(self, fn) -> None:
        _check(load().saveResults(str(fn).encode(), self._p, None), f"saveResults {fn}")

    def free_gpu(self) -> None:
        load().freeResultsGPU(ctypes.byref(self._p))


def transfer_to_gpu(index: Index | None, queries: Queries | None, results: Results | None) -> None:
    _check(load().transferCPUtoGPU(index.ptr if index else None, queries.ptr if queries else None,
                                   results.ptr if results else None), "transferCPUtoGPU")


def search(index: Index, queries: Queries, results: Results) -> None:
    _check(load().kfmi_search(index.ptr, queries.ptr, results.ptr), "searchIndexGPU")


def transfer_to_cpu(results: Results) -> None:
    _check(load().transferGPUtoCPU(results.ptr), "transferGPUtoCPU")


def count_blocks(index: Index, queries: Queries) -> int:
    n = ctypes.c_uint64()
    _check(load().kfmi_count_blocks(index.ptr, queries.ptr, ctypes.byref(n)), "count_blocks")
    return int(n.value)


def count_lines(index: Index, queries: Queries) -> dict:
    out = (ctypes.c_uint64 * 4)()
    _check(load().kfmi_count_lines(index.ptr, queries.ptr, out), "count_lines")
    return {"lines": int(out[0]), "counter_outside_planes_line": int(out[1]), "ends_fetched": int(out[2]),
            "line_local_ends": int(out[3])}


def probe_replay(index: Index, queries: Queries, unroll: int = 1, reps: int = 5, groups: int = 1) -> dict:
    ms, lines, tb = ctypes.c_double(), ctypes.c_uint64(), ctypes.c_uint64()
    _check(load().kfmi_probe_replay(index.ptr, queries.ptr, int(unroll), int(groups), int(reps), ctypes.byref(ms),
                                    ctypes.byref(lines), ctypes.byref(tb)), "kfmi_probe_replay")
    return {"unroll": int(unroll), "groups": int(groups), "ms": ms.value, "lines": int(lines.value), "trace_bytes": int(tb.value),
            "G_lines_per_s": lines.value / (ms.value / 1e3) / 1e9 if ms.value > 0 else None}


class Locations(_Handle):
    _free = "kfmi_locations_free"

    _num = 0

    def offsets(self) -> np.ndarray:
        return _owned_view(load().kfmi_locations_offsets(self._p), 8 * (self._num + 1), np.uint64, self)

    def positions(self) -> np.ndarray:
        L = load()
        t = self.total()
        if not t:
            return np.zeros(0, dtype=np.uint32)
        return _owned_view(L.kfmi_locations_positions(self._p), 4 * t, np.uint32, self)

    def total(self) -> int:
        return int(load().kfmi_locations_total(self._p))


def locate(index: Index, results: Results, max_occ: int = 0) -> Locations:
    p = ctypes.c_void_p()
    _check(load().kfmi_locate(index.ptr, results.ptr, int(max_occ), ctypes.byref(p)), "kfmi_locate")
    loc = Locations(p.value)
    loc._num = int(load().kfmi_results_num(results.ptr))
    return loc


def locate_array(index: Index, queries: np.ndarray, backend: str | None = None, max_occ: int = 0):
    if backend:
        set_backend(backend)
    q = Queries.from_array(queries)
    r = Results.alloc(queries.shape[0])
    transfer_to_gpu(index, q, r)
    search(index, q, r)
    loc = locate(index, r, max_occ)
    transfer_to_cpu(r)
    out = (r.array().copy(), loc.offsets().copy(), loc.positions().copy())
    loc.close()
    q.close()
    r.close()
    return out


class _Pinned:

    def __init__(self, nbytes: int):
        self.ptr = ctypes.c_void_p()
        _check(load().kfmi_host_alloc(int(nbytes), ctypes.byref(self.ptr)), "kfmi_host_alloc")
        self.nbytes = int(nbytes)

    def __del__(self):
        if self.ptr and _lib is not None:
            _lib.kfmi_host_free(self.ptr)
            self.ptr = ctypes.c_void_p()


def pinned_empty(shape, dtype=np.uint8) -> np.ndarray:
    dt = np.dtype(dtype)
    n = int(np.prod(shape)) * dt.itemsize
    owner = _Pinned(max(n, 1))
    return _owned_view(owner.ptr.value, n, dt, owner).reshape(shape)


def pack_queries(reads: np.ndarray) -> np.ndarray:
    reads = np.ascontiguousarray(reads, dtype=np.uint8)
    n, m = reads.shape
    out = np.empty(((m + 15) // 16, n), dtype=np.uint32)
    _check(load().kfmi_pack_queries(reads.ctypes.data, n, m, out.ctypes.data), "kfmi_pack_queries")
    return out


def pack_queries_k(reads: np.ndarray, k: int) -> np.ndarray:
    reads = np.ascontiguousarray(reads, dtype=np.uint8)
    n, m = reads.shape
    r = m % k
    out = np.empty(((m - r + 15) // 16 + (1 if r else 0), n), dtype=np.uint32)
    _check(load().kfmi_pack_queries_k(reads.ctypes.data, n, m, int(k), out.ctypes.data), "kfmi_pack_queries_k")
    return out


STRAND_FWD, STRAND_REV, STRAND_BOTH = 1, 2, 3


def _strand_count(strands: int) -> int:
    return 2 if int(strands) == STRAND_BOTH else 1


def revcomp(reads: np.ndarray) -> np.ndarray:
    reads = np.ascontiguousarray(reads, dtype=np.uint8)
    n, m = reads.shape
    out = np.empty_like(reads)
    _check(load().kfmi_revcomp_queries(reads.ctypes.data, n, m, out.ctypes.data), "kfmi_revcomp_queries")
    return out


def strand_words_host(words: np.ndarray, m: int, k: int, strands: int) -> np.ndarray:
    words = np.ascontiguousarray(words, dtype=np.uint32)
    rows, n = words.shape
    out = np.empty((rows, _strand_count(strands) * n), dtype=np.uint32)
    _check(load().kfmi_strand_words_host(words.ctypes.data, n, int(m), int(k), int(strands), out.ctypes.data),
           "kfmi_strand_words_host")
    return out


def reverse_stream_host(words: np.ndarray, m: int, maxw: int) -> np.ndarray:
    words = np.ascontiguousarray(words, dtype=np.uint32)
    rows, n = words.shape
    if rows != int(maxw):
        raise KfmiError(33, "kfmi_reverse_stream_host")
    out = np.empty((rows, n), dtype=np.uint32)
    _check(load().kfmi_reverse_stream_host(words.ctypes.data, n, int(m), int(maxw), out.ctypes.data),
           "kfmi_reverse_stream_host")
    return out


def search_strands(index: Index, queries: Queries, results: Results, strands: int) -> None:
    _check(load().kfmi_search_strands(index.ptr, queries.ptr, results.ptr, int(strands)), "kfmi_search_strands")


def search_stream(index: Index, reads: np.ndarray, out: np.ndarray | None = None, chunk: int = 0,
                  strands: int = STRAND_FWD) -> np.ndarray:
    reads = np.ascontiguousarray(reads, dtype=np.uint8)
    n, m = reads.shape
    ns = _strand_count(strands)
    if out is None:
        out = np.empty(2 * ns * n, dtype=np.uint32)
    assert out.dtype == np.uint32 and out.flags.c_contiguous and out.size >= 2 * ns * n
    if int(strands) == STRAND_FWD:
        _check(load().kfmi_search_stream(index.ptr, reads.ctypes.data, n, m, out.ctypes.data, int(chunk)),
               "kfmi_search_stream")
    else:
        _check(load().kfmi_search_stream_strands(index.ptr, reads.ctypes.data, n, m, out.ctypes.data, int(chunk),
                                                 int(strands)), "kfmi_search_stream_strands")
    return out


def search_cpu(index: Index, queries: Queries, results: Results, nthreads: int = 0) -> None:
    _check(load().kfmi_search_cpu(index.ptr, queries.ptr, results.ptr, int(nthreads)), "searchIndexCPU")


def search_cpu_strands(index: Index, queries: Queries, results: Results, strands: int, nthreads: int = 0) -> None:
    _check(load().kfmi_search_cpu_strands(index.ptr, queries.ptr, results.ptr, int(strands), int(nthreads)),
           "kfmi_search_cpu_strands")


def search_cpu_array(index: Index, queries: np.ndarray, nthreads: int = 0, strands: int = STRAND_FWD) -> np.ndarray:
    q = Queries.from_array(queries)
    r = Results.alloc(_strand_count(strands) * queries.shape[0])
    try:
        if int(strands) == STRAND_FWD:
            search_cpu(index, q, r, nthreads)
        else:
            search_cpu_strands(index, q, r, strands, nthreads)
        return r.array().copy()
    finally:
        q.close()
        r.close()


def search_array(index: Index, queries: np.ndarray, backend: str | None = None,
                 strands: int = STRAND_FWD) -> np.ndarray:
    if backend:
        set_backend(backend)
    q = Queries.from_array(queries)
    r = Results.alloc(_strand_count(strands) * queries.shape[0])
    try:
        transfer_to_gpu(index, q, r)
        if int(strands) == STRAND_FWD:
            search(index, q, r)
        else:
            search_strands(index, q, r, strands)
        transfer_to_cpu(r)
        return r.array().copy()
    finally:
        q.close()
        r.close()


TRACE_JUMP_OUTCOMES = ("taken", "refused", "differed", "bad_isa")
TRACE_FIELDS = ("steps", "skip_hits", "skip_misses", "jump_tried", "jump_pos", "jump_nb", "jump_line",
                "jump_outcome", "start_steps", "jump_split")


def decode_trace(records: np.ndarray) -> dict:
    r = np.asarray(records, dtype=np.uint32).reshape(-1, 4).astype(np.int64)
    tried = r[:, 1] & 1
    no = tried == 0
    return {
        "steps": r[:, 0] & 0xFFFF,
        "skip_hits": (r[:, 0] >> 16) & 0xFF,
        "skip_misses": (r[:, 0] >> 24) & 0xFF,
        "jump_tried": tried,
        "jump_pos": np.where(no, -1, (r[:, 1] >> 4) & 0xFFF),
        "jump_nb": np.where(no, -1, (r[:, 1] >> 16) & 0xFFFF),
        "jump_line": np.where(no, -1, (r[:, 1] >> 1) & 1),
        "jump_outcome": np.where(no, -1, (r[:, 1] >> 2) & 3),
        "start_steps": r[:, 2],
        "jump_split": r[:, 3],
    }


def search_trace(index: Index, reads: np.ndarray, backend: str | None = None):
    if backend:
        set_backend(backend)
    q = Queries.from_array(reads)
    r = Results.alloc(reads.shape[0])
    rec = np.zeros((reads.shape[0], 4), dtype=np.uint32)
    try:
        transfer_to_gpu(index, q, r)
        _check(load().kfmi_search_trace(index.ptr, q.ptr, r.ptr, rec.ctypes.data_as(ctypes.c_void_p)),
               "kfmi_search_trace")
        transfer_to_cpu(r)
        return r.array().copy(), rec
    finally:
        q.close()
        r.close()


def search_seeds(index: Index, queries: Queries, intervals: Results, spans: Results, max_seeds: int,
                 strands: int = STRAND_FWD) -> None:
    _check(load().kfmi_search_seeds(index.ptr, queries.ptr, intervals.ptr, spans.ptr, int(max_seeds), int(strands)),
           "kfmi_search_seeds")


def search_seeds_cpu(index: Index, queries: Queries, intervals: Results, spans: Results, max_seeds: int,
                     strands: int = STRAND_FWD, nthreads: int = 0) -> None:
    _check(load().kfmi_search_seeds_cpu(index.ptr, queries.ptr, intervals.ptr, spans.ptr, int(max_seeds),
                                        int(strands), int(nthreads)), "kfmi_search_seeds_cpu")


def search_seeds_array(index: Index, reads: np.ndarray, backend: str | None = None, max_seeds: int = 4,
                       strands: int = STRAND_FWD, cpu: bool = False):
    if backend and not cpu:
        set_backend(backend)
    n, s = reads.shape[0], int(max_seeds)
    slots = max(s, 0) * _strand_count(strands) * n
    q = Queries.from_array(reads)
    iv, sp = Results.alloc(slots), Results.alloc(slots)
    try:
        if cpu:
            search_seeds_cpu(index, q, iv, sp, s, strands)
        else:
            transfer_to_gpu(index, q, iv)
            transfer_to_gpu(index, None, sp)
            search_seeds(index, q, iv, sp, s, strands)
            transfer_to_cpu(iv)
            transfer_to_cpu(sp)
        shape = (_strand_count(strands) * n, s, 2)
        return iv.array().copy().reshape(shape), sp.array().copy().reshape(shape)
    finally:
        q.close()
        iv.close()
        sp.close()


HIT_NONE = 0xFFFFFFFF
HIT_MISM_MASK = 0x0000FFFF
HIT_MULTI = 0x00010000
HIT_SCORED_SHIFT = 20
VERIFY_MAX_OCC = 256


def results_to_gpu(results: Results) -> None:
    _check(load().kfmi_results_to_device(results.ptr), "kfmi_results_to_device")


def verify_seeds(index: Index, queries: Queries, intervals: Results, spans: Results, hits: Results, max_seeds: int,
                 strands: int, max_occ: int, max_mism: int) -> None:
    _check(load().kfmi_verify_seeds(index.ptr, queries.ptr, intervals.ptr, spans.ptr, hits.ptr, int(max_seeds),
                                    int(strands), int(max_occ), int(max_mism)), "kfmi_verify_seeds")


def verify_seeds_cpu(text, sa: np.ndarray, queries: Queries, intervals: Results, spans: Results, hits: Results,
                     max_seeds: int, strands: int, max_occ: int, max_mism: int, nthreads: int = 0) -> None:
    t = np.ascontiguousarray(np.frombuffer(text, dtype=np.uint8) if isinstance(text, (bytes, bytearray)) else text,
                             dtype=np.uint8)
    sa = np.ascontiguousarray(sa, dtype=np.uint32)
    _check(load().kfmi_verify_seeds_cpu(t.ctypes.data_as(ctypes.c_void_p), t.size, sa.ctypes.data_as(ctypes.c_void_p),
                                        sa.size, queries.ptr, intervals.ptr, spans.ptr, hits.ptr, int(max_seeds),
                                        int(strands), int(max_occ), int(max_mism), int(nthreads)),
           "kfmi_verify_seeds_cpu")


def decode_hits(hits: np.ndarray):
    h = np.asarray(hits, dtype=np.uint32).reshape(-1, 2)
    x, y = h[:, 0].astype(np.int64), h[:, 1].astype(np.int64)
    none = x == HIT_NONE
    return (np.where(none, -1, x), np.where(none, 0, y & HIT_MISM_MASK), ((y & HIT_MULTI) != 0) & ~none,
            y >> HIT_SCORED_SHIFT)


def map_reads_array(index: Index, reads: np.ndarray, backend: str | None = None, max_seeds: int = 4,
                    strands: int = STRAND_BOTH, max_occ: int = 8, max_mism: int | None = None, cpu: bool = False,
                    text=None):
    n, s = reads.shape[0], int(max_seeds)
    ns = _strand_count(strands)
    mm = 0xFFFFFFFF if max_mism is None else int(max_mism)
    if backend and not cpu:
        set_backend(backend)
    q = Queries.from_array(reads)
    iv, sp, hits = Results.alloc(max(s, 0) * ns * n), Results.alloc(max(s, 0) * ns * n), Results.alloc(ns * n)
    tmp = None
    try:
        if cpu:
            if text is None:
                raise ValueError("map_reads_array(cpu=True) needs the indexed text")
            rate, sa = index.sa()
            if rate != 1:
                tmp = Index.build(bytes(text), k=1, d=64, sa_rate=1)
                rate, sa = tmp.sa()
            search_seeds_cpu(index, q, iv, sp, s, strands)
            verify_seeds_cpu(text, sa, q, iv, sp, hits, s, strands, max_occ, mm)
        else:
            transfer_to_gpu(index, q, iv)
            transfer_to_gpu(index, None, sp)
            transfer_to_gpu(index, None, hits)
            search_seeds(index, q, iv, sp, s, strands)
            verify_seeds(index, q, iv, sp, hits, s, strands, max_occ, mm)
            transfer_to_cpu(hits)
        return decode_hits(hits.array().copy())
    finally:
        if tmp is not None:
            tmp.close()
        q.close()
        iv.close()
        sp.close()
        hits.close()


def env_int(name: str, default: int) -> int:
    try:
        return int(os.environ.get(name, default))
    except ValueError:
        return default
```

Baseline: 9985 Mqueries/s.

## Fold suffix-array position into ftab entries for singleton intervals

Re-encodes ftab entries whose interval width is one so the second word holds the suffix-array position (as 0xFFFFFFFF - p) instead of R. When a jump is attempted, the search can then take the starting position from the ftab entry and skip the dependent jsa[L] global load. The fold runs only when both the ftab and the jump tables were auto-built, and only after a check kernel confirms every interval width stays below the bound. It adds a decode branch to every ftab lookup and a one-time table rewrite pass.

After: 10790 Mqueries/s, median of 6. 1.08x the previous value.

```diff
diff --git a/include/kstep_fmi.h b/include/kstep_fmi.h
--- a/include/kstep_fmi.h
+++ b/include/kstep_fmi.h
@@ -103,6 +103,15 @@
 uint64_t    kfmi_device_jump_line_bytes(void *index);
 int32_t     kfmi_device_jump_lines(void *index, uint32_t member, uint32_t *out, uint64_t lines);
 int32_t     kfmi_jump_line_geometry(uint64_t n, uint64_t p, uint32_t nb, uint64_t *out);
+int32_t     kfmi_set_ftab_fold(uint32_t on);
+uint32_t    kfmi_ftab_fold(void);
+int32_t     kfmi_set_ftab_fold_bound(uint32_t bound);
+uint32_t    kfmi_ftab_fold_bound(uint64_t n);
+uint32_t    kfmi_ftab_fold_fits(uint64_t n, uint64_t max_width);
+int32_t     kfmi_ftab_fold_encode(uint64_t n, uint32_t L, uint32_t R, uint32_t p, uint32_t *out);
+int32_t     kfmi_ftab_fold_decode(uint64_t n, uint32_t x, uint32_t y, uint32_t folded, uint32_t *out);
+int32_t     kfmi_device_ftab_entries(void *index, uint32_t member, uint32_t *out, uint64_t first, uint64_t count,
+                                     uint32_t *bases, uint32_t *folded);
 int32_t     kfmi_set_split_class(uint32_t cls);
 int32_t     kfmi_set_fused(int32_t on);
 int32_t     kfmi_set_walk_check(uint32_t mode);
@@ -182,6 +191,7 @@
   KFMI_TRACE_JUMP_OUT_SHIFT = 2, KFMI_TRACE_JUMP_POS_SHIFT = 4, KFMI_TRACE_JUMP_NB_SHIFT = 16,
   KFMI_TRACE_JUMP_TAKEN = 0, KFMI_TRACE_JUMP_REFUSED = 1, KFMI_TRACE_JUMP_DIFFERED = 2, KFMI_TRACE_JUMP_BAD_ISA = 3
 };
+#define KFMI_TRACE_START_FOLDED 0x80000000u
 int32_t kfmi_search_trace(void *index, void *queries, void *results, uint32_t *trace);
 
 int32_t kfmi_probe_replay(void *index, void *queries, int32_t unroll, int32_t groups, int32_t reps, double *ms,
diff --git a/k-step_fm-index_amd/csrc/hip/kfmi_coop.h b/k-step_fm-index_amd/csrc/hip/kfmi_coop.h
--- a/k-step_fm-index_amd/csrc/hip/kfmi_coop.h
+++ b/k-step_fm-index_amd/csrc/hip/kfmi_coop.h
@@ -195,9 +195,9 @@
     uint32_t w0;
     if constexpr (MAXW > 0) w0 = cw[0];
     else w0 = qp[qs];
-    const uint2 lr = ix.ftab[w0 & ix.ftab_mask];
-    L = lr.x;
-    R = lr.y;
+    const FtabAt lr = ftab_lookup(ix, w0);
+    L = lr.L;
+    R = lr.R;
   }
   if (ix.rem) {
     if constexpr (MAXW == 0) rc = qp[(uint64_t) nwords * num + qs];
diff --git a/k-step_fm-index_amd/csrc/hip/kfmi_device.h b/k-step_fm-index_amd/csrc/hip/kfmi_device.h
--- a/k-step_fm-index_amd/csrc/hip/kfmi_device.h
+++ b/k-step_fm-index_amd/csrc/hip/kfmi_device.h
@@ -66,6 +66,7 @@
 constexpr uint32_t JUMP_LINE_S = 16, JUMP_LINE_W = 256 - JUMP_LINE_S, JUMP_LINE_DW = 32, JUMP_LINE_TEXT = JUMP_LINE_S;
 static_assert(JUMP_LINE_S == 16 && JUMP_LINE_S + 256 / 16 == JUMP_LINE_DW, "a line: S entries, then 256 bases in 16 dwords");
 constexpr uint32_t JUMP_SPLIT4 = 4u, JUMP_LINES = 0x100u, JUMP_LINES_GROUPED = 0x200u;
+constexpr uint32_t JUMP_FTAB_FOLDED = 0x400u;
 constexpr uint32_t JUMP_LINES_GROUPED_MAX_M = 192;
 
 __host__ __device__ constexpr uint64_t jump_text_words(uint64_t n) { return n / 16 + 2; }
@@ -86,6 +87,26 @@
   const uint64_t line = (uint64_t) j * JUMP_LINE_DW;
   return JumpLineAt{line + e % JUMP_LINE_S, line + JUMP_LINE_TEXT + (s >> 4), (s & 15u) * 2u,
                     ((s + nb + 15u) >> 4) - (s >> 4)};
+}
+
+struct FtabAt {
+  uint32_t L, R, p;
+};
+__host__ __device__ constexpr uint32_t ftab_fold_bound(uint32_t n) { return 0xFFFFFFFFu - n; }
+__host__ __device__ constexpr bool ftab_fold_fits(uint32_t n, uint32_t max_width) { return max_width < ftab_fold_bound(n); }
+__host__ __device__ inline uint2 ftab_fold_entry(uint32_t L, uint32_t R, uint32_t p)
+{
+  return make_uint2(L, R - L == 1u ? 0xFFFFFFFFu - p : R - L);
+}
+__host__ __device__ inline FtabAt ftab_entry_at(uint2 e, bool folded, uint32_t n)
+{
+  if (!folded) return FtabAt{e.x, e.y, SKIP_NONE};
+  const uint32_t c = 0xFFFFFFFFu - e.y;
+  return c <= n ? FtabAt{e.x, e.x + 1u, c} : FtabAt{e.x, e.x + e.y, SKIP_NONE};
+}
+__device__ __forceinline__ FtabAt ftab_lookup(const IdxArgs& ix, uint32_t w0)
+{
+  return ftab_entry_at(ix.ftab[w0 & ix.ftab_mask], (ix.jump_split & JUMP_FTAB_FOLDED) != 0u, ix.bwtsize - 1u);
 }
 
 typedef unsigned int v4u __attribute__((ext_vector_type(4)));
diff --git a/k-step_fm-index_amd/csrc/hip/kfmi_jump.hip b/k-step_fm-index_amd/csrc/hip/kfmi_jump.hip
--- a/k-step_fm-index_amd/csrc/hip/kfmi_jump.hip
+++ b/k-step_fm-index_amd/csrc/hip/kfmi_jump.hip
@@ -244,9 +244,10 @@
 
 int32_t use_jump(kfmi_dev_index* di, hipStream_t st, IdxArgs& ix, uint32_t want)
 {
+  const uint32_t folded = ix.jump_split & JUMP_FTAB_FOLDED;
   ix.jsa = nullptr;
   ix.jump_min = 0xFFFFFFFFu;
-  ix.jump_split = 1;
+  ix.jump_split = 1 | folded;
   if (!want || !jump_applies(di)) return KFMI_SUCCESS;
   if (want == 2) {
     const int32_t e = auto_jump(di, st);
@@ -265,7 +266,8 @@
   ix.jump_min = g_jump_min.load(std::memory_order_relaxed);
   const uint32_t lines = kfmi_jump_lines();
   const bool split4 = split_for(8ull * di->bwtsize, LAY_INTER) == 4u;
-  ix.jump_split = (split4 ? JUMP_SPLIT4 : 0u) | (lines ? JUMP_LINES : 0u) | (lines == 1u && split4 ? JUMP_LINES_GROUPED : 0u);
+  ix.jump_split = (split4 ? JUMP_SPLIT4 : 0u) | (lines ? JUMP_LINES : 0u) | (lines == 1u && split4 ? JUMP_LINES_GROUPED : 0u) |
+                  folded;
   return KFMI_SUCCESS;
 }
 
diff --git a/k-step_fm-index_amd/csrc/hip/kfmi_kernels.h b/k-step_fm-index_amd/csrc/hip/kfmi_kernels.h
--- a/k-step_fm-index_amd/csrc/hip/kfmi_kernels.h
+++ b/k-step_fm-index_amd/csrc/hip/kfmi_kernels.h
@@ -176,10 +176,11 @@
 
 template <class G, int MAXW, int SPLIT, bool JUMP = false, class TR = NoTrace>
 __device__ __forceinline__ void skip_walk(const IdxArgs& ix, const uint32_t (&cw)[MAXW], uint32_t steps, uint32_t pos,
-                                          uint32_t& Lq, uint32_t& Rq, typename TR::Out tr = typename TR::Out{})
+                                          uint32_t& Lq, uint32_t& Rq, typename TR::Out tr = typename TR::Out{},
+                                          uint32_t p0 = SKIP_NONE)
 {
   static_assert(G::K <= 2 && MAXW > 0, "skip table: fused task kernels at K <= 2");
-  [[maybe_unused]] uint32_t tr_walk = 0, tr_jump = 0, tr_line = 0;
+  [[maybe_unused]] uint32_t tr_walk = 0, tr_jump = 0, tr_line = 0, tr_fold = 0;
   [[maybe_unused]] const uint32_t tr_start = pos;
   extern __shared__ __attribute__((aligned(16))) uint8_t stage[];
   const uint32_t lane = threadIdx.x & 63u, wv = threadIdx.x >> 6;
@@ -206,13 +207,19 @@
     uint32_t p = SKIP_NONE;
     if constexpr (JUMP) {
       jmp = row1 && !(fl & 2u) && L[0] < ix.bwtsize && (steps - pos) * (uint32_t) G::K >= ix.jump_min;
+      const bool ld = jmp && p0 == SKIP_NONE;
       if (ix.jump_split & JUMP_SPLIT4) {
 #pragma unroll
         for (int g = 0; g < 4; ++g)
-          if (jmp && grp == g) p = ix.jsa[L[0]];
-      } else if (jmp) {
+          if (ld && grp == g) p = ix.jsa[L[0]];
+      } else if (ld) {
         p = ix.jsa[L[0]];
       }
+      if (jmp && !ld) {
+        p = p0;
+        if constexpr (TR::ON) tr_fold = KFMI_TRACE_START_FOLDED;
+      }
+      p0 = SKIP_NONE;
     }
     const bool one = row1 && !jmp && !is_dead() && L[0] < ix.skip_rows && pos + J <= steps;
     uint2 e = make_uint2(SKIP_NONE, 0u);
@@ -330,7 +337,7 @@
   }
   Lq = L[0];
   Rq = R[0];
-  if constexpr (TR::ON) *tr = make_uint4(tr_walk, tr_jump, tr_start, ix.jump_split);
+  if constexpr (TR::ON) *tr = make_uint4(tr_walk, tr_jump, tr_start | tr_fold, ix.jump_split & ~JUMP_FTAB_FOLDED);
 }
 
 template <class G, int MAXW, int SPLIT>
@@ -409,9 +416,10 @@
         dead = true;
       }
     } else if (jump) {
-      if (te.y > te.x) {
-        L[0] = te.x;
-        R[0] = te.y;
+      const FtabAt fe = ftab_entry_at(te, (ix.jump_split & JUMP_FTAB_FOLDED) != 0u, ix.bwtsize - 1u);
+      if (fe.R > fe.L) {
+        L[0] = fe.L;
+        R[0] = fe.R;
         pos += F;
       } else {
         dead = true;
@@ -466,6 +474,7 @@
     R[i] = ix.bwtsize;
   }
   uint32_t skip = 0;
+  [[maybe_unused]] uint32_t p0 = SKIP_NONE;
   if (ix.ftab && steps >= ix.ftab_steps) {
     skip = ix.ftab_steps;
 #pragma unroll
@@ -473,9 +482,10 @@
       uint32_t w0;
       if constexpr (MAXW > 0) w0 = cw[i][0];
       else w0 = qp[q[i]];
-      const uint2 lr = ix.ftab[w0 & ix.ftab_mask];
-      L[i] = lr.x;
-      R[i] = lr.y;
+      const FtabAt lr = ftab_lookup(ix, w0);
+      L[i] = lr.L;
+      R[i] = lr.R;
+      if constexpr (JUMP) p0 = lr.p;
     }
   }
   if (ix.rem) {
@@ -485,9 +495,10 @@
       L[i] = lr.x;
       R[i] = lr.y;
     }
+    p0 = SKIP_NONE;
   }
   if constexpr (SKIP) {
-    skip_walk<G, MAXW, SPLIT, JUMP, TR>(ix, cw[0], steps, skip, L[0], R[0], TR::at(trace, base));
+    skip_walk<G, MAXW, SPLIT, JUMP, TR>(ix, cw[0], steps, skip, L[0], R[0], TR::at(trace, base), p0);
     *reinterpret_cast<uint2*>(res + 2 * base) = make_uint2(L[0], R[0]);
     return;
   }
@@ -553,9 +564,9 @@
   uint32_t L = 0, R = ix.bwtsize, skip = 0;
   if (ix.ftab && steps >= ix.ftab_steps) {
     skip = ix.ftab_steps;
-    const uint2 lr = ix.ftab[cw[0] & ix.ftab_mask];
-    L = lr.x;
-    R = lr.y;
+    const FtabAt lr = ftab_lookup(ix, cw[0]);
+    L = lr.L;
+    R = lr.R;
   }
   if (ix.rem) {
     const uint2 lr = ix.rtab[qp[(uint64_t) nwords * num + q]];
@@ -610,9 +621,9 @@
   uint32_t L = 0, R = ix.bwtsize, skip = 0;
   if (ix.ftab && steps >= ix.ftab_steps) {
     skip = ix.ftab_steps;
-    const uint2 lr = ix.ftab[cw[0] & ix.ftab_mask];
-    L = lr.x;
-    R = lr.y;
+    const FtabAt lr = ftab_lookup(ix, cw[0]);
+    L = lr.L;
+    R = lr.R;
   }
   skip_walk<G, MAXW, SPLIT>(ix, cw, steps, skip, L, R);
   *reinterpret_cast<uint2*>(res + 2 * t) = make_uint2(L, R);
diff --git a/k-step_fm-index_amd/csrc/hip/kfmi_runtime.h b/k-step_fm-index_amd/csrc/hip/kfmi_runtime.h
--- a/k-step_fm-index_amd/csrc/hip/kfmi_runtime.h
+++ b/k-step_fm-index_amd/csrc/hip/kfmi_runtime.h
@@ -39,6 +39,7 @@
   uint2* ftab[17] = {};
   std::mutex ftab_mu;
   int ftab_auto = -1;
+  uint32_t ftab_folded = 0;
   uint2* skip = nullptr;
   int skip_auto = -1;
   uint32_t* jump_sa = nullptr;
diff --git a/k-step_fm-index_amd/csrc/hip/kfmi_tables.hip b/k-step_fm-index_amd/csrc/hip/kfmi_tables.hip
--- a/k-step_fm-index_amd/csrc/hip/kfmi_tables.hip
+++ b/k-step_fm-index_amd/csrc/hip/kfmi_tables.hip
@@ -153,6 +153,7 @@
   ix.ftab = nullptr;
   ix.ftab_steps = 0;
   ix.ftab_mask = 0;
+  ix.jump_split &= ~JUMP_FTAB_FOLDED;
   return KFMI_SUCCESS;
 }
 
@@ -177,15 +178,19 @@
   return KFMI_SUCCESS;
 }
 
-static int32_t auto_ftab(kfmi_dev_index* di, hipStream_t st, uint32_t* bases)
+static int32_t auto_ftab(kfmi_dev_index* di, hipStream_t st, uint32_t* bases, bool* built = nullptr)
 {
   std::lock_guard<std::mutex> lk(di->ftab_mu);
+  if (built) *built = false;
   if (di->ftab_auto < 0) {
     uint32_t n = kfmi_ftab_auto_bases(di->bwtsize, di->K, table_budget_now());
     for (; n; n -= di->K) {
       if (di->ftab[n]) break;
       const int32_t e = build_ftab(di, st, n);
-      if (!e) break;
+      if (!e) {
+        if (built) *built = true;
+        break;
+      }
       if (e != KFMI_E_DEVICE_ALLOC) return e;
     }
     di->ftab_auto = (int) n;
@@ -199,6 +204,7 @@
   ix.ftab = nullptr;
   ix.ftab_steps = 0;
   ix.ftab_mask = 0;
+  ix.jump_split &= ~JUMP_FTAB_FOLDED;
   if (bases == KFMI_FTAB_AUTO) {
     const int32_t e = auto_ftab(di, st, &bases);
     if (e) return e;
@@ -210,6 +216,7 @@
       const int32_t e = build_ftab(di, st, bases);
       if (e) return e;
     }
+    if ((di->ftab_folded >> bases) & 1u) ix.jump_split |= JUMP_FTAB_FOLDED;
   }
   ix.ftab = di->ftab[bases];
   ix.ftab_steps = bases / di->K;
@@ -314,6 +321,130 @@
   return KFMI_SUCCESS;
 }
 
+static std::atomic<int> g_ftab_fold{-1};
+static std::atomic<uint32_t> g_ftab_fold_bound{0};
+
+extern "C" int32_t kfmi_set_ftab_fold(uint32_t on)
+{
+  if (on > 1) return KFMI_E_BAD_ARGUMENT;
+  g_ftab_fold.store((int) on, std::memory_order_relaxed);
+  return KFMI_SUCCESS;
+}
+
+extern "C" uint32_t kfmi_ftab_fold(void)
+{
+  const int v = g_ftab_fold.load(std::memory_order_relaxed);
+  if (v >= 0) return (uint32_t) v;
+  static const uint32_t env = [] {
+    const char* e = getenv("KFMI_FTAB_FOLD");
+    return !e || !*e || atoi(e) ? 1u : 0u;
+  }();
+  return env;
+}
+
+extern "C" int32_t kfmi_set_ftab_fold_bound(uint32_t bound)
+{
+  g_ftab_fold_bound.store(bound, std::memory_order_relaxed);
+  return KFMI_SUCCESS;
+}
+
+extern "C" uint32_t kfmi_ftab_fold_bound(uint64_t n) { return n >= 0xFFFFFFFFull ? 0u : ftab_fold_bound((uint32_t) n); }
+
+extern "C" uint32_t kfmi_ftab_fold_fits(uint64_t n, uint64_t max_width)
+{
+  return n < 0xFFFFFFFFull && max_width <= 0xFFFFFFFFull && ftab_fold_fits((uint32_t) n, (uint32_t) max_width) ? 1u : 0u;
+}
+
+extern "C" int32_t kfmi_ftab_fold_encode(uint64_t n, uint32_t L, uint32_t R, uint32_t p, uint32_t* out)
+{
+  if (!out || n >= 0xFFFFFFFFull) return KFMI_E_BAD_ARGUMENT;
+  if (R - L == 1u ? (uint64_t) p > n : !ftab_fold_fits((uint32_t) n, R - L)) return KFMI_E_BAD_ARGUMENT;
+  const uint2 e = ftab_fold_entry(L, R, p);
+  out[0] = e.x;
+  out[1] = e.y;
+  return KFMI_SUCCESS;
+}
+
+extern "C" int32_t kfmi_ftab_fold_decode(uint64_t n, uint32_t x, uint32_t y, uint32_t folded, uint32_t* out)
+{
+  if (!out || n >= 0xFFFFFFFFull) return KFMI_E_BAD_ARGUMENT;
+  const FtabAt at = ftab_entry_at(make_uint2(x, y), folded != 0u, (uint32_t) n);
+  out[0] = at.L;
+  out[1] = at.R;
+  out[2] = at.p;
+  return KFMI_SUCCESS;
+}
+
+__global__ __launch_bounds__(256) void ftab_fold_check_kernel(const uint2* __restrict__ t, uint64_t entries, uint32_t rows,
+                                                              uint32_t* __restrict__ maxw)
+{
+  uint32_t m = 0;
+  for (uint64_t i = (uint64_t) blockIdx.x * 256 + threadIdx.x; i < entries; i += (uint64_t) gridDim.x * 256) {
+    const uint2 e = t[i];
+    const uint32_t w = e.y - e.x;
+    if (w != 1u) m = max(m, w);
+    else if (e.x >= rows) m = 0xFFFFFFFFu;
+  }
+#pragma unroll
+  for (int o = 32; o; o >>= 1) m = max(m, (uint32_t) __shfl_xor((int) m, o));
+  if ((threadIdx.x & 63u) == 0u && m) atomicMax(maxw, m);
+}
+
+__global__ __launch_bounds__(256) void ftab_fold_kernel(uint2* __restrict__ t, uint64_t entries,
+                                                        const uint32_t* __restrict__ sa, uint32_t split)
+{
+  const int grp = (int) (threadIdx.x & 63) / 16;
+  for (uint64_t i0 = (uint64_t) blockIdx.x * 256 + (threadIdx.x & ~63u); i0 < entries; i0 += (uint64_t) gridDim.x * 256) {
+    const uint64_t i = i0 + (threadIdx.x & 63u);
+    const bool on = i < entries;
+    const uint2 e = on ? t[i] : make_uint2(0u, 0u);
+    const bool one = on && e.y - e.x == 1u;
+    uint32_t p = 0u;
+    if (split) {
+#pragma unroll
+      for (int g = 0; g < 4; ++g)
+        if (one && grp == g) p = sa[e.x];
+    } else if (one) {
+      p = sa[e.x];
+    }
+    if (on) t[i] = ftab_fold_entry(e.x, e.y, p);
+  }
+}
+
+static int32_t fold_ftab(kfmi_dev_index* di, hipStream_t st)
+{
+  if (!kfmi_ftab_fold()) return KFMI_SUCCESS;
+  std::lock_guard<std::mutex> lk(di->ftab_mu);
+  const int N = di->ftab_auto;
+  if (N <= 0 || !di->ftab[N] || !di->jump_sa || ((di->ftab_folded >> N) & 1u)) return KFMI_SUCCESS;
+  const uint64_t entries = 1ull << (2 * N);
+  const uint32_t rows = di->bwtsize;
+  uint32_t* d_max = nullptr;
+  if (hipMalloc((void**) &d_max, 4) != hipSuccess) {
+    (void) hipGetLastError();
+    return KFMI_SUCCESS;
+  }
+  uint32_t h_max = 0xFFFFFFFFu;
+  const dim3 grid(grid_blocks((entries + 255) / 256, 1u << 14));
+  bool ok = hipMemsetAsync(d_max, 0, 4, st) == hipSuccess;
+  if (ok) {
+    hipLaunchKernelGGL(ftab_fold_check_kernel, grid, dim3(256), 0, st, di->ftab[N], entries, rows, d_max);
+    ok = hipGetLastError() == hipSuccess && hipMemcpyAsync(&h_max, d_max, 4, hipMemcpyDeviceToHost, st) == hipSuccess &&
+         hipStreamSynchronize(st) == hipSuccess;
+  }
+  (void) hipFree(d_max);
+  if (!ok) return KFMI_E_KERNEL;
+  uint32_t bound = ftab_fold_bound(rows - 1u);
+  const uint32_t lowered = g_ftab_fold_bound.load(std::memory_order_relaxed);
+  if (lowered && lowered < bound) bound = lowered;
+  if (h_max >= bound) return KFMI_SUCCESS;
+  const uint32_t split = split_for(8ull * rows, LAY_INTER) == 4u ? 1u : 0u;
+  hipLaunchKernelGGL(ftab_fold_kernel, grid, dim3(256), 0, st, di->ftab[N], entries, di->jump_sa, split);
+  if (hipGetLastError() != hipSuccess || hipStreamSynchronize(st) != hipSuccess) return KFMI_E_KERNEL;
+  di->ftab_folded |= 1u << N;
+  return KFMI_SUCCESS;
+}
+
 int32_t use_tables(kfmi_dev_index* di, hipStream_t st, IdxArgs& ix, const TableWants& w, uint32_t rem)
 {
   int32_t err = use_ftab(di, st, ix, w.ftab);
@@ -326,9 +457,15 @@
 int32_t auto_tables(kfmi_dev_index* di, hipStream_t st, const TableWants& w)
 {
   int32_t err = KFMI_SUCCESS;
-  if (w.ftab == KFMI_FTAB_AUTO) err = auto_ftab(di, st, nullptr);
+  bool ftab_built = false, jump_built = false;
+  if (w.ftab == KFMI_FTAB_AUTO) err = auto_ftab(di, st, nullptr, &ftab_built);
   if (!err && w.skip == 2u) err = auto_skip(di, st);
-  if (!err && w.jump == 2u) err = auto_jump(di, st);
+  if (!err && w.jump == 2u) {
+    const bool had = di->jump_sa != nullptr;
+    err = auto_jump(di, st);
+    jump_built = !err && !had && di->jump_sa != nullptr;
+  }
+  if (!err && ftab_built && jump_built) err = fold_ftab(di, st);
   return err;
 }
 
@@ -343,6 +480,7 @@
       t = nullptr;
     }
   di->ftab_auto = -1;
+  di->ftab_folded = 0;
   if (di->skip) (void) hipFree(di->skip);
   di->skip = nullptr;
   di->skip_auto = -1;
@@ -395,6 +533,28 @@
 extern "C" uint64_t kfmi_device_ftab_bytes(void* index) { return sum_members(index, ftab_bytes_of); }
 
 extern "C" uint64_t kfmi_device_skip_bytes(void* index) { return sum_members(index, skip_bytes_of); }
+
+extern "C" int32_t kfmi_device_ftab_entries(void* index, uint32_t member, uint32_t* out, uint64_t first, uint64_t count,
+                                            uint32_t* bases, uint32_t* folded)
+{
+  kfmi_fmi_t* f = (kfmi_fmi_t*) index;
+  if (!f || !out) return KFMI_E_BAD_ARGUMENT;
+  DeviceGuard dg;
+  std::shared_lock<RwLock> lk(index_lock(f));
+  kfmi_dev_index* di = nullptr;
+  const int32_t e = member_index(f, member, &di);
+  if (e) return e;
+  std::lock_guard<std::mutex> tl(di->ftab_mu);
+  const int N = di->ftab_auto;
+  if (N <= 0 || !di->ftab[N]) return KFMI_E_NOT_ON_DEVICE;
+  const uint64_t entries = 1ull << (2 * N);
+  if (first > entries || count > entries - first) return KFMI_E_BAD_ARGUMENT;
+  if (hipSetDevice(di->device) != hipSuccess) return KFMI_E_NO_DEVICE;
+  if (count) HIP_OK(hipMemcpy(out, di->ftab[N] + first, 8ull * count, hipMemcpyDeviceToHost));
+  if (bases) *bases = (uint32_t) N;
+  if (folded) *folded = (di->ftab_folded >> N) & 1u;
+  return KFMI_SUCCESS;
+}
 
 extern "C" int32_t kfmi_device_skip_table(void* index, void* out, uint64_t entries, uint32_t* steps)
 {
diff --git a/k-step_fm-index_amd/kstep_fmi/__init__.py b/k-step_fm-index_amd/kstep_fmi/__init__.py
--- a/k-step_fm-index_amd/kstep_fmi/__init__.py
+++ b/k-step_fm-index_amd/kstep_fmi/__init__.py
@@ -127,6 +127,14 @@
         "kfmi_device_jump_line_bytes": (u64, [vp]),
         "kfmi_device_jump_lines": (i32, [vp, u32, vp, u64]),
         "kfmi_jump_line_geometry": (i32, [u64, u64, u32, ctypes.POINTER(ctypes.c_uint64)]),
+        "kfmi_set_ftab_fold": (i32, [u32]),
+        "kfmi_ftab_fold": (u32, []),
+        "kfmi_set_ftab_fold_bound": (i32, [u32]),
+        "kfmi_ftab_fold_bound": (u32, [u64]),
+        "kfmi_ftab_fold_fits": (u32, [u64, u64]),
+        "kfmi_ftab_fold_encode": (i32, [u64, u32, u32, u32, ctypes.POINTER(u32)]),
+        "kfmi_ftab_fold_decode": (i32, [u64, u32, u32, u32, ctypes.POINTER(u32)]),
+        "kfmi_device_ftab_entries": (i32, [vp, u32, vp, u64, u64, ctypes.POINTER(u32), ctypes.POINTER(u32)]),
         "kfmi_set_fused": (i32, [i32]),
         "kfmi_set_walk_check": (i32, [u32]),
         "kfmi_fail_index_uploads": (i32, [u32]),
@@ -195,6 +203,38 @@
     _check(load().kfmi_set_ftab_budget(0xFFFFFFFFFFFFFFFF if nbytes is None else int(nbytes)), "set_ftab_budget")
 
 
+def set_ftab_fold(on) -> None:
+    _check(load().kfmi_set_ftab_fold(int(on)), f"set_ftab_fold({on})")
+
+
+def ftab_fold() -> int:
+    return int(load().kfmi_ftab_fold())
+
+
+def set_ftab_fold_bound(bound) -> None:
+    _check(load().kfmi_set_ftab_fold_bound(0 if bound is None else int(bound)), f"set_ftab_fold_bound({bound})")
+
+
+def ftab_fold_bound(n: int) -> int:
+    return int(load().kfmi_ftab_fold_bound(int(n)))
+
+
+def ftab_fold_fits(n: int, max_width: int) -> bool:
+    return bool(load().kfmi_ftab_fold_fits(int(n), int(max_width)))
+
+
+def ftab_fold_encode(n: int, L: int, R: int, p: int = 0):
+    out = (ctypes.c_uint32 * 2)()
+    _check(load().kfmi_ftab_fold_encode(int(n), int(L), int(R), int(p), out), f"ftab_fold_encode({n}, {L}, {R}, {p})")
+    return int(out[0]), int(out[1])
+
+
+def ftab_fold_decode(n: int, x: int, y: int, folded: bool = True):
+    out = (ctypes.c_uint32 * 3)()
+    _check(load().kfmi_ftab_fold_decode(int(n), int(x), int(y), int(bool(folded)), out), "ftab_fold_decode")
+    return int(out[0]), int(out[1]), (None if int(out[2]) == 0xFFFFFFFF else int(out[2]))
+
+
 SKIP_AUTO = 0xFFFFFFFF
 
 
@@ -455,6 +495,19 @@
         _check(load().kfmi_device_jump_lines(self._p, int(member), out.ctypes.data_as(ctypes.c_void_p), lines),
                "jump_lines")
         return out
+
+    def ftab_entries(self, first: int = 0, count=None, member: int = 0):
+        L = load()
+        b, fo = ctypes.c_uint32(0), ctypes.c_uint32(0)
+        if count is None:
+            probe = np.empty((0, 2), dtype=np.uint32)
+            _check(L.kfmi_device_ftab_entries(self._p, int(member), probe.ctypes.data_as(ctypes.c_void_p), 0, 0,
+                                              ctypes.byref(b), ctypes.byref(fo)), "ftab_entries")
+            count = (1 << (2 * int(b.value))) - int(first)
+        out = np.empty((int(count), 2), dtype=np.uint32)
+        _check(L.kfmi_device_ftab_entries(self._p, int(member), out.ctypes.data_as(ctypes.c_void_p), int(first),
+                                          int(count), ctypes.byref(b), ctypes.byref(fo)), "ftab_entries")
+        return int(b.value), bool(fo.value), out
 
     def skip_table(self):
         rows = int(self.header()["bwtsize"])
@@ -768,9 +821,14 @@
         "jump_nb": np.where(no, -1, (r[:, 1] >> 16) & 0xFFFF),
         "jump_line": np.where(no, -1, (r[:, 1] >> 1) & 1),
         "jump_outcome": np.where(no, -1, (r[:, 1] >> 2) & 3),
-        "start_steps": r[:, 2],
+        "start_steps": r[:, 2] & 0x7FFFFFFF,
         "jump_split": r[:, 3],
     }
+
+
+def trace_start_folded(records: np.ndarray) -> np.ndarray:
+    r = np.asarray(records, dtype=np.uint32).reshape(-1, 4).astype(np.int64)
+    return (r[:, 2] >> 31) & 1
 
 
 def search_trace(index: Index, reads: np.ndarray, backend: str | None = None):
```
